# dylkot/cNMF

Measured on AMD Instinct MI355X. Metric: NMF restarts/sec (50000x2000xK5..13), higher is better.
Workload: dtype f32 (exact integer f16 plane x 2 f16 planes with per-row exponent, f32 accumulate)

## Files before the change

### cnmf_amd/csrc/batch_host.hip.h

```cpp
#pragma once

#include "batch_sched.h"

static_assert(PLAN_BK == BK && PLAN_G3_MW == G3_MW && PLAN_G3_JW == G3_JW && PLAN_G3C_JW == G3C_JW && PLAN_G3_BK == G3_BK &&
              PLAN_KSMALL == KSMALL, "pass_plan.h repeats the tile constants of the kernel headers");
static PadShape pad_shape(const cnmf_ctx* ctx) { return PadShape{ctx->N_pad, ctx->G_pad}; }
static int sweep_chunks(const cnmf_ctx* ctx, int L) { return sweep_chunks(ctx->knobs.sweep_parts, L); }
static int sweep_parts(const cnmf_ctx* ctx, int L) { return sweep_parts(ctx->knobs.sweep_parts, L); }

static int ensure_batch(cnmf_ctx* ctx, int KC, int max_k = KMAX, int min_k = 1)
{
    const bool use3 = gemm3_enabled(ctx, KC);
    const SplitCaps caps = size_splits(pad_shape(ctx), KC, use3, gemm3_wg_slots(ctx->knobs));
    const int nsplit = caps.nsplit, nsplitA = caps.nsplitA;
    const int parts = std::max(sweep_parts(ctx, (int)ctx->N), sweep_parts(ctx, (int)ctx->G));
    const size_t gp_need = (size_t)(KC / std::max(1, min_k) + 1) * parts * max_k * max_k;
    if (ctx->bat.kc == KC && ctx->bat.nsplit == nsplit && ctx->bat.nsplitA == nsplitA &&
        ctx->bat.parts == parts && ctx->bat.gram_part_floats >= gp_need && (!use3 || ctx->bat.H3)) return CNMF_OK;
    ctx->bat.release();
    OwnedLocal<BatchBuffersF> b;
    const size_t hb = (size_t)KC * ctx->G_pad * sizeof(float);
    const size_t wb = (size_t)KC * ctx->N_pad * sizeof(float);
    HIP_TRY(ctx, hipMalloc(&b.H, hb));
    HIP_TRY(ctx, hipMalloc(&b.Wt, wb));
    HIP_TRY(ctx, hipMalloc(&b.XHt, wb * nsplitA));
    HIP_TRY(ctx, hipMalloc(&b.XHt1, wb));
    if (use3) {
        HIP_TRY(ctx, hipMalloc(&b.XHt2, wb));
        HIP_TRY(ctx, hipMalloc(&b.H3, (size_t)KC * (ctx->G_pad / 16) * G3_ROWB));
        HIP_TRY(ctx, hipMalloc(&b.Wt3, (size_t)KC * (ctx->N_pad / 16) * G3_ROWB));
        HIP_TRY(ctx, hipMemsetAsync(b.Wt3, 0, (size_t)KC * (ctx->N_pad / 16) * G3_ROWB, ctx->stream));
        HIP_TRY(ctx, hipMalloc(&b.rmaxH, (size_t)KC * parts * sizeof(float)));
        HIP_TRY(ctx, hipMalloc(&b.rmaxW, (size_t)KC * parts * sizeof(float)));
        HIP_TRY(ctx, hipMalloc(&b.iscaleH, (size_t)KC * sizeof(float)));
        HIP_TRY(ctx, hipMalloc(&b.iscaleW, (size_t)KC * sizeof(float)));
        HIP_TRY(ctx, hipMemsetAsync(b.rmaxH, 0, (size_t)KC * parts * sizeof(float), ctx->stream));
        HIP_TRY(ctx, hipMemsetAsync(b.rmaxW, 0, (size_t)KC * parts * sizeof(float), ctx->stream));
        HIP_TRY(ctx, hipMemsetAsync(b.iscaleH, 0, (size_t)KC * sizeof(float), ctx->stream));
        HIP_TRY(ctx, hipMemsetAsync(b.iscaleW, 0, (size_t)KC * sizeof(float), ctx->stream));
        HIP_TRY(ctx, hipMalloc(&b.shiftW, (size_t)3 * KC * sizeof(int)));
        HIP_TRY(ctx, hipMemsetAsync(b.shiftW, 0, (size_t)3 * KC * sizeof(int), ctx->stream));
    }
    HIP_TRY(ctx, hipMalloc(&b.d_split, (size_t)(KC / 32 + 1) * (ctx->N_pad / 128 + 1)));
    HIP_TRY(ctx, hipMalloc(&b.XtW, hb * nsplit));
    HIP_TRY(ctx, hipMalloc(&b.gramH, (size_t)KC * GRAM_SZ * sizeof(float)));
    HIP_TRY(ctx, hipMalloc(&b.gramW, (size_t)KC * GRAM_SZ * sizeof(float)));
    HIP_TRY(ctx, hipMalloc(&b.gram_part, gp_need * sizeof(float)));
    HIP_TRY(ctx, hipMalloc(&b.viol_part, (size_t)KC * parts * sizeof(double)));
    HIP_TRY(ctx, hipMalloc(&b.d_slots, (size_t)KC * sizeof(SlotDesc)));
    HIP_TRY(ctx, hipMalloc(&b.d_slot_list, (size_t)KC * RING * sizeof(int)));
    HIP_TRY(ctx, hipHostMalloc(&b.h_slots, (size_t)KC * sizeof(SlotDesc)));
    HIP_TRY(ctx, hipHostMalloc(&b.h_snap, (size_t)KC * RING * sizeof(SlotDesc),
                               hipHostMallocMapped | hipHostMallocCoherent));
    memset(b.h_snap, 0, (size_t)KC * RING * sizeof(SlotDesc));
    HIP_TRY(ctx, hipHostMalloc(&b.h_slot_list, (size_t)KC * RING * sizeof(int)));
    HIP_TRY(ctx, hipMemsetAsync(b.H, 0, hb, ctx->stream));
    HIP_TRY(ctx, hipMemsetAsync(b.Wt, 0, wb, ctx->stream));
    HIP_TRY(ctx, hipMemsetAsync(b.XHt, 0, wb * nsplitA, ctx->stream));
    HIP_TRY(ctx, hipMemsetAsync(b.XtW, 0, hb * nsplit, ctx->stream));
    HIP_TRY(ctx, hipMemsetAsync(b.d_slots, 0, (size_t)KC * sizeof(SlotDesc), ctx->stream));
    b.kc = KC; b.nsplit = nsplit; b.nsplitA = nsplitA; b.parts = parts; b.gram_part_floats = gp_need;
    ctx->bat.take(b);
    return CNMF_OK;
}

static int ensure_stage(cnmf_ctx* ctx, size_t wfloats, size_t hfloats)
{
    if (wfloats > ctx->stageW_sz) {
        hipFree(ctx->stageW); ctx->stageW = nullptr;
        HIP_TRY(ctx, hipMalloc(&ctx->stageW, wfloats * sizeof(float)));
        ctx->stageW_sz = wfloats;
    }
    if (hfloats > ctx->stageH_sz) {
        hipFree(ctx->stageH); ctx->stageH = nullptr;
        HIP_TRY(ctx, hipMalloc(&ctx->stageH, hfloats * sizeof(float)));
        ctx->stageH_sz = hfloats;
    }
    return CNMF_OK;
}

static int wait_snapshot(cnmf_ctx* ctx, const SlotDesc* sp, int n, int stamp)
{
    using clk = std::chrono::steady_clock;
    for (int s = 0; s < n; ++s) {
        const volatile int* flag = &sp[s].pad_;
        long spins = 0;
        clk::time_point t0;
        bool timing = false;
        while (*flag != stamp) {
            if (++spins % 4096 != 0) continue;
            if (!timing) { t0 = clk::now(); timing = true; continue; }
            if (std::chrono::duration_cast<std::chrono::milliseconds>(clk::now() - t0).count() < 20) continue;
            t0 = clk::now();
            const hipError_t q = hipStreamQuery(ctx->stream);
            if (q == hipSuccess) {
                if (*flag == stamp) break;
                SET_ERR(ctx, "slot snapshot %d was never published (slot %d)", stamp, s);
                return CNMF_EHIP;
            }
            if (q != hipErrorNotReady) {
                SET_ERR(ctx, "stream failed while waiting for a slot snapshot: %s", hipGetErrorString(q));
                return CNMF_EHIP;
            }
        }
    }
    __atomic_thread_fence(__ATOMIC_ACQUIRE);
    return CNMF_OK;
}

static int validate_params(cnmf_ctx* ctx, const cnmf_cd_params* p)
{
    if (!p) { SET_ERR(ctx, "params is NULL"); return CNMF_EINVAL; }
    if (!(p->tol >= 0) || p->max_iter < 1) { SET_ERR(ctx, "bad tol/max_iter"); return CNMF_EINVAL; }
    if (p->l1_reg_W < 0 || p->l2_reg_W < 0 || p->l1_reg_H < 0 || p->l2_reg_H < 0) {
        SET_ERR(ctx, "negative regularisation"); return CNMF_EINVAL;
    }
    return CNMF_OK;
}

static_assert(SCHED_KMAX == KMAX && SCHED_RING == RING, "batch_sched.h repeats KMAX and RING");

struct PassScheme {
    bool use3 = false;
    bool usec = false;
    bool use2g = false;
    bool use2h = false;
    int mode = 0;
    XOperand xA{}, xB{};
    const double* dsc = nullptr;
    int jwA = G3_JW;
    int nsubA = 1, nsubB = 1, KbA = 0, KbB = 0;
    void leave_matrix_pipe() { use3 = usec = use2h = use2g = false; }
};

static int pick_scheme(cnmf_ctx* ctx, int KC, PassScheme* out)
{
    const CdKnobs& kn = ctx->knobs;
    PassScheme p;
    int rc;
    p.use3 = gemm3_enabled(ctx, KC);
    if (p.use3 && kn.gemm3 >= 3) {
        if ((rc = ensure_counts(ctx))) return rc;
        p.usec = ctx->counts.state == 1;
    }
    p.use2g = p.use3 && !p.usec && kn.gemm3 >= 4 && ctx->G_pad % G3C_JW == 0 && ctx->N_pad % G3C_JW == 0;
    if (p.use2g && (rc = ensure_x2planes(ctx))) return rc;
    p.use2h = (p.usec && ctx->counts.fmt == 4) || p.use2g;
    p.mode = !p.use3 ? 0 : (p.use2g ? 5 : (p.usec ? (p.use2h ? 4 : 3) : std::min(kn.gemm3, 2)));
    p.KbA = ctx->G_pad / 16; p.KbB = ctx->N_pad / 16;
    p.xA = p.use2g ? ctx->x2.passA() : ctx->counts.passA();
    p.xB = p.use2g ? ctx->x2.passB() : ctx->counts.passB();
    p.dsc = p.use2g ? nullptr : ctx->counts.d_scale;
    p.nsubA = p.use2h ? gemm2h_nsub(p.xA.hi != nullptr, p.KbA, kn.g2_nsub) : 1;
    p.nsubB = p.use2h ? gemm2h_nsub(p.xB.hi != nullptr, p.KbB, kn.g2_nsub) : 1;
    if (p.use3 && !p.usec && !p.use2g && (rc = ensure_planes(ctx))) return rc;
    p.jwA = (p.usec || p.use2g) ? G3C_JW : G3_JW;
    *out = p;
    return CNMF_OK;
}

struct BatchRun {
    cnmf_ctx* ctx; const cnmf_cd_params* prm; hipStream_t st;
    int n; const int32_t* kk; int init_mode; const double* avg; const float *W0, *H0;
    int32_t* n_iter_out; double* viol_out; bool resident;
    int N, G, max_k; int64_t total_k;
    std::vector<size_t> hoff, woff;
    DevPool pool;
    EventPool events;
    struct PinnedInts { int* p = nullptr; ~PinnedInts() { if (p) hipHostFree(p); } } repack_host;
    float *d_Hres = nullptr, *d_Wres = nullptr;
    float *d_H0 = nullptr, *d_Wt0 = nullptr;
    int* d_repack = nullptr;
    int n_repack = 0;
    PassScheme ps;
    bool fuseW = false;
    int shgen = 0;
    int* shW[2] = {nullptr, nullptr};
    bool h3_valid = false;
    int fin_y = 1, lag = 2;
    int chunksW, partsW, chunksH, partsH;
    float l1W, l2W, l1H, l2H;
    PassPlan plan;
    int time_stride = 0;
    std::vector<hipEvent_t> gev;
    hipEvent_t ev_begin = nullptr, ev_end = nullptr, ev_tail = nullptr;
    int nsplit3_first = 1;
    BatchSched sched;
    BatchRun(int n_, const int32_t* kk_, int KC, const double* hint, bool dbg) : n(n_), kk(kk_), sched(n_, kk_, KC, hint, dbg) {}
};

static int plan_passes(BatchRun& b, int cap, int capA)
{
    cnmf_ctx* ctx = b.ctx;
    PassPlan& p = b.plan;
    plan_pass_splits(p, pad_shape(ctx), b.sched.KC, b.ps.use3, b.ps.jwA, b.ps.nsubA, gemm3_wg_slots(ctx->knobs), ctx->knobs.no_streamk, cap, capA);
    const std::vector<unsigned char>* flags = b.ps.use3 ? (p.sk3.on ? &p.sk3.flags : nullptr) : (p.sk.on ? &p.sk.split : nullptr);
    if (flags) HIP_TRY(ctx, hipMemcpyAsync(ctx->bat.d_split, flags->data(), flags->size(), hipMemcpyHostToDevice, b.st));
    return CNMF_OK;
}

static int retire_slot(BatchRun& b, int s, const SlotDesc& snap)
{
    cnmf_ctx* ctx = b.ctx;
    hipStream_t st = b.st;
    const HostSlot& h = b.sched.hs[s];
    const int r = h.restart, k = h.k, N = b.N, G = b.G;
    dim3 gH((G + 255) / 256, k), gW((N + 255) / 256, k);
    extract_kernel<<<gH, 256, 0, st>>>(ctx->bat.H, ctx->G_pad, G, h.off, k, b.d_Hres + b.hoff[r], 0);
    if (b.d_Wres) extract_kernel<<<gW, 256, 0, st>>>(ctx->bat.Wt, ctx->N_pad, N, h.off, k, b.d_Wres + b.woff[r], 1);
    clear_rows_kernel<<<gH, 256, 0, st>>>(ctx->bat.H, ctx->G_pad, ctx->G_pad, h.off, k);
    clear_rows_kernel<<<gW, 256, 0, st>>>(ctx->bat.Wt, ctx->N_pad, ctx->N_pad, h.off, k);
    HIP_TRY(ctx, hipGetLastError());
    if (b.n_iter_out) b.n_iter_out[r] = snap.iter;
    if (b.viol_out) b.viol_out[r] = snap.viol_last;
    b.sched.retire(s, snap.iter);
    return CNMF_OK;
}

static int repack(BatchRun& b, int width, bool balanced = false)
{
    cnmf_ctx* ctx = b.ctx;
    hipStream_t st = b.st;
    const int KC0 = b.sched.KC0;
    int* hm = b.repack_host.p + (size_t)(b.n_repack++ % RING) * 3 * KC0;
    int* d_colmap = b.d_repack, *d_ids = b.d_repack + KC0, *d_offs = b.d_repack + 2 * KC0;
    const RepackPlan pl = b.sched.plan_repack(width, balanced, hm);
    if (pl.nmove || pl.pos < width) {
        HIP_TRY(ctx, hipMemcpyAsync(d_colmap, hm, (size_t)width * sizeof(int), hipMemcpyHostToDevice, st));
        gather_rows_cm_kernel<<<dim3((ctx->N_pad / 4 + 255) / 256, width), 256, 0, st>>>(ctx->bat.Wt, ctx->N_pad, d_colmap, ctx->bat.XHt);
        gather_rows_cm_kernel<<<dim3((ctx->G_pad / 4 + 255) / 256, width), 256, 0, st>>>(ctx->bat.H, ctx->G_pad, d_colmap, ctx->bat.XtW);
        HIP_TRY(ctx, hipGetLastError());
        HIP_TRY(ctx, hipMemcpyAsync(ctx->bat.Wt, ctx->bat.XHt, (size_t)width * ctx->N_pad * sizeof(float), hipMemcpyDeviceToDevice, st));
        HIP_TRY(ctx, hipMemcpyAsync(ctx->bat.H, ctx->bat.XtW, (size_t)width * ctx->G_pad * sizeof(float), hipMemcpyDeviceToDevice, st));
        if (b.fuseW) {
            int* tmp = ctx->bat.shiftW + 2 * ctx->bat.kc;
            for (int g2 = 0; g2 < 2; ++g2) {
                permute_ints_kernel<<<(width + 255) / 256, 256, 0, st>>>(b.shW[g2], d_colmap, tmp, width);
                HIP_TRY(ctx, hipMemcpyAsync(b.shW[g2], tmp, (size_t)width * sizeof(int), hipMemcpyDeviceToDevice, st));
            }
            HIP_TRY(ctx, hipGetLastError());
        }
        if (pl.nmove) {
            HIP_TRY(ctx, hipMemcpyAsync(d_ids, hm + KC0, (size_t)pl.nmove * sizeof(int), hipMemcpyHostToDevice, st));
            HIP_TRY(ctx, hipMemcpyAsync(d_offs, hm + 2 * KC0, (size_t)pl.nmove * sizeof(int), hipMemcpyHostToDevice, st));
            set_slot_offs_kernel<<<(pl.nmove + 255) / 256, 256, 0, st>>>(ctx->bat.d_slots, d_ids, d_offs, pl.nmove);
            HIP_TRY(ctx, hipGetLastError());
        }
    }
    b.h3_valid = false;
    if (b.ps.use2h) HIP_TRY(ctx, launch_rowmax_part(st, ctx->bat.Wt, ctx->N_pad, b.N, b.sched.KC, b.chunksW * 256, nullptr, b.partsW, ctx->bat.rmaxW));
    return CNMF_OK;
}

static int install(BatchRun& b, const Placement& p)
{
    cnmf_ctx* ctx = b.ctx;
    hipStream_t st = b.st;
    const int r = p.restart, k = p.k, off = p.off, N = b.N, G = b.G;
    dim3 gI((std::max(N, G) + 255) / 256, k);
    if (b.init_mode == 0) {
        HIP_TRY(ctx, hipMemcpyAsync(ctx->stageH, b.H0 + b.hoff[r], (size_t)k * G * sizeof(float), hipMemcpyHostToDevice, st));
        HIP_TRY(ctx, hipMemcpyAsync(ctx->stageW, b.W0 + b.woff[r], (size_t)k * N * sizeof(float), hipMemcpyHostToDevice, st));
        install_kernel<<<gI, 256, 0, st>>>(ctx->stageH, ctx->stageW, ctx->bat.H, ctx->G_pad, G, ctx->bat.Wt, ctx->N_pad, N, off, k);
    } else {
        install_cm_kernel<<<gI, 256, 0, st>>>(b.d_H0 + b.hoff[r], b.d_Wt0 + b.woff[r], ctx->bat.H, ctx->G_pad, G, ctx->bat.Wt, ctx->N_pad, N, off);
    }
    HIP_TRY(ctx, hipGetLastError());
    if (b.fuseW) {
        float mx = 0.f;
        if (b.init_mode == 1) mx = 6.0f * (float)b.avg[r];
        else if (b.init_mode == 2) mx = ctx->inits.maxW[r];
        else for (size_t q = 0; q < (size_t)k * N; ++q) mx = std::max(mx, b.W0[b.woff[r] + q]);
        int e2 = 0;
        if (mx > 0.f) std::frexp(mx, &e2);
        const int sh0 = mx > 0.f ? std::max(-110, std::min(120, 13 - e2)) : 0;
        set_ints_kernel<<<1, 128, 0, st>>>(b.shW[0], b.shW[1], off, k, sh0);
        HIP_TRY(ctx, hipGetLastError());
    }
    SlotDesc* d = &ctx->bat.h_slots[p.slot];
    memset(d, 0, sizeof *d);
    d->off = off; d->k = k; d->active = 1; d->iter = 0; d->restart = r;
    HIP_TRY(ctx, hipMemcpyAsync(ctx->bat.d_slots + p.slot, d, sizeof(SlotDesc), hipMemcpyHostToDevice, st));
    return CNMF_OK;
}

static int refill(BatchRun& b, int& n_new)
{
    cnmf_ctx* ctx = b.ctx;
    BatchSched& sc = b.sched;
    n_new = 0;
    int* new_list = ctx->bat.h_slot_list + (size_t)(sc.it % RING) * sc.KC0;
    int rc;
    sc.begin_refill();
    while (true) {
        Placement p;
        while (sc.next_placement(&p)) {
            if ((rc = install(b, p))) return rc;
            new_list[n_new++] = p.slot;
        }
        if (!sc.defrag_due()) break;
// ... 551 lines not shown
```

### cnmf_amd/csrc/cnmf_hip.hip

```cpp
#include <hip/hip_runtime.h>

#include <algorithm>
#include <chrono>
#include <cmath>
#include <cstdint>
#include <cstdio>
#include <cstdlib>
#include <cstring>
#include <functional>
#include <string>
#include <vector>

#include "../../include/cnmf_hip.h"
#ifdef CNMF_DEBUG_ABI
#include "../../include/cnmf_hip_debug.h"
#endif
#include "kernels_gemm.hip.h"
#include "kernels_gemm3.hip.h"
#include "kernels_counts.hip.h"
#include "kernels_planes.hip.h"
#include "kernels_gemm2h.hip.h"
#include "kernels_rng.hip.h"
#include "kernels_sweep.hip.h"

// ... 65 lines not shown

extern "C" void cnmf_destroy(cnmf_ctx* ctx)
{
    if (!ctx) return;
    hipSetDevice(ctx->device);
    hipStreamSynchronize(ctx->stream);
    ctx->bat.release();
    cnmf_comm_finalize(ctx);
    drop_derived_images(ctx);
    hipFree(ctx->X);
    hipFree(ctx->stageW); hipFree(ctx->stageH); hipFree(ctx->spectra);
    ctx->cons_ws.release();
    ctx->prep.release();
    ctx->pre.release();
    ctx->har.release();
    if (ctx->cons_pinned) hipHostFree(ctx->cons_pinned);
    hipStreamDestroy(ctx->stream);
    delete ctx;
}

static int alloc_dense(cnmf_ctx* ctx)
{
    const size_t bytes = ((size_t)ctx->N_pad + 1) * ctx->G_pad * sizeof(float);
    HIP_TRY(ctx, hipMalloc(&ctx->X, bytes));
    HIP_TRY(ctx, hipMemsetAsync(ctx->X, 0, bytes, ctx->stream));
    return CNMF_OK;
}

static int alloc_matrix(cnmf_ctx* ctx, int64_t N, int64_t G, bool dense = true)
{
    if (N <= 0 || G <= 0 || N > (1ll << 30) || G > (1ll << 24)) {
        SET_ERR(ctx, "bad matrix shape %lld x %lld", (long long)N, (long long)G);
        return CNMF_EINVAL;
    }
    HIP_TRY(ctx, hipSetDevice(ctx->device));
    ctx->bat.release();
    drop_derived_images(ctx);
    hipFree(ctx->X); ctx->X = nullptr;
    ctx->iter_prior.clear(); ctx->iter_hint.clear();
    ctx->N = N; ctx->G = G;
    ctx->N_pad = round_up(N, N >= 512 ? 256 : 128);
    ctx->G_pad = round_up(G, G >= 512 ? 256 : 32);
    return dense ? alloc_dense(ctx) : CNMF_OK;
}

extern "C" int cnmf_set_matrix(cnmf_ctx* ctx, const float* X, int64_t N, int64_t G)
{
    if (!ctx || !X) { SET_ERR(ctx, "null argument"); return CNMF_EINVAL; }
    int rc = alloc_matrix(ctx, N, G);
    if (rc) return rc;
    HIP_TRY(ctx, hipMemcpy2DAsync(ctx->X, (size_t)ctx->G_pad * sizeof(float), X,
                                  (size_t)G * sizeof(float), (size_t)G * sizeof(float), (size_t)N,
                                  hipMemcpyHostToDevice, ctx->stream));
    HIP_TRY(ctx, hipStreamSynchronize(ctx->stream));
    return CNMF_OK;
}

__global__ void csr_densify_kernel(const long long* __restrict__ indptr, const int* __restrict__ indices,
                                   const float* __restrict__ data, float* __restrict__ X, int ld,
                                   int n_rows, int n_cols, int* __restrict__ bad)
{
    const int row = blockIdx.x;
    if (row >= n_rows) return;
    const long long b = indptr[row], e = indptr[row + 1];
    for (long long p = b + threadIdx.x; p < e; p += blockDim.x) {
        const int c = indices[p];
        if (c < 0 || c >= n_cols) { if (bad) atomicOr(bad, 2); continue; }
        if (bad && ((p > b && indices[p - 1] >= c) || data[p] == 0.f)) atomicOr(bad, 1);
        if (X) atomicAdd(&X[(size_t)row * ld + c], data[p]);
    }
}

static int ensure_dense(cnmf_ctx* ctx)
{
    if (ctx->X) return CNMF_OK;
    if (ctx->N <= 0 || !ctx->csr.ptr) { SET_ERR(ctx, "cnmf_set_matrix has not been called"); return CNMF_ESTATE; }
    HIP_TRY(ctx, hipSetDevice(ctx->device));
    int rc = alloc_dense(ctx);
    if (rc) return rc;
    if (ctx->csr.nnz > 0) {
        csr_densify_kernel<<<(unsigned)ctx->N, 64, 0, ctx->stream>>>(ctx->csr.ptr, ctx->csr.idx, ctx->csr.val, ctx->X, ctx->G_pad,
                                                                    (int)ctx->N, (int)ctx->G, nullptr);
        hipError_t e = hipGetLastError();
        if (e == hipSuccess) e = hipStreamSynchronize(ctx->stream);
        if (e != hipSuccess) { hipFree(ctx->X); ctx->X = nullptr; HIP_TRY(ctx, e); }
    }
    return CNMF_OK;
}

extern "C" int cnmf_set_matrix_csr(cnmf_ctx* ctx, const int32_t* indptr, const int32_t* indices,
                                   const float* data, int64_t N, int64_t G)
{
    if (!ctx || !indptr || (!indices && indptr[N] > 0) || (!data && indptr[N] > 0)) {
        SET_ERR(ctx, "null argument");
        return CNMF_EINVAL;
    }
    int rc = alloc_matrix(ctx, N, G, false);
    if (rc) return rc;
    const int64_t nnz = indptr[N];
    DevPool pool;
    int* d_ptr32 = pool.get<int>((size_t)(N + 1));
    int* d_bad = pool.get<int>(1, true, ctx->stream);
    POOL_TRY(ctx, pool);
    hipStream_t st = ctx->stream;
    DevCsrLocal<float> L;
    HIP_TRY(ctx, L.alloc_ptr(N, G));
    HIP_TRY(ctx, L.alloc_entries(nnz));
    HIP_TRY(ctx, hipMemcpyAsync(d_ptr32, indptr, (size_t)(N + 1) * sizeof(int), hipMemcpyHostToDevice, st));
    if (nnz > 0) {
        HIP_TRY(ctx, hipMemcpyAsync(L.idx, indices, (size_t)nnz * sizeof(int), hipMemcpyHostToDevice, st));
        HIP_TRY(ctx, hipMemcpyAsync(L.val, data, (size_t)nnz * sizeof(float), hipMemcpyHostToDevice, st));
    }
    int bad = 0;
    cnmf::csr_widen_ptr_kernel<<<(unsigned)((N + 1 + 255) / 256), 256, 0, st>>>(d_ptr32, N + 1, L.ptr);
    if (nnz > 0) csr_densify_kernel<<<(unsigned)N, 64, 0, st>>>(L.ptr, L.idx, L.val, nullptr, ctx->G_pad, (int)N, (int)G, d_bad);
    HIP_TRY(ctx, hipGetLastError());
    HIP_TRY(ctx, hipMemcpyAsync(&bad, d_bad, sizeof(int), hipMemcpyDeviceToHost, st));
    HIP_TRY(ctx, hipStreamSynchronize(st));
    if (bad & 2) { SET_ERR(ctx, "column index out of range in the CSR arrays"); return CNMF_EINVAL; }
    ctx->csr.take(L);
    if (bad & 1) {
        rc = ensure_dense(ctx);
        free_csr(ctx);
        if (rc) return rc;
    }
    return CNMF_OK;
}

extern "C" int cnmf_set_count_detection(cnmf_ctx* ctx, int enabled)
{
    if (!ctx) return CNMF_EINVAL;
    if (ctx->count_detect != (enabled != 0)) {
        ctx->count_detect = enabled != 0;
        if (ctx->counts.state == -1 || !ctx->count_detect) {
            hipStreamSynchronize(ctx->stream);
            ctx->counts.release();
        }
    }
    return CNMF_OK;
}

extern "C" int cnmf_get_shape(const cnmf_ctx* ctx, int64_t* N, int64_t* G)
{
    if (!ctx) return CNMF_EINVAL;
    if (N) *N = ctx->N;
    if (G) *G = ctx->G;
    return (ctx->X || ctx->csr.ptr) ? CNMF_OK : CNMF_ESTATE;
}

extern "C" int cnmf_matrix_images(const cnmf_ctx* ctx, int32_t* flags)
{
    if (!ctx || !flags) return CNMF_EINVAL;
    *flags = (ctx->X ? 1 : 0) | (ctx->csr.ptr ? 2 : 0) | (ctx->csc.ptr ? 4 : 0) | (ctx->XtF.p ? 8 : 0) |
             ((ctx->spA[0].ent && ctx->spB[0].ent) ? 16 : 0) | ((ctx->spA[1].ent && ctx->spB[1].ent) ? 32 : 0) | (ctx->counts.C1 ? 64 : 0);
    return CNMF_OK;
}

#include "batch_host.hip.h"

#include "consensus_host.hip.h"
#include "linkage_host.hip.h"

#include "mu_host.hip.h"
#include "mu_refit_host.hip.h"
#include "comm_host.hip.h"
#include "normalize_host.hip.h"
#include "prepare_host.hip.h"
#include "preprocess_host.hip.h"
#include "pca_host.hip.h"
#include "tridiag_eig_host.hip.h"
#include "harmony_host.hip.h"
#include "harmony_init_host.hip.h"
#include "filter_host.hip.h"
#include "hvg_host.hip.h"
#include "hvg_batch_host.hip.h"
#include "select_mi_host.hip.h"
#include "tail_host.hip.h"
#include "mu2_refit_host.hip.h"

#include "debug_host.hip.h"
#include "nndsvd_host.hip.h"
#include "nndsvd_tail_host.hip.h"
#include "format_host.hip.h"
```

### cnmf_amd/csrc/debug_host.hip.h

```cpp
#pragma once

extern "C" int cnmf_x_matmul(cnmf_ctx* ctx, int trans, const float* Q, int ncols, float* out)
{
    if (!ctx || !Q || !out) { SET_ERR(ctx, "null argument"); return CNMF_EINVAL; }
    if (int rcd_ = ensure_dense(ctx)) return rcd_;
    if (ncols < 1 || ncols > 256 || (trans != 0 && trans != 1)) { SET_ERR(ctx, "bad ncols/trans"); return CNMF_EINVAL; }
    HIP_TRY(ctx, hipSetDevice(ctx->device));
    hipStream_t st = ctx->stream;
    const int N = (int)ctx->N, G = (int)ctx->G;
    const int KC = ncols <= 32 ? 32 : (ncols <= 64 ? 64 : (ncols <= 128 ? 128 : 256));
    const int Kin = trans ? N : G, Kp = trans ? ctx->N_pad : ctx->G_pad;
    const int Jout = trans ? G : N, Jp = trans ? ctx->G_pad : ctx->N_pad;
    DevPool pool;
    float* dQ = pool.get<float>((size_t)Kin * ncols);
    float* dA = pool.get<float>((size_t)KC * Kp, true, st);
    const int nsplit = trans ? std::max(1, std::min(16, Kp / 2048)) : 1;
    float* dC = pool.get<float>((size_t)nsplit * KC * Jp);
    float* dO = pool.get<float>((size_t)Jout * ncols);
    if (pool.err) { SET_ERR(ctx, "device allocation failed"); return CNMF_ENOMEM; }
    HIP_TRY(ctx, hipMemcpyAsync(dQ, Q, (size_t)Kin * ncols * sizeof(float), hipMemcpyHostToDevice, st));
    dim3 gI((Kin + 255) / 256, ncols);
    install_kernel<<<gI, 256, 0, st>>>(nullptr, dQ, dA, Kp, 0, dA, Kp, Kin, 0, ncols);
    if (!trans)
        HIP_TRY(ctx, launch_gemm<false>(st, 0, dA, Kp, ctx->X, ctx->G_pad, dC, Jp, 0, KC, Kp, Jp, 1));
// ... 20 lines not shown
    HIP_TRY(ctx, hipSetDevice(ctx->device));
    hipStream_t st = ctx->stream;
    const int Jp = round_up(J, 128);
    const int Kp = K;
    DevPool pool;
    EventPool events;
    const size_t bA = (size_t)KC * Kp * sizeof(float);
    const size_t bB = (mode == 0 ? (size_t)Jp * Kp : ((size_t)Kp + 1) * J + 128) * sizeof(float);
    const size_t bC = (size_t)nsplit * KC * Jp * sizeof(float);
    float* dA = pool.get<float>(bA / sizeof(float));
    float* dB = pool.get<float>(bB / sizeof(float));
    float* dC = pool.get<float>(bC / sizeof(float));
    POOL_TRY(ctx, pool);
    HIP_TRY(ctx, hipMemsetAsync(dB, 0, bB, st));
    HIP_TRY(ctx, hipMemcpyAsync(dA, A, bA, hipMemcpyHostToDevice, st));
    HIP_TRY(ctx, hipMemcpyAsync(dB, B, (size_t)(mode == 0 ? J : Kp) * (mode == 0 ? Kp : J) * sizeof(float), hipMemcpyHostToDevice, st));
    hipEvent_t e0 = events.get(), e1 = events.get();
    POOL_TRY(ctx, events);
    reps = std::max(1, reps);
    for (int i = 0; i < reps + 1; ++i) {
        if (i == 1) hipEventRecord(e0, st);
        hipError_t e = (mode == 0)
            ? launch_gemm<false>(st, variant, dA, Kp, dB, Kp, dC, Jp, (long long)KC * Jp, KC, Kp, Jp, 1, ctx->knobs.s_mtw2)
            : launch_gemm<true>(st, variant, dA, Kp, dB, J, dC, Jp, (long long)KC * Jp, KC, Kp, J, nsplit, ctx->knobs.s_mtw2);
        HIP_TRY(ctx, e);
    }
    hipEventRecord(e1, st);
    HIP_TRY(ctx, hipStreamSynchronize(st));
    float ms = 0.f;
    if (reps >= 1) hipEventElapsedTime(&ms, e0, e1);
    if (ms_out) *ms_out = (reps >= 1) ? ms / reps : 0.0;
    std::vector<float> hc((size_t)(mode == 0 ? 1 : nsplit) * KC * Jp);
    HIP_TRY(ctx, hipMemcpy(hc.data(), dC, hc.size() * sizeof(float), hipMemcpyDeviceToHost));
    for (int c = 0; c < KC; ++c)
        for (int j = 0; j < J; ++j) {
            float s = hc[(size_t)c * Jp + j];
            if (mode == 1)
                for (int z = 1; z < nsplit; ++z) s += hc[((size_t)z * KC + c) * Jp + j];
            C[(size_t)c * J + j] = s;
        }
    return CNMF_OK;
}

extern "C" int cnmf_debug_gemm3(cnmf_ctx* ctx, const float* A, const float* B, float* C, int KC, int K, int J,
                                int nsplit, double* ms_out, int reps)
{
    if (!ctx || !A || !B || !C) { SET_ERR(ctx, "null argument"); return CNMF_EINVAL; }
    if (KC % 256 || K % 16 || J < 1 || nsplit < 1) { SET_ERR(ctx, "debug_gemm3 needs KC %% 256 == 0, K %% 16 == 0"); return CNMF_EINVAL; }
    HIP_TRY(ctx, hipSetDevice(ctx->device));
    hipStream_t st = ctx->stream;
    const int Jp = round_up(J, gemm3_jw()), Kb = K / 16;
    DevPool pool;
    EventPool events;
    float* dA = pool.get<float>((size_t)KC * K);
    float* dB = pool.get<float>((size_t)Jp * K, true, st);
    unsigned char* dA3 = pool.get<unsigned char>((size_t)KC * Kb * G3_ROWB);
    unsigned char* dB3 = pool.get<unsigned char>((size_t)Jp * Kb * G3_ROWB);
    float* dC = pool.get<float>((size_t)nsplit * KC * Jp);
    hipEvent_t e0 = events.get(), e1 = events.get();
    POOL_TRY(ctx, pool);
    POOL_TRY(ctx, events);
    HIP_TRY(ctx, hipMemcpyAsync(dA, A, (size_t)KC * K * sizeof(float), hipMemcpyHostToDevice, st));
    HIP_TRY(ctx, hipMemcpyAsync(dB, B, (size_t)J * K * sizeof(float), hipMemcpyHostToDevice, st));
    HIP_TRY(ctx, launch_split3(st, dA, K, KC, K, dA3, G3_MW));
    HIP_TRY(ctx, launch_split3(st, dB, K, Jp, K, dB3, gemm3_jw()));
    reps = std::max(1, reps);
    int zs = 1;
    for (int i = 0; i < reps + 1; ++i) {
        if (i == 1) hipEventRecord(e0, st);
        HIP_TRY(ctx, launch_gemm3(st, dA3, dB3, Kb, dC, Jp, (long long)KC * Jp, KC, Jp, nsplit, ctx->knobs.gemm3));
    }
    hipEventRecord(e1, st);
    HIP_TRY(ctx, hipStreamSynchronize(st));
    { const int kb_per = (Kb + nsplit - 1) / nsplit; zs = (Kb + kb_per - 1) / kb_per; }
    float ms = 0.f;
    hipEventElapsedTime(&ms, e0, e1);
    if (ms_out) *ms_out = ms / reps;
    std::vector<float> hc((size_t)zs * KC * Jp);
    HIP_TRY(ctx, hipMemcpy(hc.data(), dC, hc.size() * sizeof(float), hipMemcpyDeviceToHost));
    for (int c = 0; c < KC; ++c)
        for (int j = 0; j < J; ++j) {
            float v = hc[(size_t)c * Jp + j];
            for (int z = 1; z < zs; ++z) v += hc[((size_t)z * KC + c) * Jp + j];
            C[(size_t)c * J + j] = v;
        }
    return CNMF_OK;
}

extern "C" int cnmf_debug_gemm3c(cnmf_ctx* ctx, const float* A, const float* Bn, float* C, int KC, int K, int J,
                                 int nsplit, double* ms_out, int reps)
{
    if (!ctx || !A || !Bn || !C) { SET_ERR(ctx, "null argument"); return CNMF_EINVAL; }
    if (KC % 256 || K % 16 || J < 1 || nsplit < 1) { SET_ERR(ctx, "debug_gemm3c needs KC %% 256 == 0, K %% 16 == 0"); return CNMF_EINVAL; }
    HIP_TRY(ctx, hipSetDevice(ctx->device));
    hipStream_t st = ctx->stream;
    const int Jp = round_up(J, G3C_JW), Kb = K / 16;
    DevPool pool;
    EventPool events;
    float* dA = pool.get<float>((size_t)KC * K);
    float* dB = pool.get<float>((size_t)J * K);
    float* dUnit = pool.get<float>(K);
    unsigned char* dA3 = pool.get<unsigned char>((size_t)KC * Kb * G3_ROWB);
    unsigned char* dB1 = pool.get<unsigned char>((size_t)Jp * Kb * 32);
    unsigned char* dBh = pool.get<unsigned char>((size_t)Jp * Kb * 32);
    unsigned int* dFl = pool.get<unsigned int>((size_t)(Jp / G3C_JW) * ((Kb + 31) / 32), true, st);
    float* dC = pool.get<float>((size_t)nsplit * KC * Jp);
    hipEvent_t e0 = events.get(), e1 = events.get();
    POOL_TRY(ctx, pool);
    POOL_TRY(ctx, events);
    std::vector<float> ones(K, 1.0f);
    HIP_TRY(ctx, hipMemcpyAsync(dA, A, (size_t)KC * K * sizeof(float), hipMemcpyHostToDevice, st));
    HIP_TRY(ctx, hipMemcpyAsync(dB, Bn, (size_t)J * K * sizeof(float), hipMemcpyHostToDevice, st));
    HIP_TRY(ctx, hipMemcpyAsync(dUnit, ones.data(), (size_t)K * sizeof(float), hipMemcpyHostToDevice, st));
    HIP_TRY(ctx, launch_split3(st, dA, K, KC, K, dA3, G3_MW));
    HIP_TRY(ctx, launch_x_planes(st, XPlaneFormat::COUNT_BF16, false, dB, K, J, K, Jp, K, dUnit, dB1, dBh, dFl));
    reps = std::max(1, reps);
    for (int i = 0; i < reps + 1; ++i) {
        if (i == 1) hipEventRecord(e0, st);
        HIP_TRY(ctx, launch_gemm3c(st, dA3, dB1, dBh, dFl, Kb, dC, Jp, (long long)KC * Jp, KC, Jp, nsplit));
    }
    hipEventRecord(e1, st);
    HIP_TRY(ctx, hipStreamSynchronize(st));
    const int kb_per = (Kb + nsplit - 1) / nsplit, zs = (Kb + kb_per - 1) / kb_per;
    float ms = 0.f;
    hipEventElapsedTime(&ms, e0, e1);
    if (ms_out) *ms_out = ms / reps;
    std::vector<float> hc((size_t)zs * KC * Jp);
    HIP_TRY(ctx, hipMemcpy(hc.data(), dC, hc.size() * sizeof(float), hipMemcpyDeviceToHost));
    for (int c = 0; c < KC; ++c)
        for (int j = 0; j < J; ++j) {
            float v = hc[(size_t)c * Jp + j];
            for (int z = 1; z < zs; ++z) v += hc[((size_t)z * KC + c) * Jp + j];
            C[(size_t)c * J + j] = v;
        }
    return CNMF_OK;
}

__global__ __launch_bounds__(256) void debug_rowbound_part_kernel(const float* __restrict__ V, int ld, int L, int span,
                                                                  int parts, float* __restrict__ rmax_part)
{
    const int row = blockIdx.y * 4 + (threadIdx.x >> 6), lane = threadIdx.x & 63, p = blockIdx.x;
    const int j0 = p * span, j1 = min(L, j0 + span);
    float s = 0.f;
    for (int j = j0 + lane; j < j1; j += 64) { const float x = V[(size_t)row * ld + j]; s = fmaf(x, x, s); }
#pragma unroll
    for (int o = 32; o > 0; o >>= 1) s += __shfl_xor(s, o, 64);
    if (lane == 0) rmax_part[(size_t)row * parts + p] = sqrtf(s) * 1.0001f;
}

extern "C" int cnmf_debug_gemm2h(cnmf_ctx* ctx, const float* A, const float* Bn, float* C, int KC, int K, int J,
                                 int nsplit, int nsub, double* ms_out, int reps)
{
    const bool sweep_bound = (nsub & 128) != 0;
    nsub &= 127;
    if (!ctx || !A || !Bn || !C) { SET_ERR(ctx, "null argument"); return CNMF_EINVAL; }
    if (KC % 256 || K % 64 || J < 1 || nsplit < 1) { SET_ERR(ctx, "debug_gemm2h needs KC %% 256 == 0, K %% 64 == 0"); return CNMF_EINVAL; }
    HIP_TRY(ctx, hipSetDevice(ctx->device));
    hipStream_t st = ctx->stream;
    const int Jp = round_up(J, G3C_JW), Kb = K / 16;
    bool has_hi = false;
    for (size_t i = 0; i < (size_t)J * K && !has_hi; ++i) has_hi = Bn[i] > G2_COUNT_BASE;
    DevPool pool;
    EventPool events;
    float* dA = pool.get<float>((size_t)KC * K);
    float* dB = pool.get<float>((size_t)J * K);
    float* dUnit = pool.get<float>(K);
    const int bparts = sweep_bound ? (K + 1023) / 1024 : 1;
    float* dRmax = pool.get<float>((size_t)KC * bparts);
    float* dInv = pool.get<float>(KC);
    unsigned char* dA2 = pool.get<unsigned char>((size_t)KC * Kb * G2_ROWB);
    unsigned char* dB1 = pool.get<unsigned char>((size_t)Jp * Kb * 32);
    unsigned char* dBh = has_hi ? pool.get<unsigned char>((size_t)Jp * Kb * 32) : nullptr;
    unsigned int* dFl = pool.get<unsigned int>((size_t)(Jp / G3C_JW) * ((Kb + 31) / 32), true, st);
    float* dC = pool.get<float>((size_t)nsplit * KC * Jp);
    hipEvent_t e0 = events.get(), e1 = events.get();
    POOL_TRY(ctx, pool);
    POOL_TRY(ctx, events);
    std::vector<float> ones(K, 1.0f);
    HIP_TRY(ctx, hipMemcpyAsync(dA, A, (size_t)KC * K * sizeof(float), hipMemcpyHostToDevice, st));
    HIP_TRY(ctx, hipMemcpyAsync(dB, Bn, (size_t)J * K * sizeof(float), hipMemcpyHostToDevice, st));
    HIP_TRY(ctx, hipMemcpyAsync(dUnit, ones.data(), (size_t)K * sizeof(float), hipMemcpyHostToDevice, st));
    if (sweep_bound) {
        debug_rowbound_part_kernel<<<dim3(bparts, KC / 4), 256, 0, st>>>(dA, K, K, 1024, bparts, dRmax);
        HIP_TRY(ctx, hipGetLastError());
    } else
        HIP_TRY(ctx, launch_rowmax_part(st, dA, K, K, KC, K, nullptr, 1, dRmax));
    HIP_TRY(ctx, launch_split2h(st, dA, K, KC, K, dA2, G3_MW, nullptr, dRmax, bparts, dInv));
    HIP_TRY(ctx, launch_x_planes(st, XPlaneFormat::COUNT_F16, false, dB, K, J, K, Jp, K, dUnit, dB1, dBh, dFl));
    reps = std::max(1, reps);
    const int var = (nsub >> 4) & 7;
    nsub &= 15;
    const int ns = (!has_hi && nsub == 2 && Kb % 2 == 0) ? 2 : 1;
    G2Launch g;
    g.A2 = dA2; g.rscale = dInv; g.x = XOperand{dB1, dBh, dFl, nullptr}; g.Kb = Kb;
    g.C[0] = dC; g.ldc = Jp; g.cstride = (long long)KC * Jp; g.KC = KC; g.Jpad = Jp; g.nsplit = nsplit;
    for (int i = 0; i < reps + 1; ++i) {
        if (i == 1) hipEventRecord(e0, st);
        hipError_t e;
        if (has_hi) e = launch_gemm2h_t<1, true>(st, g);
        else if (ns == 2 && var == 2) e = launch_gemm2h_t<2, false, 2>(st, g);
        else if (ns == 2 && var == 3) e = launch_gemm2h_t<2, false, 3>(st, g);
        else if (ns == 2 && var == 4) e = launch_gemm2h_t<2, false, 4>(st, g);
        else if (ns == 2 && var == 6) e = launch_gemm2h_t<2, false, 6>(st, g);
        else if (ns == 2 && var == 7) e = launch_gemm2h_t<2, false, 7>(st, g);
        else if (ns == 2) e = launch_gemm2h_t<2, false, 0>(st, g);
        else e = launch_gemm2h_t<1, false>(st, g);
        HIP_TRY(ctx, e);
    }
    hipEventRecord(e1, st);
    HIP_TRY(ctx, hipStreamSynchronize(st));
    const int zs = gemm2h_splits(Kb, nsplit, ns);
    float ms = 0.f;
    hipEventElapsedTime(&ms, e0, e1);
    if (ms_out) *ms_out = ms / reps;
    std::vector<float> hc((size_t)zs * KC * Jp);
    HIP_TRY(ctx, hipMemcpy(hc.data(), dC, hc.size() * sizeof(float), hipMemcpyDeviceToHost));
    for (int c = 0; c < KC; ++c)
        for (int j = 0; j < J; ++j) {
            float v = hc[(size_t)c * Jp + j];
            for (int z = 1; z < zs; ++z) v += hc[((size_t)z * KC + c) * Jp + j];
            C[(size_t)c * J + j] = v;
        }
    return CNMF_OK;
}

namespace cnmf {
__global__ __launch_bounds__(256) void calib_copy1_kernel(const float* __restrict__ a, float* __restrict__ b, long long n)
{
    for (long long i = (long long)blockIdx.x * 256 + threadIdx.x; i < n; i += (long long)gridDim.x * 256) b[i] = a[i];
}
__global__ __launch_bounds__(256) void calib_copy4_kernel(const float4* __restrict__ a, float4* __restrict__ b, long long n4)
{
    for (long long i = (long long)blockIdx.x * 256 + threadIdx.x; i < n4; i += (long long)gridDim.x * 256) b[i] = a[i];
}
__global__ __launch_bounds__(256) void calib_ldsdma_kernel(const unsigned char* __restrict__ a, long long nbytes, float* __restrict__ sink)
{
    __shared__ __attribute__((aligned(16))) unsigned char buf[4][4096];
    const long long chunk = 4096;
    float acc = 0.f;
    for (long long off = (long long)blockIdx.x * chunk; off + chunk <= nbytes; off += (long long)gridDim.x * chunk) {
        const int w = (threadIdx.x >> 6);
        __builtin_amdgcn_global_load_lds(G3_AS1(a + off + threadIdx.x * 16), G3_AS3(&buf[0][0] + w * 1024), 16, 0, 0);
        asm volatile("s_waitcnt vmcnt(0)" ::: "memory");
        acc += reinterpret_cast<const float*>(&buf[0][0])[threadIdx.x];
    }
    if (acc == 1.2345f) sink[0] = acc;
}
}

extern "C" int cnmf_debug_stream(cnmf_ctx* ctx, int width, long long n_floats, int reps)
{
    using namespace cnmf;
    if (!ctx || n_floats < 1024 || reps < 1) { SET_ERR(ctx, "bad argument"); return CNMF_EINVAL; }
    HIP_TRY(ctx, hipSetDevice(ctx->device));
    hipStream_t st = ctx->stream;
    DevPool pool;
    n_floats = (n_floats / 1024) * 1024;
    float* a = pool.get<float>((size_t)n_floats, true, st);
    float* b = pool.get<float>((size_t)n_floats, true, st);
    POOL_TRY(ctx, pool);
    for (int r = 0; r < reps; ++r) {
        if (width == 1) calib_copy1_kernel<<<4096, 256, 0, st>>>(a, b, n_floats);
        else if (width == 4) calib_copy4_kernel<<<4096, 256, 0, st>>>((const float4*)a, (float4*)b, n_floats / 4);
        else calib_ldsdma_kernel<<<2048, 256, 0, st>>>((const unsigned char*)a, n_floats * 4, b);
    }
    HIP_TRY(ctx, hipGetLastError());
    HIP_TRY(ctx, hipStreamSynchronize(st));
    return CNMF_OK;
}

extern "C" int cnmf_debug_standard_normal(cnmf_ctx* ctx, uint32_t seed, int64_t n, double* out)
{
    if (!ctx || !out || n < 0) { SET_ERR(ctx, "bad argument"); return CNMF_EINVAL; }
    HIP_TRY(ctx, hipSetDevice(ctx->device));
    DevPool pool;
    double* d = pool.get<double>((size_t)n);
    POOL_TRY(ctx, pool);
    launch_standard_normal(ctx->stream, seed, n, d);
    HIP_TRY(ctx, hipGetLastError());
    HIP_TRY(ctx, hipMemcpyAsync(out, d, (size_t)n * sizeof(double), hipMemcpyDeviceToHost, ctx->stream));
    HIP_TRY(ctx, hipStreamSynchronize(ctx->stream));
    return CNMF_OK;
}
#endif
```

### cnmf_amd/csrc/gemm_host.hip.h

```cpp
#pragma once

#include "pass_plan.h"


template <int MTW, int WM, int WN, bool NN, int TBK = BK>
static hipError_t launch_gemm_t(hipStream_t st, const float* A, int lda, const float* B, int ldb,
                                float* C, int ldc, long long cstride, int KC, int Ktot, int J,
                                int nsplit)
{
    constexpr int MW = WM * MTW * 32, JW = WN * 32;
    const int Kper = round_up((Ktot + nsplit - 1) / nsplit, BK);
    dim3 grid((J + JW - 1) / JW, KC / MW, nsplit);
    constexpr size_t lds = gemm_lds_bytes<MTW, WM, WN, NN, TBK>();
    {
        if (hipError_t e_ = dyn_lds_optin((const void*)gemm_kernel<MTW, WM, WN, NN, TBK>, (int)lds)) return e_;
    }
    gemm_kernel<MTW, WM, WN, NN, TBK><<<grid, 256, lds, st>>>(A, lda, B, ldb, C, ldc, cstride, Kper,
                                                             Ktot, J);
    return hipGetLastError();
}

template <bool NN>
static hipError_t launch_gemm(hipStream_t st, int variant, const float* A, int lda, const float* B,
                              int ldb, float* C, int ldc, long long cstride, int KC, int Ktot,
// ... 15 lines not shown
            if (KC % 128 == 0) GO(4, 1, 4);
            if (KC % 64 == 0) GO(2, 1, 4);
            GO(1, 1, 4);
    }
#undef GO
}

static constexpr CutPlanes NO_CUT{nullptr, nullptr, 1, 1, 1, nullptr};
static constexpr PlaneOut NO_PLANES{nullptr, nullptr, 0, 0};

struct SweepLaunch {
    int nslots = 0;
    float* V = nullptr; int ldv = 0, L = 0;
    const float* P = nullptr;
    enum { ONE_PLANE, CUT_PLANES, SPLIT_SUM } from = ONE_PLANE;
    CutPlanes cut = NO_CUT;
    SplitSum sum{1, 0, nullptr};
    const float* gram = nullptr;
    const SlotDesc* slots = nullptr;
    float l1 = 0.f;
    float* gram_part = nullptr; double* viol_part = nullptr;
    int chunks = 1, parts = 1;
    int want_gram = 0, kmax = 0, tiers = 0;
    float* rmax_part = nullptr;
    const double* rmax_scale = nullptr;
    const PlaneOut* planes = nullptr;
};

using SweepFn = void (*)(float*, int, int, const float*, SplitInfo, const float*, const SlotDesc*, float, float*, double*, int, int, int,
                         int, float*, const double*, PlaneOut);
static constexpr SweepFn SWEEP_KERNELS[6][3] = {
    {sweep_kernel<0>, sweep_kernel<1>, sweep_kernel<2>},
    {sweep_kernel<0, false, false, false, true>, sweep_kernel<1, false, false, false, true>, sweep_kernel<2, false, false, false, true>},
    {sweep_kernel<0, false, false, true>, sweep_kernel<1, false, false, true>, sweep_kernel<2, false, false, true>},
    {sweep_kernel<0, false, false, true, true>, sweep_kernel<1, false, false, true, true>, sweep_kernel<2, false, false, true, true>},
    {sweep_kernel<0, true>, sweep_kernel<1, true>, sweep_kernel<2, true>},
    {sweep_kernel<0, true, true>, sweep_kernel<1, true, true>, sweep_kernel<2, true, true>}};

static hipError_t launch_sweep(hipStream_t st, const SweepLaunch& s)
{
    const bool pln = s.planes != nullptr, exact = s.rmax_part && s.rmax_scale;
    const SweepForm form = sweep_form(pln, s.from == SweepLaunch::SPLIT_SUM, exact, sweep_a64(s.ldv), s.tiers);
    if (form == SweepForm::INVALID || (pln && s.planes->TR != G3_MW)) return hipErrorInvalidValue;
    SplitInfo sp;
    if (form == SweepForm::H_PSUM) sp.sum = s.sum;
    else sp.cut = s.from == SweepLaunch::CUT_PLANES ? s.cut : NO_CUT;
    const dim3 grid(s.parts, s.nslots);
    for (int t = 0; t < 3; ++t) {
        if (!(s.tiers & (1 << t))) continue;
        const SweepFn fn = SWEEP_KERNELS[(int)form][t];
        if (hipError_t e_ = dyn_lds_optin((const void*)fn, (int)sweep_lds_bytes(KSMALL, pln))) return e_;
        fn<<<grid, 256, sweep_lds_bytes(s.kmax, pln), st>>>(s.V, s.ldv, s.L, s.P, sp, s.gram, s.slots, s.l1, s.gram_part, s.viol_part, s.chunks,
                                                           s.want_gram, sweep_kg(s.kmax), s.kmax, s.rmax_part, pln ? nullptr : s.rmax_scale,
                                                           pln ? *s.planes : NO_PLANES);
    }
    if (s.tiers & 8) {
        const size_t blds = sweep_big_lds_bytes();
        const auto big = exact ? sweep_big_kernel<true> : sweep_big_kernel<false>;
        if (hipError_t e_ = dyn_lds_optin((const void*)big, (int)blds)) return e_;
        big<<<grid, 256, blds, st>>>(s.V, s.ldv, s.L, s.P, sp, s.gram, s.slots, s.l1, s.viol_part, s.chunks, exact ? s.rmax_part : nullptr,
                                     exact ? s.rmax_scale : nullptr);
        if (s.want_gram)
            gram_big_kernel<<<grid, 256, 0, st>>>(s.V, s.ldv, s.L, s.slots, s.gram_part, s.chunks, s.kmax,
                                                  (s.rmax_part && !s.rmax_scale) ? s.rmax_part : nullptr);
    }
    return hipGetLastError();
}

static hipError_t launch_streamk_passA(hipStream_t st, const StreamK& sk, const float* A, int lda,
                                       const float* B, int ldb, float* C0, float* C1, int ldc, int Jtot)
{
    constexpr size_t lds = gemm_lds_bytes<4, 1, 4, false>();
    {
        if (hipError_t e_ = dyn_lds_optin((const void*)gemm_streamk_kernel<4, 1, 4, false>, (int)lds)) return e_;
    }
    gemm_streamk_kernel<4, 1, 4, false><<<sk.P, 256, lds, st>>>(A, lda, B, ldb, C0, C1, ldc, sk.MG, sk.T,
                                                               sk.nk, Jtot);
    return hipGetLastError();
}

static hipError_t launch_reduce_splits(hipStream_t st, float* P, int nsplit, long long split_stride,
                                       long long n_floats, const double* colscale = nullptr, int ld = 1)
{
    if (nsplit <= 1 && !colscale) return hipSuccess;
    const long long nv = n_floats / 4;
    reduce_splits_kernel<<<(unsigned)((nv + 255) / 256), 256, 0, st>>>(P, nsplit, split_stride, P, nv, colscale, ld);
    return hipGetLastError();
}


static hipError_t launch_split3(hipStream_t st, const float* src, int ld, int rows, int K, unsigned char* dst, int TR,
                                const double* kscale = nullptr)
{
    if (rows % 64 == 0 && K % 64 == 0 && TR % 64 == 0) {
        if (rows / 64 > PLAN_GRID_YZ) return hipErrorInvalidValue;
        dim3 grid(K / 64, rows / 64);
        split3_tiled_kernel<<<grid, 256, 0, st>>>(src, ld, K, TR, (unsigned short*)dst, kscale);
        return hipGetLastError();
    }
    const long long total = (long long)rows * (K / 16);
    split3_kernel<<<(unsigned)((total + 255) / 256), 256, 0, st>>>(src, ld, rows, K, TR, (unsigned short*)dst, kscale);
    return hipGetLastError();
}

static int gemm3_wg_slots(const CdKnobs& k) { return gemm3_wg_slots(k.gemm3, k.wg_slots); }
static int gemm3_jw() { return G3_JW; }

static hipError_t launch_gemm3(hipStream_t st, const unsigned char* A3, const unsigned char* B3, int Kb,
                               float* C, int ldc, long long cstride, int KC, int Jpad, int nsplit, int gemm3_mode)
{
    {
        if (hipError_t e_ = dyn_lds_optin((const void*)gemm3_kernel, G3_LDS_BYTES)) return e_;
        if (hipError_t e_ = dyn_lds_optin((const void*)gemm3g_kernel, G3G_LDS_BYTES)) return e_;
    }
    const int kb_per = (Kb + nsplit - 1) / nsplit;
    dim3 grid(Jpad / gemm3_jw(), KC / G3_MW, (Kb + kb_per - 1) / kb_per);
    if (gemm3_mode >= 2)
        gemm3g_kernel<<<grid, 512, G3G_LDS_BYTES, st>>>(A3, B3, Kb, C, ldc, cstride, kb_per);
    else
        gemm3_kernel<<<grid, 256, G3_LDS_BYTES, st>>>(A3, B3, Kb, C, ldc, cstride, kb_per);
    return hipGetLastError();
}


static hipError_t launch_split3_finalize(hipStream_t st, const float* src, int ld, int rows, int K, unsigned char* dst,
                                         int TR, const double* kscale, const FinalizeArgs& fa, int nslots, int fin_y)
{
    const int bx = K / 64, by = rows / 64;
    split3_finalize_kernel<<<bx * by + nslots * fin_y, 256, 0, st>>>(src, ld, K, TR, (unsigned short*)dst, kscale, bx, by,
                                                                  fa, fin_y);
    return hipGetLastError();
}

static hipError_t launch_split2h_finalize(hipStream_t st, const float* src, int ld, int rows, int K, unsigned char* dst,
                                          int TR, const double* kscale, const float* rmax_part, int parts,
                                          float* inv_scale, const FinalizeArgs& fa, int nslots, int fin_y,
                                          SplitFused fu = SplitFused{nullptr, nullptr});

static hipError_t launch_gemm3_streamk(hipStream_t st, const StreamK3& sk, const unsigned char* A3,
                                       const unsigned char* B3, float* C0, float* C1, float* C2, int ldc,
                                       int gemm3_mode)
{
    {
        if (hipError_t e_ = dyn_lds_optin((const void*)gemm3_streamk_kernel, G3_LDS_BYTES)) return e_;
        if (hipError_t e_ = dyn_lds_optin((const void*)gemm3g_streamk_kernel, G3G_LDS_BYTES)) return e_;
    }
    if (gemm3_mode >= 2)
        gemm3g_streamk_kernel<<<sk.P, 512, G3G_LDS_BYTES, st>>>(A3, B3, sk.Kb, C0, C1, C2, ldc, sk.MG, sk.T);
    else
        gemm3_streamk_kernel<<<sk.P, 256, G3_LDS_BYTES, st>>>(A3, B3, sk.Kb, C0, C1, C2, ldc, sk.MG, sk.T);
    return hipGetLastError();
}

enum class XPlaneFormat { COUNT_BF16, COUNT_F16, SPLIT_F16 };

template <class F>
static hipError_t launch_x_planes_t(hipStream_t st, bool transpose, const float* X, int ld, int N, int G, int rows_pad, int K,
                                    const void* aux, unsigned char* plane0, unsigned char* plane1, unsigned int* flags)
{
    const auto* a = static_cast<const typename F::Aux*>(aux);
    auto* p0 = reinterpret_cast<unsigned short*>(plane0);
    auto* p1 = reinterpret_cast<unsigned short*>(plane1);
    if (transpose) {
        const int groups = (rows_pad + 255) / 256;
        if (groups > PLAN_GRID_YZ) return hipErrorInvalidValue;
        x_planes_kernel<F, true><<<dim3(K / 16, groups), 256, 0, st>>>(X, ld, N, G, rows_pad, K, G3C_JW, a, p0, p1, flags);
    } else {
        const long long blocks = ((long long)rows_pad * (K / 16) + 255) / 256;
        if (blocks > 0x7fffffffll) return hipErrorInvalidValue;
        x_planes_kernel<F, false><<<(unsigned)blocks, 256, 0, st>>>(X, ld, N, G, rows_pad, K, G3C_JW, a, p0, p1, flags);
    }
    return hipGetLastError();
}

static hipError_t launch_x_planes(hipStream_t st, XPlaneFormat fmt, bool transpose, const float* X, int ld, int N, int G,
                                  int rows_pad, int K, const void* aux, unsigned char* plane0, unsigned char* plane1,
                                  unsigned int* flags = nullptr)
{
    switch (fmt) {
        case XPlaneFormat::COUNT_BF16: return launch_x_planes_t<CountBf16>(st, transpose, X, ld, N, G, rows_pad, K, aux, plane0, plane1, flags);
        case XPlaneFormat::COUNT_F16: return launch_x_planes_t<CountF16>(st, transpose, X, ld, N, G, rows_pad, K, aux, plane0, plane1, flags);
        default: return launch_x_planes_t<SplitF16>(st, transpose, X, ld, N, G, rows_pad, K, aux, plane0, plane1, flags);
    }
}

static int ensure_planes(cnmf_ctx* ctx)
{
    const int TR = gemm3_jw();
    if (ctx->planes.X3 && ctx->planes.tr == TR) return CNMF_OK;
    ctx->planes.release();
    const size_t bA = (size_t)ctx->N_pad * (ctx->G_pad / 16) * G3_ROWB;
    const size_t bB = (size_t)ctx->G_pad * (ctx->N_pad / 16) * G3_ROWB;
    OwnedLocal<Bf16PlanesF> L;
    L.tr = TR;
    HIP_TRY(ctx, hipMalloc(&L.X3, bA));
    HIP_TRY(ctx, hipMalloc(&L.Xt3, bB));
    HIP_TRY(ctx, launch_split3(ctx->stream, ctx->X, ctx->G_pad, ctx->N_pad, ctx->G_pad, L.X3, TR));
    dim3 grid(ctx->N_pad / 16, (ctx->G_pad + 255) / 256);
    split3_transpose_kernel<<<grid, 256, 0, ctx->stream>>>(ctx->X, ctx->G_pad, ctx->N_pad, ctx->G_pad, ctx->N_pad,
                                                            TR, (unsigned short*)L.Xt3);
    HIP_TRY(ctx, hipGetLastError());
    HIP_TRY(ctx, hipStreamSynchronize(ctx->stream));
    ctx->planes.take(L);
    return CNMF_OK;
}

static int ensure_x2planes(cnmf_ctx* ctx)
{
    if (ctx->x2.X2h) return CNMF_OK;
    hipStream_t st = ctx->stream;
    const int N = (int)ctx->N, G = (int)ctx->G, Np = ctx->N_pad, Gp = ctx->G_pad;
    const size_t pb = (size_t)Np * Gp * 2;
    const size_t fa = (size_t)(Np / G3C_JW) * ((Gp / 16 + 31) / 32) * sizeof(unsigned), fb = (size_t)(Gp / G3C_JW) * ((Np / 16 + 31) / 32) * sizeof(unsigned);
    DevPool pool;
    int* shA = pool.get<int>(Np);
    int* shB = pool.get<int>(Gp);
    POOL_TRY(ctx, pool);
    OwnedLocal<GeneralPlanesF> L;
    HIP_TRY(ctx, hipMalloc(&L.X2h, pb));
    HIP_TRY(ctx, hipMalloc(&L.X2m, pb));
    HIP_TRY(ctx, hipMalloc(&L.Xt2h, pb));
    HIP_TRY(ctx, hipMalloc(&L.Xt2m, pb));
    HIP_TRY(ctx, hipMalloc(&L.sA, (size_t)Np * sizeof(float)));
    HIP_TRY(ctx, hipMalloc(&L.sB, (size_t)Gp * sizeof(float)));
    HIP_TRY(ctx, hipMalloc(&L.onesA, fa));
    HIP_TRY(ctx, hipMalloc(&L.onesB, fb));
    HIP_TRY(ctx, hipMemsetAsync(L.onesA, 0xff, fa, st));
    HIP_TRY(ctx, hipMemsetAsync(L.onesB, 0xff, fb, st));
    x2h_rowshift_kernel<<<(Np + 3) / 4, 256, 0, st>>>(ctx->X, Gp, N, G, 0, Np, shA, L.sA);
    x2h_rowshift_kernel<<<(Gp + 255) / 256, 256, 0, st>>>(ctx->X, Gp, N, G, 1, Gp, shB, L.sB);
    HIP_TRY(ctx, hipGetLastError());
    HIP_TRY(ctx, launch_x_planes(st, XPlaneFormat::SPLIT_F16, false, ctx->X, Gp, N, G, Np, Gp, shA, L.X2h, L.X2m));
    HIP_TRY(ctx, launch_x_planes(st, XPlaneFormat::SPLIT_F16, true, ctx->X, Gp, N, G, Gp, Np, shB, L.Xt2h, L.Xt2m));
    HIP_TRY(ctx, hipStreamSynchronize(st));
    ctx->x2.take(L);
    return CNMF_OK;
}

static hipError_t launch_gemm3c(hipStream_t st, const unsigned char* A3, const unsigned char* B1,
                                const unsigned char* Bhi, const unsigned int* hiflag, int Kb,
                                float* C, int ldc, long long cstride, int KC, int Jpad, int nsplit)
{
    {
        if (hipError_t e_ = dyn_lds_optin((const void*)gemm3c_kernel, g3c_lds_bytes(true))) return e_;
    }
    const int kb_per = (Kb + nsplit - 1) / nsplit;
    dim3 grid(Jpad / G3C_JW, KC / G3_MW, (Kb + kb_per - 1) / kb_per);
    gemm3c_kernel<<<grid, 512, g3c_lds_bytes(Bhi != nullptr), st>>>(A3, B1, Bhi, hiflag, Kb, C, ldc, cstride, kb_per);
    return hipGetLastError();
}

static hipError_t launch_gemm3c_streamk(hipStream_t st, const StreamK3& sk, const unsigned char* A3,
                                        const unsigned char* B1, const unsigned char* Bhi,
                                        const unsigned int* hiflag, float* C0, float* C1, float* C2, int ldc)
{
    {
        if (hipError_t e_ = dyn_lds_optin((const void*)gemm3c_streamk_kernel, g3c_lds_bytes(true))) return e_;
    }
    gemm3c_streamk_kernel<<<sk.P, 512, g3c_lds_bytes(Bhi != nullptr), st>>>(A3, B1, Bhi, hiflag, sk.Kb, C0, C1, C2, ldc,
                                                                            sk.MG, sk.T);
    return hipGetLastError();
}


struct G2Launch {
    const unsigned char* A2 = nullptr;
    const float* rscale = nullptr;
    XOperand x{};
    int Kb = 0;
    float* C[3] = {nullptr, nullptr, nullptr};
    int ldc = 0;
    unsigned long long livemask = ~0ull;
    long long cstride = 0; int KC = 0, Jpad = 0, nsplit = 1;
    const StreamK3* sk = nullptr;
    const CdKnobs* kn = nullptr;
};
using G2Fn = hipError_t (*)(hipStream_t, const G2Launch&);
struct G2Entry { G2Form form; G2Fn fn; };

template <int NSUB, bool HI, int VAR = 0, bool PART = false, bool GEN = false>
static hipError_t launch_gemm2h_t(hipStream_t st, const G2Launch& g)
{
    constexpr int lds = G2Geom<NSUB, HI>::LDS_BYTES;
    {
        if (hipError_t e_ = dyn_lds_optin((const void*)gemm2h_kernel<NSUB, HI, VAR, PART, GEN>, lds)) return e_;
    }
    int kb_per = (g.Kb + g.nsplit - 1) / g.nsplit;
    kb_per = ((kb_per + NSUB - 1) / NSUB) * NSUB;
    dim3 grid(g.Jpad / G3C_JW, g.KC / G3_MW, (g.Kb + kb_per - 1) / kb_per);
    gemm2h_kernel<NSUB, HI, VAR, PART, GEN><<<grid, 512, lds, st>>>(g.A2, g.x.plane, HI ? g.x.hi : nullptr, HI ? g.x.flags : nullptr, g.rscale,
                                                                   g.Kb, g.C[0], g.ldc, g.cstride, kb_per, g.x.colscale,
                                                                   PART ? g.livemask : ~0ull);
    return hipGetLastError();
}

template <int NSUB, bool HI, int VAR = 0, bool NTB = true, bool PART = false, bool GEN = false>
static hipError_t launch_gemm2h_streamk_t(hipStream_t st, const G2Launch& g)
{
    constexpr int lds = G2Geom<NSUB, HI>::LDS_BYTES;
    {
        if (hipError_t e_ = dyn_lds_optin((const void*)gemm2h_streamk_kernel<NSUB, HI, VAR, NTB, PART, GEN>, lds)) return e_;
    }
    const int xmap = g2_xmap(G2Form{true, NSUB, HI, VAR, NTB, PART, GEN}, g.kn->g2_xmap);
    gemm2h_streamk_kernel<NSUB, HI, VAR, NTB, PART, GEN><<<g.sk->P, 512, lds, st>>>(g.A2, g.x.plane, HI ? g.x.hi : nullptr,
                                                                                    HI ? g.x.flags : nullptr, g.rscale, g.Kb, g.C[0], g.C[1],
                                                                                    g.C[2], g.ldc, g.sk->MG, g.sk->T, xmap, g.x.colscale,
                                                                                    PART ? g.livemask : ~0ull);
    return hipGetLastError();
}

template <int NSUB, bool HI, int VAR, bool PART, bool GEN>
static constexpr G2Entry g2_ksplit() { return {G2Form{true, NSUB, HI, VAR, false, PART, GEN}, launch_gemm2h_t<NSUB, HI, VAR, PART, GEN>}; }
template <int NSUB, bool HI, int VAR, bool NTB, bool PART, bool GEN>
static constexpr G2Entry g2_streamk() { return {G2Form{true, NSUB, HI, VAR, NTB, PART, GEN}, launch_gemm2h_streamk_t<NSUB, HI, VAR, NTB, PART, GEN>}; }

static constexpr G2Entry G2_KSPLIT[] = {
    g2_ksplit<1, true, 0, false, true>(),  g2_ksplit<1, true, 0, true, true>(),  g2_ksplit<1, true, 4, false, true>(),
    g2_ksplit<1, true, 4, true, true>(),   g2_ksplit<1, true, 0, false, false>(), g2_ksplit<1, true, 0, true, false>(),
    g2_ksplit<2, false, 4, false, false>(), g2_ksplit<2, false, 4, true, false>(), g2_ksplit<1, false, 4, false, false>()};
static constexpr G2Entry G2_STREAMK[] = {
    g2_streamk<1, true, 0, false, true, true>(),   g2_streamk<1, true, 0, false, false, true>(),  g2_streamk<1, true, 0, true, false, true>(),
    g2_streamk<1, true, 4, false, true, true>(),   g2_streamk<1, true, 4, false, false, true>(),  g2_streamk<1, true, 4, true, false, true>(),
    g2_streamk<1, true, 0, false, true, false>(),  g2_streamk<1, true, 0, false, false, false>(), g2_streamk<1, true, 0, true, false, false>(),
    g2_streamk<2, false, 4, false, true, false>(), g2_streamk<2, false, 4, false, false, false>(), g2_streamk<2, false, 4, true, false, false>(),
    g2_streamk<1, false, 4, false, false, false>(), g2_streamk<1, false, 4, true, false, false>()};

static G2Form g2_form_of(const G2Launch& g, int KC, bool shared)
{
    const unsigned long long full = g2_full_mask(KC);
    return g2_form(g.x.hi != nullptr, g.x.colscale != nullptr, g.kn->g2_gen4, g.kn->g2_gvar, gemm2h_nsub(false, g.Kb, g.kn->g2_nsub),
                   (g.livemask & full) != full, shared);
}

static hipError_t launch_gemm2h(hipStream_t st, const G2Launch& g)
{
    G2Form f = g2_form_of(g, g.KC, false);
    f.NTB = false;
    for (const G2Entry& e : G2_KSPLIT) if (e.form == f) return e.fn(st, g);
    return hipErrorInvalidValue;
}

static hipError_t launch_gemm2h_streamk(hipStream_t st, const G2Launch& g)
{
    const G2Form f = g2_form_of(g, g.sk->MG * G3_MW, g.sk->MG > 1);
    for (const G2Entry& e : G2_STREAMK) if (e.form == f) return e.fn(st, g);
    return hipErrorInvalidValue;
}

static hipError_t launch_split2h(hipStream_t st, const float* src, int ld, int rows, int K, unsigned char* dst, int TR,
                                 const double* kscale, const float* rmax_part, int parts, float* inv_scale)
{
    if (split2h_wide(K)) {
        dim3 grid(split2h_col_groups(K, rows), rows / 16);
        split2h_tiled_kernel<16, 16><<<grid, 256, 0, st>>>(src, ld, K, TR, (unsigned short*)dst, kscale, rmax_part, parts, inv_scale);
    } else {
        dim3 grid(split2h_col_groups(K, rows), rows / 64);
        split2h_tiled_kernel<64, 4><<<grid, 256, 0, st>>>(src, ld, K, TR, (unsigned short*)dst, kscale, rmax_part, parts, inv_scale);
    }
    return hipGetLastError();
}

static hipError_t launch_rowmax_part(hipStream_t st, const float* V, int ld, int L, int rows, int span,
                                     const double* kscale, int parts, float* rmax_part)
{
    dim3 grid(parts, rows / 4);
    rowmax_part_kernel<<<grid, 256, 0, st>>>(V, ld, L, span, kscale, parts, rmax_part);
    return hipGetLastError();
}

static int ensure_counts(cnmf_ctx* ctx)
{
    const int fmt = ctx->knobs.gemm3 == 4 ? 4 : 3;
    if (ctx->counts.state == 1 && ctx->counts.fmt != fmt) {
        hipStreamSynchronize(ctx->stream);
        ctx->counts.release();
    }
    if (ctx->counts.state != 0) return CNMF_OK;
    auto absent = [ctx] { ctx->counts.state = -1; return CNMF_OK; };
    const int N = (int)ctx->N, G = (int)ctx->G;
    if (ctx->N_pad % G3C_JW || ctx->G_pad % G3C_JW || ctx->knobs.no_counts || !ctx->count_detect) return absent();
    hipStream_t st = ctx->stream;
    const int chunks = (N + CNT_ROWS - 1) / CNT_ROWS;
    if (chunks > PLAN_GRID_YZ) { SET_ERR(ctx, "count detection: too many rows for one launch"); return CNMF_EINVAL; }
    DevPool pool;
    float* part = pool.get<float>((size_t)chunks * G);
    float* vmin = pool.get<float>(G);
    unsigned* fail = pool.get<unsigned>(G, true, st);
    float* unit = pool.get<float>(G);
    double* psx = pool.get<double>((size_t)chunks * G);
    double* psn = pool.get<double>((size_t)chunks * G);
    POOL_TRY(ctx, pool);
    dim3 grid((G + 255) / 256, chunks);
    col_minpos_kernel<<<grid, 256, 0, st>>>(ctx->X, ctx->G_pad, N, G, part);
    col_min_combine_kernel<<<(G + 255) / 256, 256, 0, st>>>(part, chunks, G, vmin);
    count_check_kernel<<<grid, 256, 0, st>>>(ctx->X, ctx->G_pad, N, G, vmin, fail);
    HIP_TRY(ctx, hipGetLastError());
    std::vector<float> h_v(G), h_unit(G);
    std::vector<unsigned> h_fail(G);
    HIP_TRY(ctx, hipMemcpyAsync(h_v.data(), vmin, (size_t)G * sizeof(float), hipMemcpyDeviceToHost, st));
    HIP_TRY(ctx, hipMemcpyAsync(h_fail.data(), fail, (size_t)G * sizeof(unsigned), hipMemcpyDeviceToHost, st));
    HIP_TRY(ctx, hipStreamSynchronize(st));
    for (int g = 0; g < G; ++g) {
        int m = 0;
        for (int c = 1; c <= CNT_MAXMULT && !m; ++c) if (!(h_fail[g] & (1u << (c - 1)))) m = c;
        if (!m) return absent();
        h_unit[g] = h_v[g] > 0.f ? h_v[g] / (float)m : 0.f;
    }
    HIP_TRY(ctx, hipMemcpyAsync(unit, h_unit.data(), (size_t)G * sizeof(float), hipMemcpyHostToDevice, st));
    OwnedLocal<CountPlanesF> L;
    L.fmt = fmt;
    HIP_TRY(ctx, hipMalloc(&L.d_scale, (size_t)ctx->G_pad * sizeof(double)));
    count_sums_kernel<<<grid, 256, 0, st>>>(ctx->X, ctx->G_pad, N, G, unit, psx, psn);
    count_scale_kernel<<<(ctx->G_pad + 255) / 256, 256, 0, st>>>(psx, psn, chunks, G, ctx->G_pad, L.d_scale);
    unsigned* any_big = pool.get<unsigned>(1, true, st);
    POOL_TRY(ctx, pool);
    count_max_base_kernel<<<grid, 256, 0, st>>>(ctx->X, ctx->G_pad, N, G, unit, fmt == 4 ? G2_COUNT_BASE : 256.0f, any_big);
    unsigned h_big = 0;
    HIP_TRY(ctx, hipMemcpyAsync(&h_big, any_big, sizeof h_big, hipMemcpyDeviceToHost, st));
    HIP_TRY(ctx, hipStreamSynchronize(st));
    const size_t bytes = (size_t)ctx->N_pad * ctx->G_pad * 2;
    HIP_TRY(ctx, hipMalloc(&L.C1, bytes));
    HIP_TRY(ctx, hipMalloc(&L.Ct1, bytes));
    if (h_big) {
        const size_t nfA = (size_t)(ctx->N_pad / G3C_JW) * ((ctx->G_pad / 16 + 31) / 32) * sizeof(unsigned int);
        const size_t nfB = (size_t)(ctx->G_pad / G3C_JW) * ((ctx->N_pad / 16 + 31) / 32) * sizeof(unsigned int);
        HIP_TRY(ctx, hipMalloc(&L.C1h, bytes));
        HIP_TRY(ctx, hipMalloc(&L.Ct1h, bytes));
        HIP_TRY(ctx, hipMalloc(&L.hiA, nfA));
        HIP_TRY(ctx, hipMalloc(&L.hiB, nfB));
        HIP_TRY(ctx, hipMemsetAsync(L.hiA, 0, nfA, st));
        HIP_TRY(ctx, hipMemsetAsync(L.hiB, 0, nfB, st));
    }
    const XPlaneFormat pf = fmt == 4 ? XPlaneFormat::COUNT_F16 : XPlaneFormat::COUNT_BF16;
    HIP_TRY(ctx, launch_x_planes(st, pf, false, ctx->X, ctx->G_pad, N, G, ctx->N_pad, ctx->G_pad, unit, L.C1, L.C1h, L.hiA));
    HIP_TRY(ctx, launch_x_planes(st, pf, true, ctx->X, ctx->G_pad, N, G, ctx->G_pad, ctx->N_pad, unit, L.Ct1, L.Ct1h, L.hiB));
    HIP_TRY(ctx, hipGetLastError());
    HIP_TRY(ctx, hipStreamSynchronize(st));
    L.state = 1;
    ctx->counts.take(L);
    return CNMF_OK;
}

static bool gemm3_enabled(const cnmf_ctx* ctx, int KC)
{
    return ctx->knobs.gemm3 != 0 && KC % G3_MW == 0 && ctx->G_pad % gemm3_jw() == 0 && ctx->N_pad % gemm3_jw() == 0 &&
           x_launches_fit(PadShape{ctx->N_pad, ctx->G_pad}, ctx->knobs.gemm3);
}

static hipError_t launch_split2h_finalize(hipStream_t st, const float* src, int ld, int rows, int K, unsigned char* dst,
                                          int TR, const double* kscale, const float* rmax_part, int parts,
                                          float* inv_scale, const FinalizeArgs& fa, int nslots, int fin_y, SplitFused fu)
{
    const int bx = split2h_col_groups(K, rows);
    if (split2h_wide(K)) {
        const int by = rows / 16;
        split2h_finalize_kernel<16, 16><<<bx * by + nslots * fin_y, 256, 0, st>>>(src, ld, K, TR, (unsigned short*)dst, kscale,
                                                                                rmax_part, parts, inv_scale, bx, by, fa, fin_y, fu);
    } else {
        const int by = rows / 64;
        split2h_finalize_kernel<64, 4><<<bx * by + nslots * fin_y, 256, 0, st>>>(src, ld, K, TR, (unsigned short*)dst, kscale,
                                                                               rmax_part, parts, inv_scale, bx, by, fa, fin_y, fu);
    }
    return hipGetLastError();
}
```

### cnmf_amd/csrc/kernels_gemm2h.hip.h

```cpp
#pragma once
#include <hip/hip_runtime.h>
#include "kernels_gemm3.hip.h"

namespace cnmf {

typedef _Float16 f16x8 __attribute__((ext_vector_type(8)));
typedef float f32x4_g __attribute__((ext_vector_type(4)));

constexpr int G2_ROWB = 64;
constexpr int G2_A = G3_MW * G2_ROWB;
constexpr int G2_B = G3C_JW * 32;

template <int NSUB, bool HI>
struct G2Geom {
    static_assert(NSUB == 1 || (NSUB == 2 && !HI), "two blocks per step: one count plane only");
    static constexpr int IMGS = NSUB == 1 ? 4 : 3;
    static constexpr int IMG = NSUB * (G2_A + (HI ? 2 : 1) * G2_B);
    static constexpr int OFF_B = NSUB * G2_A, OFF_H = OFF_B + NSUB * G2_B;
    static constexpr int NA = NSUB * 2, NB = NSUB;
    static constexpr int AHEAD = IMGS - 1;
    static constexpr int LDS_BYTES = IMGS * IMG;
};

template <int NSUB> struct G2Sub {};

#define G2_DMA_PIECE(NSUB_, HI_, NTB_, s_, i_)                                                     \
    {                                                                                              \
        using GEO_ = G2Geom<NSUB_, HI_>;                                                           \
        unsigned char* d_ = smem + ((s_) % GEO_::IMGS) * GEO_::IMG + wave * 1024;                  \
        if ((i_) < GEO_::NA)                                                                       \
            __builtin_amdgcn_global_load_lds(G3_AS1(abase + (size_t)(s_) * ((NSUB_) * G2_A) + (i_) * 8192), \
                                             G3_AS3(d_ + (i_) * 8192), 16, 0, 0);                  \
        else if ((i_) < GEO_::NA + GEO_::NB)    \
            __builtin_amdgcn_global_load_lds(G3_AS1(bbase + (size_t)(s_) * ((NSUB_) * G2_B) + ((i_) - GEO_::NA) * 8192), \
                                             G3_AS3(d_ + GEO_::OFF_B + ((i_) - GEO_::NA) * 8192), 16, 0, (NTB_) ? 2 : 0); \
        else if constexpr (HI_)                                                                    \
            __builtin_amdgcn_global_load_lds(G3_AS1(hbase + (size_t)(s_) * ((NSUB_) * G2_B) + ((i_) - GEO_::NA - GEO_::NB) * 8192), \
                                             G3_AS3(d_ + GEO_::OFF_H + ((i_) - GEO_::NA - GEO_::NB) * 8192), 16, 0, (NTB_) ? 2 : 0); \
    }

template <bool PART>
__device__ __forceinline__ unsigned g2_wave_live(unsigned live, int grp)
{
    return PART ? (unsigned)__builtin_amdgcn_readfirstlane((int)((live >> (grp * 4)) & 0xfu)) : 0xfu;
}


template <int VAR, bool NTB, bool PART>
__device__ __forceinline__ void gemm2h_segment_mf16(const unsigned char* __restrict__ A2, const unsigned char* __restrict__ B1,
                                                    const float* __restrict__ rscale, int Kb, float* __restrict__ C,
                                                    int ldc, int m0, int j0, int kb0, int nkb, unsigned char* smem,
                                                    unsigned live)
{
    static_assert(VAR == 0 || VAR == 2 || VAR == 3 || VAR == 4 || VAR == 6 || VAR == 7, "instruction streams 1 and 5 were retired");
    using GEO = G2Geom<2, false>;
    constexpr int NSUB = 2, IMGS = GEO::IMGS, IMG = GEO::IMG, OFF_B = GEO::OFF_B, NA = GEO::NA, NB = GEO::NB, AHEAD = GEO::AHEAD;
    constexpr bool BURST = VAR == 0, NOMFMA = VAR == 2, NODMA = VAR == 3 || VAR == 6 || VAR == 7;
    constexpr bool NOREAD = VAR == 6 || VAR == 7, NOBAR = VAR == 7;
    static_assert(IMGS == 3 && NA + NB == 6, "three images, six pieces per step");
    const int tid = threadIdx.x;
    const int lane = tid & 63, wave = tid >> 6;
    const int grp = wave >> 2, wn = wave & 3;
    const int r = lane & 15, g = lane >> 4;
    const int ub = g >> 1, hf = g & 1;
    const int nst = nkb / NSUB;
    const unsigned lv = g2_wave_live<PART>(live, grp);
#define G2_LIVE(mt_) (!PART || ((lv >> ((mt_) >> 1)) & 1u))

    const unsigned char* abase = A2 + ((size_t)(m0 / G3_MW) * Kb + kb0) * G2_A + tid * 16;
    const unsigned char* bbase = B1 + ((size_t)(j0 / G3C_JW) * Kb + kb0) * G2_B + tid * 16;
    constexpr const unsigned char* hbase = nullptr;

    f32x4_g acc[8][4];
#pragma unroll
    for (int mt = 0; mt < 8; ++mt)
#pragma unroll
        for (int nt = 0; nt < 4; ++nt)
#pragma unroll
            for (int i = 0; i < 4; ++i) acc[mt][nt][i] = 0.f;

    const int a_row = ub * G2_A + (grp * 128 + r) * G2_ROWB;
    const int a_s0 = ((0 + hf) ^ ((r >> 2) & 3)) * 16, a_s1 = ((2 + hf) ^ ((r >> 2) & 3)) * 16;
    const int b_off = OFF_B + ub * G2_B + (wn * 64 + r) * 32 + (hf ^ ((r >> 3) & 1)) * 16;

#define G2_PIECE(s_, i_) { G2_DMA_PIECE(2, false, NTB, s_, i_) __builtin_amdgcn_sched_barrier(0); }
#define G2_ISSUE(s_) { _Pragma("unroll") for (int i = 0; i < NA + NB; ++i) G2_PIECE(s_, i) }
#define G2_FRAG(ptr_) __builtin_bit_cast(f16x8, *reinterpret_cast<const u32x4*>(ptr_))
#define G2_AFRAG(bb_, mt_, q_) G2_FRAG((bb_) + a_row + (mt_) * 16 * G2_ROWB + ((q_) ? a_s1 : a_s0))
#define G2_READ_A(s_)                                                                              \
    {                                                                                              \
        const unsigned char* bb = smem + ((s_) % IMGS) * IMG;                                      \
        _Pragma("unroll") for (int nt = 0; nt < 4; ++nt) bq[nt] = G2_FRAG(bb + b_off + nt * 16 * 32); \
        _Pragma("unroll") for (int mp = 0; mp < 4; mp += 2) {                                      \
            aq[mp][1] = G2_AFRAG(bb, mp, 1); aq[mp + 1][1] = G2_AFRAG(bb, mp + 1, 1);              \
            aq[mp][0] = G2_AFRAG(bb, mp, 0); aq[mp + 1][0] = G2_AFRAG(bb, mp + 1, 0);              \
        }                                                                                          \
        __builtin_amdgcn_sched_barrier(0);                                                         \
    }
#define G2_READ_B(s_)                                                                              \
    {                                                                                              \
        const unsigned char* bb = smem + ((s_) % IMGS) * IMG;                                      \
        _Pragma("unroll") for (int mp = 4; mp < 8; mp += 2) {                                      \
            aq[mp][1] = G2_AFRAG(bb, mp, 1); aq[mp + 1][1] = G2_AFRAG(bb, mp + 1, 1);              \
            aq[mp][0] = G2_AFRAG(bb, mp, 0); aq[mp + 1][0] = G2_AFRAG(bb, mp + 1, 0);              \
        }                                                                                          \
        __builtin_amdgcn_sched_barrier(0);                                                         \
    }
#define G2_MF(mt_, q_)                                                                             \
    if constexpr (NOMFMA) { asm volatile("" :: "v"(aq[mt_][q_]), "v"(bq[0]), "v"(bq[1]), "v"(bq[2]), "v"(bq[3])); } \
    else if (G2_LIVE(mt_)) {                                                                       \
        _Pragma("unroll") for (int nt = 0; nt < 4; ++nt)                                           \
            acc[mt_][nt] = __builtin_amdgcn_mfma_f32_16x16x32_f16(aq[mt_][q_], bq[nt], acc[mt_][nt], 0, 0, 0); \
    }
#define G2_MF8(ma_, mb_, q_) G2_MF(ma_, q_) G2_MF(mb_, q_)
#define G2_STEP(MORE_)                                                                             \
    {                                                                                              \
        if constexpr (!NOBAR) G3_RAW_BARRIER()                   \
        if (BURST && MORE_) G2_ISSUE(s + AHEAD)                                                    \
        if constexpr (NOREAD) { if (s == 0) { G2_READ_A(s) G2_READ_B(s) } } else { G2_READ_A(s) }  \
        G2_MF8(0, 1, 1)                                                                            \
        if (!BURST && MORE_) G2_PIECE(s + AHEAD, 0)                                                \
        G2_MF8(0, 1, 0)                                                                            \
        if constexpr (!NOREAD) { G2_READ_B(s) }                                                    \
        if (!BURST && MORE_) G2_PIECE(s + AHEAD, 1)                                                \
        G2_MF8(2, 3, 1)                                                                            \
        if (!BURST && MORE_) G2_PIECE(s + AHEAD, 2)                                                \
        G2_MF8(2, 3, 0)                                                                            \
        asm volatile("s_waitcnt lgkmcnt(0)" ::: "memory");       \
         \
        if (s + 1 < nst) { if (MORE_) { if constexpr (BURST) G3_WAIT_VM(6); else G3_WAIT_VM(3); } else G3_WAIT_VM(0); } \
        if constexpr (!NOBAR) G3_RAW_BARRIER()                                            \
        G2_MF8(4, 5, 1)                                                                            \
        if (!BURST && MORE_) G2_PIECE(s + AHEAD, 3)                                                \
        G2_MF8(4, 5, 0)                                                                            \
        if (!BURST && MORE_) G2_PIECE(s + AHEAD, 4)                                                \
        G2_MF8(6, 7, 1)                                                                            \
        if (!BURST && MORE_) G2_PIECE(s + AHEAD, 5)                                                \
        G2_MF8(6, 7, 0)                                                                            \
    }

    f16x8 bq[4], aq[8][2];
    G3_WAIT_VM(0);
    G2_ISSUE(0)
    if (nst > 1) G2_ISSUE(1)
    if (nst > 1) G3_WAIT_VM(6); else G3_WAIT_VM(0);
    if (grp == 1) G3_RAW_BARRIER()
    {
        int s = 0;
        const int n_main = NODMA ? 0 : nst - AHEAD;
        for (; s < n_main; ++s) G2_STEP(true)
        for (; s < nst; ++s) G2_STEP(false)
    }
    if (grp == 0) G3_RAW_BARRIER()
#undef G2_STEP
#undef G2_MF8
#undef G2_MF
#undef G2_READ_B
#undef G2_READ_A
#undef G2_AFRAG
#undef G2_FRAG
#undef G2_ISSUE
#undef G2_PIECE

    if (C == nullptr) return;
#pragma unroll
    for (int mt = 0; mt < 8; ++mt) {
        if (!G2_LIVE(mt)) continue;
        const int row0 = m0 + grp * 128 + mt * 16 + 4 * g;
#pragma unroll
        for (int i = 0; i < 4; ++i) {
            const float rs = rscale[row0 + i];
#pragma unroll
            for (int nt = 0; nt < 4; ++nt)
                C[(size_t)(row0 + i) * ldc + j0 + wn * 64 + nt * 16 + r] = acc[mt][nt][i] * rs;
        }
    }
#undef G2_LIVE
}

template <bool HI, int VAR, bool NTB, bool PART, bool GEN>
__device__ __forceinline__ void gemm2h_segment(G2Sub<1>, const unsigned char* __restrict__ A2, const unsigned char* __restrict__ B1,
                                                   const unsigned char* __restrict__ Bhi,
                                                   const unsigned int* __restrict__ hiflag,
                                                   const float* __restrict__ rscale,
                                                   int Kb, float* __restrict__ C, int ldc, int m0, int j0, int kb0,
                                                   int nkb, unsigned char* smem, const float* __restrict__ cscale,
                                                   unsigned live)
{
    static_assert(VAR == 0 || VAR == 4, "the 32x32x16 body has the burst and the spread stream only");
    using GEO = G2Geom<1, HI>;
    constexpr int IMGS = GEO::IMGS, IMG = GEO::IMG, OFF_B = GEO::OFF_B, AHEAD = GEO::AHEAD;
    static_assert(IMGS == 4 && GEO::NA == 2 && GEO::NB == 1, "four images, pieces A0 A1 B (Bhi)");
    const int tid = threadIdx.x;
    const int lane = tid & 63, wave = tid >> 6;
    const int grp = wave >> 2, wn = wave & 3;
    const int li = lane & 31, h = lane >> 5;
    const int nst = nkb;
    const unsigned lv = g2_wave_live<PART>(live, grp);
#define G2_LIVE(m_) (!PART || ((lv >> (m_)) & 1u))

    const size_t jblk = ((size_t)(j0 / G3C_JW) * Kb + kb0);
    const unsigned char* abase = A2 + ((size_t)(m0 / G3_MW) * Kb + kb0) * G2_A + tid * 16;
    const unsigned char* bbase = B1 + jblk * G2_B + tid * 16;
    const unsigned char* hbase = HI ? Bhi + jblk * G2_B + tid * 16 : nullptr;
    unsigned int fw[5] = {0u, 0u, 0u, 0u, 0u};
    if (HI) {
        const int KW = (Kb + 31) >> 5, w0 = kb0 >> 5;
        const unsigned int* fr = hiflag + (size_t)(j0 / G3C_JW) * KW;
#pragma unroll
        for (int w = 0; w < 5; ++w)
            fw[w] = (nkb > 129) ? 0xFFFFFFFFu : ((w0 + w < KW) ? __builtin_amdgcn_readfirstlane(fr[w0 + w]) : 0u);
    }
    const int fbit0 = kb0 & 31;

    f32x16_3 acc[4][2];
#pragma unroll
    for (int m = 0; m < 4; ++m)
#pragma unroll
        for (int n = 0; n < 2; ++n)
#pragma unroll
            for (int r = 0; r < 16; ++r) acc[m][n][r] = 0.f;

    const int a_row = (grp * 128 + li) * G2_ROWB;
    const int a_s0 = ((0 + h) ^ ((li >> 2) & 3)) * 16, a_s1 = ((2 + h) ^ ((li >> 2) & 3)) * 16;
    const int b_off = OFF_B + (wn * 64 + li) * 32 + (h ^ ((li >> 3) & 1)) * 16;

#define G2_BLKFLAG(b_) (HI && ((fw[(fbit0 + (b_)) >> 5 > 4 ? 4 : (fbit0 + (b_)) >> 5] >> ((fbit0 + (b_)) & 31)) & 1u))
#define G2_ISSUE(s_)                                                                               \
    {                                                                                              \
        unsigned char* d_ = smem + ((s_) % IMGS) * IMG + wave * 1024;                              \
        const unsigned char* a_ = abase + (size_t)(s_) * G2_A;                                     \
        _Pragma("unroll") for (int i = 0; i < 2; ++i)                                              \
            __builtin_amdgcn_global_load_lds(G3_AS1(a_ + i * 8192), G3_AS3(d_ + i * 8192), 16, 0, 0); \
        __builtin_amdgcn_global_load_lds(G3_AS1(bbase + (size_t)(s_) * G2_B), G3_AS3(d_ + OFF_B), 16, 0, NTB ? 2 : 0); \
        if (HI) {                                                                                  \
            if (G2_BLKFLAG(s_))                                                                    \
                __builtin_amdgcn_global_load_lds(G3_AS1(hbase + (size_t)(s_) * G2_B), G3_AS3(d_ + GEO::OFF_H), 16, 0, NTB ? 2 : 0); \
        }                                                                                          \
    }
#define G2_PIECE(s_, i_) { G2_DMA_PIECE(1, HI, NTB, s_, i_) __builtin_amdgcn_sched_barrier(0); }
#define G2_FRAG(ptr_) __builtin_bit_cast(f16x8, *reinterpret_cast<const u32x4*>(ptr_))
#define G2_MFMA(b_, m_, q_)                                                                        \
    if (G2_LIVE(m_)) {                                                                             \
    acc[m_][0] = __builtin_amdgcn_mfma_f32_32x32x16_f16(aq[m_][q_], b_[0], acc[m_][0], 0, 0, 0);   \
    acc[m_][1] = __builtin_amdgcn_mfma_f32_32x32x16_f16(aq[m_][q_], b_[1], acc[m_][1], 0, 0, 0); }
#define G2_WAIT_AHEAD(cnt_)                                                                        \
    {                                                                                              \
        if constexpr ((cnt_) == 1) G3_WAIT_VM(3);                                                  \
        else if constexpr ((cnt_) == 2) G3_WAIT_VM(6);                                             \
        else G3_WAIT_VM(0);                                                                        \
    }

    f16x8 bq[2], bh[2], aq[4][2];
    constexpr bool SPREAD = VAR == 4 && (!HI || GEN);
    G3_WAIT_VM(0);
    G2_ISSUE(0)
    if (nst > 1) G2_ISSUE(1)
    if (nst > 2) G2_ISSUE(2)
    if (nst > 2) G2_WAIT_AHEAD(2) else if (nst > 1) G2_WAIT_AHEAD(1) else G2_WAIT_AHEAD(0)
    if (grp == 1) G3_RAW_BARRIER()
    if constexpr (SPREAD) {
#define G2_READ_A(s_)                                                                              \
        {                                                                                          \
            const unsigned char* bb = smem + ((s_) % IMGS) * IMG;                                  \
            _Pragma("unroll") for (int n = 0; n < 2; ++n) bq[n] = G2_FRAG(bb + b_off + n * 32 * 32); \
            _Pragma("unroll") for (int m = 0; m < 2; ++m) {                                        \
                aq[m][1] = G2_FRAG(bb + a_row + m * 32 * G2_ROWB + a_s1);                          \
                aq[m][0] = G2_FRAG(bb + a_row + m * 32 * G2_ROWB + a_s0);                          \
            }                                                                                      \
            if constexpr (HI) { _Pragma("unroll") for (int n = 0; n < 2; ++n) bh[n] = G2_FRAG(bb + b_off + G2_B + n * 32 * 32); } \
            __builtin_amdgcn_sched_barrier(0);                                                     \
        }
#define G2_READ_B(s_)                                                                              \
        {                                                                                          \
            const unsigned char* bb = smem + ((s_) % IMGS) * IMG;                                  \
            _Pragma("unroll") for (int m = 2; m < 4; ++m) {                                        \
                aq[m][1] = G2_FRAG(bb + a_row + m * 32 * G2_ROWB + a_s1);                          \
                aq[m][0] = G2_FRAG(bb + a_row + m * 32 * G2_ROWB + a_s0);                          \
            }                                                                                      \
            __builtin_amdgcn_sched_barrier(0);                                                     \
        }
#define G2_STEP(MORE_)                                                                             \
        {                                                                                          \
            G3_RAW_BARRIER()                                         \
            G2_READ_A(s)                                                                           \
            G2_MFMA(bq, 0, 1) G2_MFMA(bq, 1, 1)                                                    \
            if (MORE_) G2_PIECE(s + AHEAD, 0)                                                      \
            G2_MFMA(bq, 0, 0) G2_MFMA(bq, 1, 0)                                                    \
            G2_READ_B(s)                                                                           \
            if (MORE_) G2_PIECE(s + AHEAD, 1)                                                      \
            if constexpr (HI) { G2_MFMA(bh, 0, 0) G2_MFMA(bh, 1, 0) }                              \
            asm volatile("s_waitcnt lgkmcnt(0)" ::: "memory");                                     \
             \
            if (s + 1 < nst) { if (MORE_) { if constexpr (HI) G3_WAIT_VM(6); else G3_WAIT_VM(5); } else G3_WAIT_VM(0); } \
            G3_RAW_BARRIER()                                                              \
            G2_MFMA(bq, 2, 1) G2_MFMA(bq, 3, 1)                                                    \
            if (MORE_) G2_PIECE(s + AHEAD, 2)                                                      \
            G2_MFMA(bq, 2, 0) G2_MFMA(bq, 3, 0)                                                    \
            if constexpr (HI) { if (MORE_) G2_PIECE(s + AHEAD, 3)                                  \
                                G2_MFMA(bh, 2, 0) G2_MFMA(bh, 3, 0) }                              \
        }
        {
            int s = 0;
            const int n_main = nst - AHEAD;
            for (; s < n_main; ++s) G2_STEP(true)
            for (; s < nst; ++s) G2_STEP(false)
        }
#undef G2_STEP
#undef G2_READ_B
#undef G2_READ_A
    } else {
#define G2_READ(s_)                                                                                \
        {                                                                                          \
            const unsigned char* bb = smem + ((s_) % IMGS) * IMG;                                  \
            _Pragma("unroll") for (int n = 0; n < 2; ++n) bq[n] = G2_FRAG(bb + b_off + n * 32 * 32); \
            if (HI) { _Pragma("unroll") for (int n = 0; n < 2; ++n) bh[n] = G2_FRAG(bb + b_off + G2_B + n * 32 * 32); } \
            _Pragma("unroll") for (int m = 0; m < 4; ++m) {                                        \
                aq[m][0] = G2_FRAG(bb + a_row + m * 32 * G2_ROWB + a_s0);                          \
                aq[m][1] = G2_FRAG(bb + a_row + m * 32 * G2_ROWB + a_s1);                          \
            }                                                                                      \
            __builtin_amdgcn_sched_barrier(0);                                                     \
        }
#define G2_MFMA4(b_, ma_, mb_) G2_MFMA(b_, ma_, 1) G2_MFMA(b_, mb_, 1) G2_MFMA(b_, ma_, 0) G2_MFMA(b_, mb_, 0)
#define G2_MFMA2H(b_, ma_, mb_) G2_MFMA(b_, ma_, 0) G2_MFMA(b_, mb_, 0)
#define G2_HALF(ma_, mb_)                                                                          \
        {                                                                                          \
            G2_MFMA4(bq, ma_, mb_)                                                                 \
            if (HI) { if (hi_blk) { if constexpr (GEN) { G2_MFMA2H(bh, ma_, mb_) } else { G2_MFMA4(bh, ma_, mb_) } } } \
        }
        for (int s = 0; s < nst; ++s) {
            const bool hi_blk = G2_BLKFLAG(s);
            G3_RAW_BARRIER()
            if (s + AHEAD < nst) G2_ISSUE(s + AHEAD)
            G2_READ(s)
            G2_HALF(0, 1)
            asm volatile("s_waitcnt lgkmcnt(0)" ::: "memory");
            if (s + 1 < nst) {
                if (s + 3 < nst) G2_WAIT_AHEAD(2) else if (s + 2 < nst) G2_WAIT_AHEAD(1) else G2_WAIT_AHEAD(0)
            }
            G3_RAW_BARRIER()
            G2_HALF(2, 3)
        }
#undef G2_HALF
#undef G2_MFMA2H
#undef G2_MFMA4
#undef G2_READ
    }
    if (grp == 0) G3_RAW_BARRIER()
#undef G2_WAIT_AHEAD
#undef G2_MFMA
#undef G2_FRAG
#undef G2_PIECE
#undef G2_ISSUE
#undef G2_BLKFLAG

    if (C == nullptr) return;
    const int j = j0 + wn * 64 + li;
    const float cs[2] = {(HI && cscale) ? cscale[j] : 1.0f, (HI && cscale) ? cscale[j + 32] : 1.0f};
#pragma unroll
    for (int m = 0; m < 4; ++m) {
        if (!G2_LIVE(m)) continue;
        const int cbase = m0 + grp * 128 + m * 32 + 4 * h;
#pragma unroll
        for (int n = 0; n < 2; ++n)
#pragma unroll
            for (int r = 0; r < 16; ++r) {
                const int row = cbase + (r & 3) + 8 * (r >> 2);
                C[(size_t)row * ldc + j + n * 32] = (acc[m][n][r] * rscale[row]) * cs[n];
            }
    }
#undef G2_LIVE
}

template <bool HI, int VAR, bool NTB, bool PART, bool GEN>
__device__ __forceinline__ void gemm2h_segment(G2Sub<2>, const unsigned char* __restrict__ A2, const unsigned char* __restrict__ B1,
                                               const unsigned char* __restrict__, const unsigned int* __restrict__,
                                               const float* __restrict__ rscale, int Kb, float* __restrict__ C, int ldc,
                                               int m0, int j0, int kb0, int nkb, unsigned char* smem, const float* __restrict__,
                                               unsigned live)
{
    static_assert(!HI && !GEN, "two blocks per step: one count plane only");
    gemm2h_segment_mf16<VAR, NTB, PART>(A2, B1, rscale, Kb, C, ldc, m0, j0, kb0, nkb, smem, live);
}

template <int NSUB, bool HI, int VAR = 0, bool PART = false, bool GEN = false>
__global__ __launch_bounds__(512) void gemm2h_kernel(const unsigned char* __restrict__ A2,
                                                     const unsigned char* __restrict__ B1,
                                                     const unsigned char* __restrict__ Bhi,
                                                     const unsigned int* __restrict__ hiflag,
                                                     const float* __restrict__ rscale, int Kb,
                                                     float* __restrict__ C, int ldc, long long c_split_stride,
                                                     int kb_per, const float* __restrict__ cscale = nullptr,
                                                     unsigned long long livemask = ~0ull)
{
    extern __shared__ __attribute__((aligned(16))) unsigned char smem3[];
    int jt = blockIdx.x, mg = blockIdx.y, z = blockIdx.z;
    if ((gridDim.z & 7) == 0) {
        const int L = blockIdx.x + (int)gridDim.x * (blockIdx.y + (int)gridDim.y * blockIdx.z);
        const int xcd = L & 7, idx = L >> 3;
        jt = idx % (int)gridDim.x;
        mg = (idx / (int)gridDim.x) % (int)gridDim.y;
        z = xcd + 8 * (idx / (int)(gridDim.x * gridDim.y));
    }
    const int kb0 = z * kb_per;
    const int nkb = min(kb_per, Kb - kb0);
    gemm2h_segment<HI, VAR, true, PART, GEN>(G2Sub<NSUB>{}, A2, B1, Bhi, hiflag, rscale, Kb, C ? C + (size_t)z * c_split_stride : nullptr, ldc, mg * G3_MW,
                                                   jt * G3C_JW, kb0, nkb, smem3, cscale, (unsigned)((livemask >> (8 * mg)) & 0xffu));
}

template <int NSUB, bool HI, int VAR = 0, bool NTB = true, bool PART = false, bool GEN = false>
__global__ __launch_bounds__(512) void gemm2h_streamk_kernel(const unsigned char* __restrict__ A2,
                                                             const unsigned char* __restrict__ B1,
                                                             const unsigned char* __restrict__ Bhi,
                                                             const unsigned int* __restrict__ hiflag,
                                                             const float* __restrict__ rscale, int Kb,
                                                             float* __restrict__ C0, float* __restrict__ C1,
                                                             float* __restrict__ C2, int ldc, int MG, int T, int xmap,
                                                             const float* __restrict__ cscale = nullptr,
                                                             unsigned long long livemask = ~0ull)
{
    extern __shared__ __attribute__((aligned(16))) unsigned char smem3[];
    const int Ks = Kb / NSUB;
    const long long U = (long long)T * Ks;
    const int P = (int)gridDim.x;
    const int q = (xmap && MG > 1 && P % MG == 0) ? ((int)blockIdx.x % MG) * (P / MG) + (int)blockIdx.x / MG : (int)blockIdx.x;
    long long u = U * q / P;
    const long long u1 = U * (q + 1) / P;
    const int NJ = T / MG;
    while (u < u1) {
        const int tile = (int)(u / Ks), ks = (int)(u % Ks);
        const int ke = (int)min((long long)Ks, ks + (u1 - u));
        const int mg = tile / NJ, jt = tile % NJ;
        gemm2h_segment<HI, VAR, NTB, PART, GEN>(G2Sub<NSUB>{}, A2, B1, Bhi, hiflag, rscale, Kb, (ks == 0) ? C0 : (ke == Ks ? C1 : C2), ldc, mg * G3_MW,
                                                      jt * G3C_JW, ks * NSUB, (ke - ks) * NSUB, smem3, cscale,
                                                      (unsigned)((livemask >> (8 * mg)) & 0xffu));
        u += ke - ks;
        G3_WAIT_VM(0);
        __syncthreads();
    }
}

}
```

### cnmf_amd/csrc/kernels_planes.hip.h

```cpp
#pragma once
#include <hip/hip_runtime.h>
#include "kernels_gemm3.hip.h"

namespace cnmf {

constexpr float G2_COUNT_BASE = 2048.0f;

__device__ __forceinline__ unsigned short f16_bits(float x)
{
    const _Float16 h = (_Float16)x;
    return __builtin_bit_cast(unsigned short, h);
}
__device__ __forceinline__ float f16_to_f32(unsigned short b) { return (float)__builtin_bit_cast(_Float16, b); }

__device__ __forceinline__ int g2_row_shift(float mx)
{
    if (!(mx > 0.f)) return 0;
    int e;
    frexpf(mx, &e);
    const int s = 15 - e;
    return s > 120 ? 120 : (s < -110 ? -110 : s);
}

__device__ __forceinline__ void split2h(float y, unsigned short& h, unsigned short& m)
{
    h = f16_bits(y);
    m = f16_bits(y - f16_to_f32(h));
}

template <int BASE>
__device__ __forceinline__ void count_lo_hi(float n, float& lo, float& hi)
{
    if (n <= (float)BASE) { lo = n; hi = 0.f; }
    else { hi = floorf(n * (1.0f / (float)BASE)); lo = n - (float)BASE * hi; hi *= (float)BASE; }
}

template <int BASE>
struct CountFormat {
    using Aux = float;
    static constexpr bool FLAGGED = true;
    static __device__ __forceinline__ float value(const float* __restrict__ X, size_t at, bool inside,
                                                  const float* __restrict__ unit, int , int gene)
    {
        if (!inside) return 0.f;
        const float u = unit[gene];
        return u > 0.f ? rintf(X[at] / u) : 0.f;
    }
};
struct CountBf16 : CountFormat<256> {
    static constexpr bool SWIZZLE = false;
    static __device__ __forceinline__ void pair(float n, unsigned short& a, unsigned short& b)
    {
        float lo, hi;
        count_lo_hi<256>(n, lo, hi);
        a = bf16_rne(lo); b = bf16_rne(hi);
    }
};
struct CountF16 : CountFormat<(int)G2_COUNT_BASE> {
    static constexpr bool SWIZZLE = true;
    static __device__ __forceinline__ void pair(float n, unsigned short& a, unsigned short& b)
    {
        float lo, hi;
        count_lo_hi<(int)G2_COUNT_BASE>(n, lo, hi);
        a = f16_bits(lo); b = f16_bits(hi);
    }
};
struct SplitF16 {
    using Aux = int;
    static constexpr bool SWIZZLE = true, FLAGGED = false;
    static __device__ __forceinline__ float value(const float* __restrict__ X, size_t at, bool inside,
                                                  const int* __restrict__ shift, int row, int )
    {
        return ldexpf(inside ? X[at] : 0.f, shift[row]);
    }
    static __device__ __forceinline__ void pair(float y, unsigned short& h, unsigned short& m) { split2h(y, h, m); }
};

__device__ __forceinline__ void store_plane_row(unsigned short* d, const unsigned short* p, int swz)
{
#pragma unroll
    for (int hf = 0; hf < 2; ++hf) {
        u32x4 w;
        w.x = p[8 * hf + 0] | ((unsigned)p[8 * hf + 1] << 16); w.y = p[8 * hf + 2] | ((unsigned)p[8 * hf + 3] << 16);
        w.z = p[8 * hf + 4] | ((unsigned)p[8 * hf + 5] << 16); w.w = p[8 * hf + 6] | ((unsigned)p[8 * hf + 7] << 16);
        *reinterpret_cast<u32x4*>(d + (hf ^ swz) * 8) = w;
    }
}

template <class F, bool TRANSPOSE>
__global__ __launch_bounds__(256) void x_planes_kernel(const float* __restrict__ X, int ld, int N, int G, int rows_pad,
                                                       int K, int TR, const typename F::Aux* __restrict__ aux,
                                                       unsigned short* __restrict__ plane0,
                                                       unsigned short* __restrict__ plane1,
                                                       unsigned int* __restrict__ flags)
{
    const int Kb = K / 16;
    int row, kb;
    if constexpr (TRANSPOSE) {
        row = blockIdx.y * 256 + threadIdx.x;
        kb = blockIdx.x;
        if (row >= rows_pad) return;
    } else {
        const long long t = (long long)blockIdx.x * 256 + threadIdx.x;
        if (t >= (long long)rows_pad * Kb) return;
        row = (int)(t / Kb);
        kb = (int)(t % Kb);
    }
    unsigned short p0[16], p1[16];
    bool any1 = false;
#pragma unroll
    for (int i = 0; i < 16; ++i) {
        const int k = kb * 16 + i;
        const int cell = TRANSPOSE ? k : row, gene = TRANSPOSE ? row : k;
        const float v = F::value(X, (size_t)cell * ld + gene, cell < N && gene < G, aux, row, gene);
        F::pair(v, p0[i], p1[i]);
        any1 |= p1[i] != 0;
    }
    const int rin = row % TR, swz = F::SWIZZLE ? (rin >> 3) & 1 : 0;
    const size_t at = (((size_t)(row / TR) * Kb + kb) * TR + rin) * 16;
    store_plane_row(plane0 + at, p0, swz);
    if (plane1) {
        store_plane_row(plane1 + at, p1, swz);
        if (F::FLAGGED && any1) atomicOr(&flags[(size_t)(row / TR) * ((Kb + 31) / 32) + (kb >> 5)], 1u << (kb & 31));
    }
}

__global__ __launch_bounds__(256) void count_max_base_kernel(const float* __restrict__ X, int ld, int N, int G,
                                                             const float* __restrict__ unit, float base,
                                                             unsigned* __restrict__ any_big)
{
    const int g = blockIdx.x * 256 + threadIdx.x;
    if (g >= G) return;
    const float u = unit[g];
    if (u <= 0.f) return;
    const int r0 = blockIdx.y * 256, r1 = min(N, r0 + 256);
    bool big = false;
    for (int r = r0; r < r1; ++r) big |= rintf(X[(size_t)r * ld + g] / u) > base;
    if (big) atomicOr(any_big, 1u);
}

__global__ __launch_bounds__(256) void x2h_rowshift_kernel(const float* __restrict__ X, int ld, int N, int G,
                                                           int transpose, int rows_pad, int* __restrict__ shift,
                                                           float* __restrict__ inv_scale)
{
    if (!transpose) {
        const int row = blockIdx.x * 4 + (threadIdx.x >> 6), lane = threadIdx.x & 63;
        if (row >= rows_pad) return;
        float mx = 0.f;
        if (row < N) for (int g = lane; g < G; g += 64) mx = fmaxf(mx, X[(size_t)row * ld + g]);
#pragma unroll
        for (int o = 32; o > 0; o >>= 1) mx = fmaxf(mx, __shfl_xor(mx, o, 64));
        if (lane == 0) { const int s = g2_row_shift(mx); shift[row] = s; inv_scale[row] = ldexpf(1.0f, -s); }
    } else {
        const int g = blockIdx.x * 256 + threadIdx.x;
        if (g >= rows_pad) return;
        float mx = 0.f;
        if (g < G) for (int r = 0; r < N; ++r) mx = fmaxf(mx, X[(size_t)r * ld + g]);
        const int s = g2_row_shift(mx);
        shift[g] = s; inv_scale[g] = ldexpf(1.0f, -s);
    }
}

struct SplitFused { const int* shift_in; int* shift_out; };
template <int TROWS, int TKB>
__device__ __forceinline__ void split2h_tiled_body(const float* __restrict__ src, int ld, int K, int TR,
                                                   unsigned short* __restrict__ dst, const double* __restrict__ kscale,
                                                   const float* __restrict__ rmax_part, int parts,
                                                   float* __restrict__ inv_scale, int bx, int nbx, int by,
                                                   unsigned short* tile_, float* red_, SplitFused fu = SplitFused{nullptr, nullptr})
{
    static_assert(TROWS * TKB == 256, "tile = 256 (row, block) pairs");
    constexpr int NQ = 256 / TROWS;
    constexpr int KQ = TKB * 4;
    constexpr int RPP = 256 / KQ;
    unsigned short (*tile)[TROWS][32] = reinterpret_cast<unsigned short (*)[TROWS][32]>(tile_);
    float (*red)[TROWS] = reinterpret_cast<float (*)[TROWS]>(red_);
    const int t = threadIdx.x;
    const int r0 = by * TROWS;
    const int kq = t % KQ, rr = t / KQ;
    const int ntiles = K / (16 * TKB);
    const bool fused = fu.shift_in != nullptr;
    float4 v[4];
    if (!fused) {
        const int k0 = bx * 16 * TKB;
#pragma unroll
        for (int i = 0; i < 4; ++i)
            v[i] = *reinterpret_cast<const float4*>(src + (size_t)(r0 + rr + RPP * i) * ld + k0 + kq * 4);
    }
    {
        const int row = t % TROWS, qt = t / TROWS;
        float mx = 0.f;
        for (int p0 = qt; p0 < parts; p0 += 8 * NQ) {
            float v[8];
#pragma unroll
            for (int j = 0; j < 8; ++j) v[j] = (p0 + j * NQ < parts) ? rmax_part[(size_t)(r0 + row) * parts + p0 + j * NQ] : 0.f;
#pragma unroll
            for (int j = 0; j < 8; ++j) mx = fmaxf(mx, v[j]);
        }
        red[qt][row] = mx;
    }
    __syncthreads();
    int sh[4];
    bool redo = false;
#pragma unroll
    for (int i = 0; i < 4; ++i) {
        const int row = rr + RPP * i;
        float mx = 0.f;
#pragma unroll
        for (int q = 0; q < NQ; ++q) mx = fmaxf(mx, red[q][row]);
        sh[i] = g2_row_shift(mx);
        if (fused) {
            const int su = fu.shift_in[r0 + row];
            const float ymax = ldexpf(mx, su);
            const bool ok = !(mx > 0.f) || (ymax < 60000.0f && ymax >= 1024.0f);
            const bool keep = !(mx > 0.f) || (ymax < 46340.0f && ymax >= 8192.0f);
            if (bx == 0 && kq == 0) fu.shift_out[r0 + row] = (ok && keep) ? su : sh[i];
            if (ok) sh[i] = su; else redo = true;
        }
        if (bx == 0 && kq == 0) inv_scale[r0 + row] = ldexpf(1.0f, -sh[i]);
    }
    if (fused) {
        if (!__syncthreads_or(redo ? 1 : 0)) return;
        const int k0 = bx * 16 * TKB;
#pragma unroll
        for (int i = 0; i < 4; ++i)
            v[i] = *reinterpret_cast<const float4*>(src + (size_t)(r0 + rr + RPP * i) * ld + k0 + kq * 4);
    }
    __syncthreads();
    const int Kb = K / 16;
    const int tr = r0 / TR, rin = r0 % TR;
    for (int kt = bx; kt < ntiles; kt += nbx) {
        const int k0 = kt * 16 * TKB;
        float4 vn[4];
        const bool has_next = kt + nbx < ntiles;
        if (has_next) {
#pragma unroll
            for (int i = 0; i < 4; ++i)
                vn[i] = *reinterpret_cast<const float4*>(src + (size_t)(r0 + rr + RPP * i) * ld + (k0 + nbx * 16 * TKB) + kq * 4);
        }
#pragma unroll
        for (int i = 0; i < 4; ++i) {
            const int row = rr + RPP * i;
            float x[4] = {v[i].x, v[i].y, v[i].z, v[i].w};
            if (kscale) {
#pragma unroll
                for (int e = 0; e < 4; ++e) x[e] = (float)((double)x[e] * kscale[k0 + kq * 4 + e]);
            }
            unsigned short p[2][4];
#pragma unroll
            for (int e = 0; e < 4; ++e) split2h(ldexpf(x[e], sh[i]), p[0][e], p[1][e]);
            const int hf = (kq >> 1) & 1, swz = (row >> 2) & 3;
#pragma unroll
            for (int q = 0; q < 2; ++q) {
                uint2 w;
                w.x = p[q][0] | ((unsigned)p[q][1] << 16); w.y = p[q][2] | ((unsigned)p[q][3] << 16);
                *reinterpret_cast<uint2*>(&tile[kq >> 2][row][((2 * q + hf) ^ swz) * 8 + (kq & 1) * 4]) = w;
            }
        }
        __syncthreads();
#pragma unroll
        for (int pass = 0; pass < 4; ++pass) {
            const int c = pass * 256 + t;
            const int b = c / (TROWS * 4), within = c % (TROWS * 4);
            unsigned short* g = dst + (((size_t)tr * Kb + (k0 / 16 + b)) * TR + rin) * 32;
            reinterpret_cast<u32x4*>(g)[within] = reinterpret_cast<const u32x4*>(&tile[b][0][0])[within];
        }
        __syncthreads();
        if (has_next) {
#pragma unroll
// ... 37 lines not shown
```

### cnmf_amd/csrc/pass_plan.h

```cpp
#pragma once

#include <algorithm>
#include <cstdint>
#include <vector>

constexpr int PLAN_BK = 32, PLAN_G3_MW = 256, PLAN_G3_JW = 128, PLAN_G3C_JW = 256, PLAN_G3_BK = 16, PLAN_KSMALL = 64;

struct PadShape { int N_pad, G_pad; };

static inline int plan_round_up(int64_t v, int m) { return (int)(((v + m - 1) / m) * m); }

constexpr int PLAN_GRID_YZ = 65535;

static inline bool x_launches_fit(PadShape s, int gemm3)
{
    if (gemm3 <= 0) return true;
    const bool whole = s.N_pad % PLAN_G3C_JW == 0 && s.G_pad % PLAN_G3C_JW == 0;
    const bool detects = gemm3 >= 3 && whole;
    const bool bf16_planes = gemm3 <= 3 || !whole;
    if ((s.G_pad + 255) / 256 > PLAN_GRID_YZ) return false;
    if (detects && (s.N_pad + 255) / 256 > PLAN_GRID_YZ) return false;
    if (bf16_planes && s.N_pad % 64 == 0 && s.G_pad % 64 == 0 && s.N_pad / 64 > PLAN_GRID_YZ) return false;
    return true;
}

static inline int sweep_chunks(int parts_knob, int L) { const int64_t m = 256ll * parts_knob; return std::max(1, (int)(((int64_t)L + m - 1) / m)); }
static inline int sweep_parts(int parts_knob, int L) { const int c = sweep_chunks(parts_knob, L); return (L + 256 * c - 1) / (256 * c); }

enum class SweepForm { W, W_A64, W_PLN, W_PLN_A64, H_RMX, H_PSUM, INVALID };

static inline bool sweep_a64(int ldv) { return 64ll * ldv * 4 > 0x7fffffffll; }

static inline SweepForm sweep_form(bool has_planes_out, bool psum, bool exact_rmax, bool a64, int tiers = 7)
{
    if (has_planes_out) {
        if (psum || exact_rmax || (tiers & 8)) return SweepForm::INVALID;
        return a64 ? SweepForm::W_PLN_A64 : SweepForm::W_PLN;
    }
    if (psum) return (tiers & 8) ? SweepForm::INVALID : SweepForm::H_PSUM;
    if (exact_rmax) return SweepForm::H_RMX;
    return a64 ? SweepForm::W_A64 : SweepForm::W;
}

static inline int pick_nsplit(PadShape s, int KC)
{
    const int jt = (s.G_pad + 127) / 128;
    const int mg = std::max(1, KC / 128);
    int n = std::max(1, 512 / (jt * mg));
    const int max_by_k = std::max(1, s.N_pad / 256);
    return std::min(n, max_by_k);
}

static inline int effective_splits(int Ktot, int nsplit)
{
    const int Kper = plan_round_up((Ktot + nsplit - 1) / nsplit, PLAN_BK);
    return (Ktot + Kper - 1) / Kper;
}

static inline int pick_nsplit_A(PadShape s, int KC)
{
    const int T = (s.N_pad / 128) * std::max(1, KC / 128);
    if (T > 256) return 1;
    int n = std::max(1, 512 / T);
    n = std::min(n, std::max(1, s.G_pad / (4 * PLAN_BK)));
    return effective_splits(s.G_pad, std::min(n, 16));
}

static inline int gemm3_wg_slots(int gemm3, int wg_slots_knob)
{
    if (wg_slots_knob >= 32 && gemm3 >= 2) return wg_slots_knob;
    return gemm3 >= 2 ? 256 : 512;
}

static inline int pick_nsplit_A3(PadShape s, int KC, int jw, int wg_slots)
{
    const int T = std::max(1, s.N_pad / jw) * std::max(1, KC / PLAN_G3_MW);
    const int Kb = s.G_pad / PLAN_G3_BK;
    int n = std::max(1, std::min(wg_slots / T, Kb / 8));
    const int kb_per = (Kb + n - 1) / n;
    return (Kb + kb_per - 1) / kb_per;
}

static inline int pick_nsplit3(PadShape s, int KC, int jw, int wg_slots)
{
    const int tiles = std::max(1, s.G_pad / jw) * std::max(1, KC / PLAN_G3_MW);
    const int Kb = s.N_pad / PLAN_G3_BK;
    int n = std::max(1, std::min(wg_slots / std::max(1, tiles), Kb / 16));
    const int kb_per = (Kb + n - 1) / n;
    return (Kb + kb_per - 1) / kb_per;
}

struct SplitCaps { int nsplit, nsplitA; };
static inline SplitCaps size_splits(PadShape s, int KC, bool use3, int wg_slots)
{
    SplitCaps c{pick_nsplit(s, KC), pick_nsplit_A(s, KC)};
    if (use3) {
        c.nsplit = std::max(c.nsplit, std::max(pick_nsplit3(s, KC, PLAN_G3_JW, wg_slots), pick_nsplit3(s, KC, PLAN_G3C_JW, wg_slots)));
        c.nsplitA = std::max(c.nsplitA, std::max(pick_nsplit_A3(s, KC, PLAN_G3_JW, wg_slots), pick_nsplit_A3(s, KC, PLAN_G3C_JW, wg_slots)));
    }
    return c;
}

struct StreamK {
    bool on = false;
    int MG = 1, T = 0, nk = 0, P = 0, mw = 128;
    std::vector<unsigned char> split;
};

static inline StreamK plan_streamk(int KC, PadShape s, int n_wg_slots, bool no_streamk)
{
    StreamK sk;
    if (KC % 128 != 0 || no_streamk) return sk;
    sk.MG = KC / sk.mw;
    sk.T = sk.MG * (s.N_pad / 128);
    sk.nk = s.G_pad / PLAN_BK;
    sk.P = n_wg_slots;
    if (sk.T <= sk.P) sk.P = n_wg_slots / 2;
    if (sk.T <= sk.P || sk.T % sk.P == 0) return sk;
    sk.on = true;
    sk.split.assign(sk.T, 0);
    const long long U = (long long)sk.T * sk.nk;
    for (int p = 1; p < sk.P; ++p) {
        const long long b = U * p / sk.P;
        if (b % sk.nk) sk.split[b / sk.nk] = 1;
    }
    return sk;
}

struct StreamK3 {
    bool on = false;
    int T = 0, Kb = 0, P = 0, MG = 1;
    std::vector<unsigned char> flags;
};

static inline StreamK3 plan_streamk3(int KC, PadShape s, int n_wg_slots, int jw, int unit, bool no_streamk)
{
    StreamK3 sk;
    sk.MG = KC / PLAN_G3_MW;
    sk.T = sk.MG * (s.N_pad / jw);
    sk.Kb = s.G_pad / (PLAN_G3_BK * unit);
    sk.P = n_wg_slots;
    if (sk.T < sk.P / 2 + sk.P / 4 || sk.P > 2 * sk.T || no_streamk) return sk;
    sk.on = true;
    sk.flags.assign(sk.T, 0);
    const long long U = (long long)sk.T * sk.Kb;
    const int NJ = sk.T / sk.MG;
    for (int p = 1; p < sk.P; ++p) {
        const long long b = U * p / sk.P;
        if (b % sk.Kb) {
            const int o = (int)(b / sk.Kb);
            unsigned char& f = sk.flags[(o % NJ) * sk.MG + o / NJ];
            f = f ? 3 : 1;
        }
    }
    return sk;
}

static inline unsigned long long g2_full_mask(int KC) { const int t = KC / 32; return t >= 64 ? ~0ull : ((1ull << t) - 1ull); }

static inline int gemm2h_splits(int Kb, int nsplit, int nsub)
{
    int kb_per = (Kb + nsplit - 1) / nsplit;
    kb_per = ((kb_per + nsub - 1) / nsub) * nsub;
    return (Kb + kb_per - 1) / kb_per;
}

static inline int gemm2h_nsub(bool hi, int Kb, int nsub_knob) { return (!hi && nsub_knob == 2 && Kb % 2 == 0) ? 2 : 1; }

struct G2Form {
    bool valid; int NSUB; bool HI; int VAR; bool NTB, PART, GEN;
    bool operator==(const G2Form& o) const { return valid == o.valid && NSUB == o.NSUB && HI == o.HI && VAR == o.VAR && NTB == o.NTB && PART == o.PART && GEN == o.GEN; }
};

static inline G2Form g2_form(bool hi, bool gen, bool gen4, int gvar, int nsub, bool part, bool shared)
{
    if (gen && !hi) return G2Form{false, 1, false, 0, false, false, false};
    const bool ntb = !part && !shared;
    if (hi && gen && !gen4) return G2Form{true, 1, true, gvar == 0 ? 0 : 4, ntb, part, true};
    if (hi) return G2Form{true, 1, true, 0, ntb, part, false};
    if (nsub == 2) return G2Form{true, 2, false, 4, ntb, part, false};
    return G2Form{true, 1, false, 4, !shared, false, false};
}

static inline int g2_xmap(const G2Form& f, int xmap_knob) { return xmap_knob >= 0 ? xmap_knob : (f.GEN ? 0 : 1); }

static inline bool split2h_wide(int K) { return K % 256 == 0; }
static inline int split2h_col_groups(int K, int rows)
{
    const int tk = split2h_wide(K) ? 256 : 64, trows = split2h_wide(K) ? 16 : 64;
    const int tiles = K / tk, rg = std::max(1, rows / trows);
    const int cap = std::max(1, (256 * 7) / rg);
    int per = (tiles + cap - 1) / cap;
    return (tiles + per - 1) / per;
}

struct PassPlan {
    int nsplit = 1, nsplit3 = 1, nsplitA = 1;
    StreamK sk;
    StreamK3 sk3;
};

static inline void plan_pass_splits(PassPlan& p, PadShape s, int KC, bool use3, int jwA, int nsubA, int wg_slots, bool no_streamk,
                                    int cap, int capA)
{
    if (use3) {
        p.nsplit3 = std::max(1, std::min(pick_nsplit3(s, KC, jwA, wg_slots), cap));
        p.sk3 = plan_streamk3(KC, s, wg_slots, jwA, nsubA, no_streamk);
        if (!p.sk3.on) p.nsplitA = std::max(1, std::min(pick_nsplit_A3(s, KC, jwA, wg_slots), capA));
    } else {
        p.nsplit = std::max(1, std::min(pick_nsplit(s, KC), cap));
        p.sk = plan_streamk(KC, s, 2 * 256, no_streamk);
        if (p.sk.on) p.nsplitA = 1;
        else p.nsplitA = std::max(1, std::min(pick_nsplit_A(s, KC), capA));
    }
}

static inline int pick_kc(int kc_knob, int kc_limit, int64_t total_k, int max_k, int kc_max, bool wide_ok)
{
    if (kc_knob >= 32) kc_max = kc_knob;
    const bool autosize = kc_max <= 0;
    if (autosize) kc_max = 256;
    kc_max = std::max(32, std::min(kc_limit, (kc_max / 32) * 32));
    if (kc_max > 256) kc_max = wide_ok ? (kc_max / 256) * 256 : 256;
    int kc = 32;
    while (kc < std::min(kc_max, 256) && kc < total_k) kc *= 2;
    kc = std::min(kc, kc_max);
    if (wide_ok && kc == 256 && total_k > 256) {
        if (autosize) kc = (int)std::min<int64_t>(kc_limit, plan_round_up(total_k, 256));
        else if (!autosize && kc_max > 256) kc = (int)std::min<int64_t>(kc_max, plan_round_up(total_k, 256));
    }
    if (kc < max_k) kc = plan_round_up(max_k, 32);
    return kc;
}
```

### cnmf_amd/csrc/runtime.hip.h

```cpp
#pragma once

#include <map>
static thread_local std::string g_last_error;

struct cnmf_comm;

struct Arena {
    struct Block { char* p; size_t cap, used; };
    std::vector<Block> blocks;
    hipError_t err = hipSuccess;
    static constexpr size_t keep_limit = (size_t)2 << 30;
    void reset() { err = hipSuccess; for (Block& b : blocks) b.used = 0; }
    size_t total() const { size_t t = 0; for (const Block& b : blocks) t += b.cap; return t; }
    void release() { for (Block& b : blocks) hipFree(b.p); blocks.clear(); }
    template <typename T> T* get(size_t n, bool zero = false, hipStream_t st = nullptr) {
        const size_t bytes = (std::max<size_t>(n, 1) * sizeof(T) + 255) & ~(size_t)255;
        Block* hit = nullptr;
        for (Block& b : blocks) if (b.cap - b.used >= bytes) { hit = &b; break; }
        if (!hit) {
            void* p = nullptr;
            const size_t cap = std::max(bytes, (size_t)16 << 20);
            hipError_t e = hipMalloc(&p, cap);
            if (e != hipSuccess) { err = e; return nullptr; }
            blocks.push_back(Block{(char*)p, cap, 0});
            hit = &blocks.back();
        }
        T* out = (T*)(hit->p + hit->used);
        hit->used += bytes;
        if (zero) hipMemsetAsync(out, 0, bytes, st);
        return out;
    }
};

template <typename F>
struct Owned : F {
    Owned() = default;
    Owned(const Owned&) = delete;
    Owned& operator=(const Owned&) = delete;
    void release() { this->free_all(); static_cast<F&>(*this) = F{}; }
    void take(Owned& s) { release(); static_cast<F&>(*this) = s; static_cast<F&>(s) = F{}; }
};
template <typename F>
struct OwnedLocal : Owned<F> {
    ~OwnedLocal() { this->release(); }
};

template <typename V>
struct CsrF {
    int64_t rows = 0, cols = 0, nnz = -1;
    long long* ptr = nullptr; int* idx = nullptr; V* val = nullptr;
    void free_all() { hipFree(ptr); hipFree(idx); hipFree(val); }
    hipError_t alloc_ptr(int64_t r, int64_t c) {
        rows = r; cols = c;
        return hipMalloc((void**)&ptr, ((size_t)r + 1) * sizeof(long long));
    }
    hipError_t alloc_entries(long long n) {
        const size_t n1 = (size_t)std::max<long long>(n, 1);
        hipError_t e = hipMalloc((void**)&idx, n1 * sizeof(int));
        if (e == hipSuccess) e = hipMalloc((void**)&val, n1 * sizeof(V));
        if (e == hipSuccess) nnz = n;
        return e;
    }
};
template <typename V> using DevCsr = Owned<CsrF<V>>;
template <typename V> using DevCsrLocal = OwnedLocal<CsrF<V>>;

struct SpImageF {
    int R = 0, C = 0, BS = 0, nblk = 0, nslice = 0;
    int* perm = nullptr; long long* off = nullptr; int* len = nullptr; void* ent = nullptr;
    size_t n_ent = 0;
    void free_all() { hipFree(perm); hipFree(off); hipFree(len); hipFree(ent); }
};
using SpImage = Owned<SpImageF>;
struct DenseTF {
    float* p = nullptr;
    void free_all() { hipFree(p); }
};

struct XOperand { const unsigned char *plane, *hi; const unsigned int* flags; const float* colscale; };

struct Bf16PlanesF {
    unsigned char *X3 = nullptr, *Xt3 = nullptr;
    int tr = 0;
    void free_all() { hipFree(X3); hipFree(Xt3); }
};

struct CountPlanesF {
    int state = 0;
    int fmt = 0;
    unsigned char *C1 = nullptr, *Ct1 = nullptr;
    unsigned char *C1h = nullptr, *Ct1h = nullptr;
    unsigned int *hiA = nullptr, *hiB = nullptr;
    double* d_scale = nullptr;
    void free_all() { hipFree(C1); hipFree(Ct1); hipFree(C1h); hipFree(Ct1h); hipFree(hiA); hipFree(hiB); hipFree(d_scale); }
    XOperand passA() const { return {C1, C1h, hiA, nullptr}; }
    XOperand passB() const { return {Ct1, Ct1h, hiB, nullptr}; }
};

struct GeneralPlanesF {
    unsigned char *X2h = nullptr, *X2m = nullptr, *Xt2h = nullptr, *Xt2m = nullptr;
    float *sA = nullptr, *sB = nullptr;
    unsigned int *onesA = nullptr, *onesB = nullptr;
    void free_all() { hipFree(X2h); hipFree(X2m); hipFree(Xt2h); hipFree(Xt2m); hipFree(sA); hipFree(sB); hipFree(onesA); hipFree(onesB); }
    XOperand passA() const { return {X2h, X2m, onesA, sA}; }
    XOperand passB() const { return {Xt2h, Xt2m, onesB, sB}; }
};

struct CountStage {
    DevCsr<double> counts, columns;
    bool staged() const { return counts.nnz >= 0; }
    void release_counts() { counts.release(); columns.release(); }
};

struct PrepStage : CountStage {
    DevCsr<double> out;
    double* odense = nullptr;
    int out_dense = 0;
    void release_out() { out.release(); hipFree(odense); odense = nullptr; }
    void release() { release_counts(); release_out(); }
};

struct PreSlot {
    int64_t n = 0;
    DevCsr<double> csr;
    double* dense = nullptr;
    bool empty() const { return !dense && csr.nnz < 0; }
    void release() { csr.release(); hipFree(dense); dense = nullptr; n = 0; }
};

struct PreStage : CountStage {
    int64_t N = 0;
    PreSlot slot[2];
    double *Rt = nullptr, *Pt = nullptr;
    int K = 0, B1 = 0;
    void release_ridge() { hipFree(Rt); hipFree(Pt); Rt = Pt = nullptr; K = B1 = 0; }
    DevCsr<double> grouped;
    int* gstart = nullptr;
    std::vector<int32_t> gcodes;
    int gB = 0;
    void release_grouped() { grouped.release(); hipFree(gstart); gstart = nullptr; gcodes.clear(); gB = 0; }
    double *triA = nullptr, *triR = nullptr, *tri_tau = nullptr, *tri_mu = nullptr;
    double *tri_d = nullptr, *tri_e = nullptr;
    int tri_n = 0, tri_slot = -1;
    void release_tridiag() {
        hipFree(triA); hipFree(triR); hipFree(tri_tau); hipFree(tri_mu); hipFree(tri_d); hipFree(tri_e);
        triA = triR = tri_tau = tri_mu = tri_d = tri_e = nullptr; tri_n = 0; tri_slot = -1;
    }
    void release() {
        release_counts(); release_ridge(); release_grouped(); release_tridiag();
        slot[0].release(); slot[1].release(); N = 0;
    }
};

struct HarStage {
    int N = 0, Np = 0, d = 0, K = 0, V = 0, B = 0;
    bool ready = false;
    double *Zo = nullptr, *Zcos = nullptr, *Zcorr = nullptr;
    double *R = nullptr, *dist = nullptr, *S = nullptr;
    double *ZoT = nullptr, *ZcT = nullptr, *Rt = nullptr, *Pt = nullptr;
    double *Y = nullptr, *theta = nullptr, *sigma = nullptr, *prb = nullptr;
    double *E = nullptr, *O = nullptr, *tab = nullptr, *obj = nullptr;
    double *ypart = nullptr, *opart = nullptr, *part_old = nullptr, *part_new = nullptr;
    size_t part_old_cap = 0, part_new_cap = 0;
    int *codes = nullptr, *lvar = nullptr, *perm = nullptr;
    void release() {
        void* all[] = {Zo, Zcos, Zcorr, R, dist, S, ZoT, ZcT, Rt, Pt, Y, theta, sigma, prb, E, O, tab, obj, ypart, opart,
                       part_old, part_new, codes, lvar, perm};
        for (void* p : all) hipFree(p);
        *this = HarStage{};
    }
};

struct BatchBuffersF {
    int kc = 0, nsplit = 0, nsplitA = 0, parts = 0;
    size_t gram_part_floats = 0;
    float *H = nullptr, *Wt = nullptr, *XHt = nullptr, *XHt1 = nullptr, *XHt2 = nullptr, *XtW = nullptr;
    unsigned char *H3 = nullptr, *Wt3 = nullptr;
    unsigned char* d_split = nullptr;
    float *rmaxH = nullptr, *rmaxW = nullptr, *iscaleH = nullptr, *iscaleW = nullptr;
    int* shiftW = nullptr;
    float *gramH = nullptr, *gramW = nullptr, *gram_part = nullptr;
    double* viol_part = nullptr;
    SlotDesc* d_slots = nullptr;
    int* d_slot_list = nullptr;
    SlotDesc* h_slots = nullptr;
    SlotDesc* h_snap = nullptr;
    int* h_slot_list = nullptr;
    void free_all() {
        void* dev[] = {H, Wt, XHt, XHt1, XHt2, XtW, H3, Wt3, d_split, rmaxH, rmaxW, iscaleH, iscaleW, shiftW, gramH, gramW,
                       gram_part, viol_part, d_slots, d_slot_list};
        for (void* p : dev) hipFree(p);
        if (h_slots) hipHostFree(h_slots);
        if (h_snap) hipHostFree(h_snap);
        if (h_slot_list) hipHostFree(h_slot_list);
    }
};

static constexpr int RING = 8;
#ifndef CNMF_GEMM3_DEFAULT
#define CNMF_GEMM3_DEFAULT 4
#endif

struct CdKnobs {
    int  gemm3 = CNMF_GEMM3_DEFAULT;
    int  g2_gvar = 4;
    bool g2_gen4 = false;
    int  g2_nsub = 2;
    int  g2_xmap = -1;
    bool part = false;
    bool no_psum = false;
    bool wide_small = true;
    bool kc_set = false;
    int  kc = 0;
    int  kc_limit = 1024;
    int  lag = 0;
    int  sweep_parts = 64;
    int  wg_slots = 0;
    bool no_streamk = false;
    bool s_mtw2 = false;
    bool no_counts = false;
    bool debug = false;
};
struct MuKnobs {
    bool valu = false;
    int  sparse = -1;
    bool sp_order = true;
    bool debug = false;
};

struct cnmf_ctx {
    int device = 0;
    hipStream_t stream = nullptr;
    std::string err;
    std::map<std::string, std::string> env;
    CdKnobs knobs;
    MuKnobs mu_knobs;

    int64_t N = 0, G = 0;
    int N_pad = 0, G_pad = 0;
    float* X = nullptr;
    bool count_detect = true;
    Owned<Bf16PlanesF> planes;
    Owned<CountPlanesF> counts;
    Owned<GeneralPlanesF> x2;
    Owned<DenseTF> XtF;
    SpImage spA[2], spB[2];
    long long x_nnz = -1;
    DevCsr<float> csr, csc;

    Owned<BatchBuffersF> bat;
    float *stageW = nullptr, *stageH = nullptr;
    size_t stageW_sz = 0, stageH_sz = 0;

    float* spectra = nullptr;
    size_t spectra_cap = 0, spectra_rows = 0;
    int64_t spectra_G = 0;
    struct InitStore {
        float *H = nullptr, *Wt = nullptr;
        size_t cap_rows = 0, rows = 0;
        int64_t N = 0, G = 0;
        std::vector<int> k;
        std::vector<float> maxW;
        void release() { hipFree(H); hipFree(Wt); H = Wt = nullptr; cap_rows = rows = 0; N = G = 0; k.clear(); maxW.clear(); }
    } inits;
    std::vector<double> iter_prior, iter_hint;

    Arena cons_ws;
    void* cons_pinned = nullptr;
    size_t cons_pinned_bytes = 0;
    double clustergram_ms[5] = {0, 0, 0, 0, 0};
    double teig_ms[5] = {0, 0, 0, 0, 0};

    cnmf_comm* comm = nullptr;

    PrepStage prep;
    PreStage pre;
    HarStage har;
};

static const char* ctx_getenv(const cnmf_ctx* ctx, const char* name)
{
    if (!ctx) return getenv(name);
    auto it = ctx->env.find(name);
    return it == ctx->env.end() ? nullptr : it->second.c_str();
}
static void parse_cd_knobs(cnmf_ctx* ctx)
{
    CdKnobs k;
    auto num = [](const char* s, int dflt) { return s ? atoi(s) : dflt; };
    k.gemm3 = num(ctx_getenv(ctx, "CNMF_GEMM3"), CNMF_GEMM3_DEFAULT);
    if (k.gemm3 < 0 || k.gemm3 > 4) k.gemm3 = CNMF_GEMM3_DEFAULT;
    k.g2_gvar = num(ctx_getenv(ctx, "CNMF_G2_GVAR"), 4) == 0 ? 0 : 4;
    k.g2_gen4 = ctx_getenv(ctx, "CNMF_G2_GEN4") != nullptr;
    k.g2_nsub = num(ctx_getenv(ctx, "CNMF_G2_NSUB"), 2) == 1 ? 1 : 2;
    k.g2_xmap = num(ctx_getenv(ctx, "CNMF_G2_XMAP"), -1);
    k.part = ctx_getenv(ctx, "CNMF_PART") != nullptr;
    k.no_psum = ctx_getenv(ctx, "CNMF_NO_PSUM") != nullptr;
    k.wide_small = num(ctx_getenv(ctx, "CNMF_WIDE_SMALL"), 1) != 0;
    k.kc_set = ctx_getenv(ctx, "CNMF_KC") != nullptr;
    k.kc = num(ctx_getenv(ctx, "CNMF_KC"), 0);
    k.kc_limit = std::max(256, std::min(2048, (num(ctx_getenv(ctx, "CNMF_KC_LIMIT"), 1024) / 256) * 256));
    k.lag = num(ctx_getenv(ctx, "CNMF_LAG"), 0);
    k.sweep_parts = std::max(1, num(ctx_getenv(ctx, "CNMF_SWEEP_PARTS"), 64));
    k.wg_slots = num(ctx_getenv(ctx, "CNMF_WG_SLOTS"), 0);
    k.no_streamk = ctx_getenv(ctx, "CNMF_NO_STREAMK") != nullptr;
    k.s_mtw2 = ctx_getenv(ctx, "CNMF_S_MTW2") != nullptr;
    k.no_counts = ctx_getenv(ctx, "CNMF_NO_COUNTS") != nullptr;
    k.debug = ctx_getenv(ctx, "CNMF_DEBUG") != nullptr;
    ctx->knobs = k;
}
static void parse_mu_knobs(cnmf_ctx* ctx)
{
    MuKnobs m;
    auto num = [](const char* s, int dflt) { return s ? atoi(s) : dflt; };
    m.valu = num(ctx_getenv(ctx, "CNMF_MU_VALU"), 0) != 0;
    const int sp = num(ctx_getenv(ctx, "CNMF_MU_SPARSE"), -1);
    m.sparse = sp == 0 || sp == 1 ? sp : -1;
    m.sp_order = num(ctx_getenv(ctx, "CNMF_SP_ORDER"), 1) != 0;
    m.debug = ctx_getenv(ctx, "CNMF_DEBUG") != nullptr;
    ctx->mu_knobs = m;
}

extern char** environ;
static void ctx_snapshot_env(cnmf_ctx* ctx)
{
    ctx->env.clear();
    for (char** e = environ; e && *e; ++e) {
        if (strncmp(*e, "CNMF_", 5) != 0) continue;
        const char* eq = strchr(*e, '=');
        if (eq) ctx->env[std::string(*e, eq - *e)] = std::string(eq + 1);
    }
    parse_cd_knobs(ctx);
    parse_mu_knobs(ctx);
}

#define SET_ERR(ctx, ...)                                                   \
    do {                                                                    \
        char buf_[512];                                                     \
        snprintf(buf_, sizeof buf_, __VA_ARGS__);                           \
        if (ctx) (ctx)->err = buf_;                                         \
        g_last_error = buf_;                                                \
    } while (0)

#define HIP_TRY(ctx, call)                                                  \
    do {                                                                    \
        hipError_t e_ = (call);                                             \
        if (e_ != hipSuccess) {                                             \
            SET_ERR(ctx, "%s failed: %s (%s:%d)", #call, hipGetErrorString(e_), __FILE__, __LINE__); \
            return (e_ == hipErrorOutOfMemory) ? CNMF_ENOMEM : CNMF_EHIP;   \
        }                                                                   \
    } while (0)

struct DevPool {
    std::vector<void*> ptrs;
    hipError_t err = hipSuccess;
    template <typename T> T* get(size_t n, bool zero = false, hipStream_t st = nullptr) {
        void* p = nullptr;
        hipError_t e = hipMalloc(&p, std::max<size_t>(n, 1) * sizeof(T));
        if (e != hipSuccess) { err = e; return nullptr; }
        ptrs.push_back(p);
        if (zero) hipMemsetAsync(p, 0, std::max<size_t>(n, 1) * sizeof(T), st);
        return (T*)p;
    }
    template <typename T> T* put(const T* host, size_t n, hipStream_t st) {
        T* p = get<T>(n);
        if (p && n > 0) {
            hipError_t e = hipMemcpyAsync(p, host, n * sizeof(T), hipMemcpyHostToDevice, st);
            if (e != hipSuccess) err = e;
        }
        return p;
    }
    ~DevPool() { for (void* p : ptrs) hipFree(p); }
};

template <typename T>
static inline hipError_t dev_fetch(hipStream_t st, void* host, const T* dev, size_t n)
{
    return hipMemcpyAsync(host, dev, n * sizeof(T), hipMemcpyDeviceToHost, st);
}

struct EventPool {
    std::vector<hipEvent_t> evs;
    hipError_t err = hipSuccess;
    hipEvent_t get(unsigned flags = hipEventDefault) {
        hipEvent_t e = nullptr;
        hipError_t r = hipEventCreateWithFlags(&e, flags);
        if (r != hipSuccess) { err = r; return nullptr; }
        evs.push_back(e);
        return e;
    }
    ~EventPool() { for (hipEvent_t e : evs) hipEventDestroy(e); }
};

#define POOL_TRY(ctx, pool)                                                                   \
    do {                                                                                      \
        if ((pool).err != hipSuccess) {                                                       \
            SET_ERR(ctx, "device allocation failed: %s (%s:%d)", hipGetErrorString((pool).err), __FILE__, __LINE__); \
            return ((pool).err == hipErrorOutOfMemory) ? CNMF_ENOMEM : CNMF_EHIP;             \
        }                                                                                     \
    } while (0)

#include <mutex>
#include <set>
#include <utility>
static hipError_t dyn_lds_optin(const void* fn, int bytes)
{
    static std::mutex mu;
    static std::set<std::pair<const void*, int>> done;
    int dev = 0;
    hipError_t e = hipGetDevice(&dev);
    if (e != hipSuccess) return e;
    std::lock_guard<std::mutex> lk(mu);
    if (done.count({fn, dev})) return hipSuccess;
    e = hipFuncSetAttribute(fn, hipFuncAttributeMaxDynamicSharedMemorySize, bytes);
    if (e == hipSuccess) done.insert({fn, dev});
    return e;
}

static inline int round_up(int64_t v, int m) { return (int)(((v + m - 1) / m) * m); }
```

### cnmf_amd/engine.py

```python
import ctypes as C
import os
import warnings

import numpy as np

from . import _lib

_ERR = {-1: ValueError, -2: RuntimeError, -3: MemoryError, -4: RuntimeError,
        -5: NotImplementedError, -6: RuntimeError}


class ConvergenceWarning(UserWarning):
    """Mirror of sklearn.exceptions.ConvergenceWarning (sklearn _nmf.py:1727-1732)."""


def _fp(a):
    return a.ctypes.data_as(C.POINTER(C.c_float))


def regularization(n_samples, n_features, alpha_W=0.0, alpha_H=0.0, l1_ratio=0.0):
    return (n_features * alpha_W * l1_ratio, n_samples * alpha_H * l1_ratio,
            n_features * alpha_W * (1.0 - l1_ratio), n_samples * alpha_H * (1.0 - l1_ratio))


# ... 12 lines not shown
    WT, HR = (VT, UT) if transpose else (UT, VT)
    S = s[:k]
    W = np.zeros_like(WT)
    H = np.zeros_like(HR)
    W[0] = np.sqrt(S[0]) * np.abs(WT[0])
    H[0] = np.sqrt(S[0]) * np.abs(HR[0])
    for j in range(1, k):
        x, y = WT[j], HR[j]
        x_p, y_p = np.maximum(x, 0), np.maximum(y, 0)
        x_n, y_n = np.abs(np.minimum(x, 0)), np.abs(np.minimum(y, 0))
        x_p_nrm, y_p_nrm = np.sqrt(x_p @ x_p), np.sqrt(y_p @ y_p)
        x_n_nrm, y_n_nrm = np.sqrt(x_n @ x_n), np.sqrt(y_n @ y_n)
        m_p, m_n = x_p_nrm * y_p_nrm, x_n_nrm * y_n_nrm
        if m_p > m_n:
            u, v, sigma = x_p / x_p_nrm, y_p / y_p_nrm, m_p
        else:
            u, v, sigma = x_n / x_n_nrm, y_n / y_n_nrm, m_n
        lbd = np.sqrt(S[j] * sigma)
        W[j] = lbd * u
        H[j] = lbd * v
    W[W < eps] = 0
    H[H < eps] = 0
    return np.ascontiguousarray(W.T), H


NNDSVD_VARIANTS = ("nndsvd", "nndsvda", "nndsvdar")


def _nndsvd_fill(W, H, variant, x_mean, random_state):
    if variant == "nndsvda":
        W[W == 0] = x_mean
        H[H == 0] = x_mean
    elif variant == "nndsvdar":
        rng = random_state if isinstance(random_state, np.random.RandomState) else np.random.RandomState(random_state)
        W[W == 0] = abs(x_mean * rng.standard_normal(size=len(W[W == 0])) / 100)
        H[H == 0] = abs(x_mean * rng.standard_normal(size=len(H[H == 0])) / 100)
    elif variant != "nndsvd":
        raise ValueError("Invalid init parameter: got %r instead of one of %r" % (variant, NNDSVD_VARIANTS))
    return W, H


class Engine:
    def __init__(self, device=0, detect_counts=True):
        self._lib = _lib.load()
        if self._lib.cnmf_device_count() <= 0:
            raise RuntimeError("cnmf_amd: no HIP device visible -- the engine has no CPU fallback")
        self._ctx = self._lib.cnmf_create(int(device))
        if not self._ctx:
            raise RuntimeError("cnmf_create failed: %s" % self._lib.cnmf_last_error(None).decode())
        self.device = int(device)
        self._env_snap = self._env_now()
        self.shape = None
        self._x_mean, self._x_mean_src = None, None
        self.x_dtype = None
        self.x_has_zero = False
        self.last_stats = None
        self._prep = None
        self.store_gen = 0
        self.last_store_offsets = None
        self.last_store_gen = -1
        if not detect_counts:
            self.set_count_detection(False)

    def set_count_detection(self, enabled):
        self._check(self._lib.cnmf_set_count_detection(self._ctx, int(bool(enabled))))

    @staticmethod
    def _env_now():
        return tuple(sorted((k, v) for k, v in os.environ.items() if k.startswith("CNMF_")))

    def reload_env(self):
        self._check(self._lib.cnmf_reload_env(self._ctx))
        self._env_snap = self._env_now()

    def _sync_env(self):
        if self._env_now() != self._env_snap:
            self.reload_env()

    def close(self):
        if getattr(self, "_ctx", None):
            self._lib.cnmf_destroy(self._ctx)
            self._ctx = None

    def __del__(self):
        try:
            self.close()
        except Exception:
            pass

    def __enter__(self):
        return self

    def __exit__(self, *a):
        self.close()

    def _check(self, rc):
        if rc != 0:
            msg = self._lib.cnmf_last_error(self._ctx).decode()
            raise _ERR.get(rc, RuntimeError)("cnmf_hip: %s (code %d)" % (msg, rc))

    def _params(self, tol, max_iter, alpha_W, alpha_H, l1_ratio, kc_max=0, lag=0, profile=0, n_features=None):
        self._sync_env()
        N, G = self.shape
        l1W, l1H, l2W, l2H = regularization(N, G if n_features is None else int(n_features), alpha_W, alpha_H, l1_ratio)
        return _lib.CdParams(float(tol), int(max_iter), int(kc_max), l1W, l2W, l1H, l2H, int(lag), int(profile))

    def set_matrix(self, X):
        import scipy.sparse as sp
        if sp.issparse(X):
            X = X.tocsr()
            if not X.has_canonical_format:
                X = X.copy()
                X.sum_duplicates()
            data = X.data
            if not np.isfinite(data).all():
                raise ValueError("Input X contains NaN or infinity.")
            if data.size and data.min() < 0:
                raise ValueError("Negative values in data passed to NMF (input X)")
            self.x_dtype = np.dtype(X.dtype) if X.dtype in (np.float32, np.float64) else np.dtype(np.float64)
            self._x_mean, self._x_mean_src = None, X
            self.x_has_zero = bool(X.nnz < X.shape[0] * X.shape[1] or (data.size and data.min() == 0))
            vals = np.ascontiguousarray(data, dtype=np.float32)
            if vals.size and not vals.all():
                Xc = sp.csr_matrix((vals, X.indices.copy(), X.indptr.copy()), shape=X.shape)
                Xc.eliminate_zeros()
                X, vals = Xc, np.ascontiguousarray(Xc.data, dtype=np.float32)
            indptr = np.ascontiguousarray(X.indptr, dtype=np.int32)
            indices = np.ascontiguousarray(X.indices, dtype=np.int32)
            ip = C.POINTER(C.c_int32)
            self._check(self._lib.cnmf_set_matrix_csr(self._ctx, indptr.ctypes.data_as(ip),
                                                      indices.ctypes.data_as(ip), _fp(vals),
                                                      X.shape[0], X.shape[1]))
        else:
            X = np.asarray(X)
            if X.ndim != 2:
                raise ValueError("Expected 2D array, got %dD array instead" % X.ndim)
            if X.dtype not in (np.float32, np.float64):
                X = X.astype(np.float64)
            if not np.isfinite(X).all():
                raise ValueError("Input X contains NaN or infinity.")
            if X.size and X.min() < 0:
                raise ValueError("Negative values in data passed to NMF (input X)")
            self.x_dtype = X.dtype
            self.x_has_zero = bool(X.size and X.min() == 0)
            self.x_mean = X.mean()
            Xf = np.ascontiguousarray(X, dtype=np.float32)
            self._check(self._lib.cnmf_set_matrix(self._ctx, _fp(Xf), Xf.shape[0], Xf.shape[1]))
        self.shape = (int(X.shape[0]), int(X.shape[1]))
        return self

    def matrix_images(self):
        f = C.c_int32(0)
        self._check(self._lib.cnmf_matrix_images(self._ctx, C.byref(f)))
        names = ("dense", "csr", "csr_of_transpose", "dense_transpose", "non_zero_images_16", "non_zero_images_32", "count_planes")
        return {n: bool(f.value >> i & 1) for i, n in enumerate(names)}

    def get_matrix(self):
        if self.shape is None:
            raise RuntimeError("set_matrix() has not been called")
        out = np.empty(self.shape, dtype=np.float32)
        self._check(self._lib.cnmf_get_matrix(self._ctx, _fp(out)))
        return out

    def col_mean_var(self):
        if self.shape is None:
            raise RuntimeError("set_matrix() has not been called")
        N, G = self.shape
        dblp = C.POINTER(C.c_double)
        mean, ssd = np.empty(G), np.empty(G)
        self._check(self._lib.cnmf_col_moments(self._ctx, mean.ctypes.data_as(dblp), ssd.ctypes.data_as(dblp)))
        return mean, ssd / N

    def scale_genes_unit_variance(self):
        if self.shape is None:
            raise RuntimeError("set_matrix() has not been called")
        N, G = self.shape
        if N < 2:
            raise ValueError("need at least two cells for a variance")
        dblp = C.POINTER(C.c_double)
        mean, ssd = np.empty(G), np.empty(G)
        self._check(self._lib.cnmf_col_moments(self._ctx, mean.ctypes.data_as(dblp), ssd.ctypes.data_as(dblp)))
        std = np.sqrt(ssd / (N - 1))
        self._check(self._lib.cnmf_scale_columns(self._ctx, std.ctypes.data_as(dblp)))
        rs = np.empty(N)
        self._check(self._lib.cnmf_row_sums(self._ctx, rs.ctypes.data_as(dblp)))
        self.x_dtype = np.dtype(np.float64)
        self.x_mean = np.float64(rs.sum() / (float(N) * float(G)))
        return std, rs

    def prepare_upload(self, counts):
        import scipy.sparse as sp
        X = sp.csr_matrix(counts)
        if not X.has_canonical_format or (X.nnz and not X.data.all()):
            X = X.copy()
            X.sum_duplicates()
            X.eliminate_zeros()
        data = X.data
        if data.dtype == np.float32 or (data.dtype.kind in "iub" and (data.size == 0 or np.abs(data).max() < (1 << 24))):
            vals, f64 = np.ascontiguousarray(data, dtype=np.float32), 0
        else:
            vals, f64 = np.ascontiguousarray(data, dtype=np.float64), 1
        indptr = np.ascontiguousarray(X.indptr, dtype=np.int64)
        indices = np.ascontiguousarray(X.indices, dtype=np.int32)
        self._check(self._lib.cnmf_prepare_upload_csr(self._ctx, indptr.ctypes.data_as(C.POINTER(C.c_int64)),
                                                      indices.ctypes.data_as(C.POINTER(C.c_int32)),
                                                      vals.ctypes.data_as(C.c_void_p), f64, X.shape[0], X.shape[1]))
        self._prep = (X.shape, X.nnz)
        return X

    def prepare_tpm_stats(self, target_sum=1e6, want_tpm=False):
        (N, G), nnz = self._prep
        dblp = C.POINTER(C.c_double)
        rs, mean, var = np.empty(N), np.empty(G), np.empty(G)
        tpm = np.empty(max(nnz, 1)) if want_tpm else None
        self._check(self._lib.cnmf_prepare_tpm_stats(self._ctx, float(target_sum), rs.ctypes.data_as(dblp),
                                                     mean.ctypes.data_as(dblp), var.ctypes.data_as(dblp),
                                                     tpm.ctypes.data_as(dblp) if want_tpm else None))
        return rs, mean, var, (tpm[:nnz] if want_tpm else None)

    def prepare_select(self, genes, densify):
        import scipy.sparse as sp
        (N, G), _ = self._prep
        genes = np.ascontiguousarray(genes, dtype=np.int32)
        n = int(genes.size)
        dblp = C.POINTER(C.c_double)
        std, rs, nnz = np.empty(max(n, 1)), np.empty(N), C.c_int64(0)
        self._check(self._lib.cnmf_prepare_select(self._ctx, n, genes.ctypes.data_as(C.POINTER(C.c_int32)), int(bool(densify)),
                                                  std.ctypes.data_as(dblp), rs.ctypes.data_as(dblp), C.byref(nnz)))
        self.shape = (int(N), n)
        self.x_dtype = np.dtype(np.float64)
        if densify:
            Y = np.empty((N, n))
            self._check(self._lib.cnmf_prepare_fetch(self._ctx, None, None, Y.ctypes.data_as(dblp)))
            self.x_has_zero = bool(Y.size and Y.min() == 0)
            self.x_mean = Y.mean()
        else:
            nz = int(nnz.value)
            indptr, indices, data = np.empty(N + 1, dtype=np.int64), np.empty(max(nz, 1), dtype=np.int32), np.empty(max(nz, 1))
            self._check(self._lib.cnmf_prepare_fetch(self._ctx, indptr.ctypes.data_as(C.POINTER(C.c_int64)),
                                                     indices.ctypes.data_as(C.POINTER(C.c_int32)), data.ctypes.data_as(dblp)))
            if indptr[-1] < (1 << 31):
                indptr = indptr.astype(np.int32)
                Y = sp.csr_matrix((data[:nz], indices[:nz], indptr), shape=(N, n))
            else:
                Y = sp.csr_matrix((data[:nz], indices[:nz].astype(np.int64), indptr), shape=(N, n))
            Y.has_canonical_format = True
            self.x_has_zero = bool(nz < N * n)
            self._x_mean, self._x_mean_src = None, Y
        self._prep = None
        return std[:n], rs, Y

    def prepare_release(self):
        self._check(self._lib.cnmf_prepare_release(self._ctx))
        self._prep = None

    def preprocess_upload(self, counts):
        import scipy.sparse as sp
        X = sp.csr_matrix(counts)
        if not X.has_canonical_format or (X.nnz and not X.data.all()):
            X = X.copy()
            X.sum_duplicates()
            X.eliminate_zeros()
        vals = np.ascontiguousarray(X.data, dtype=np.float64)
        indptr = np.ascontiguousarray(X.indptr, dtype=np.int64)
        indices = np.ascontiguousarray(X.indices, dtype=np.int32)
        self._check(self._lib.cnmf_preprocess_upload_csr(self._ctx, indptr.ctypes.data_as(C.POINTER(C.c_int64)),
                                                         indices.ctypes.data_as(C.POINTER(C.c_int32)),
                                                         vals.ctypes.data_as(C.c_void_p), 1, X.shape[0], X.shape[1]))
        self._pre = {"N": X.shape[0], "G": X.shape[1], 0: None, 1: None}
        return X

    def preprocess_set_dense(self, slot, X):
        X = np.ascontiguousarray(X, dtype=np.float64)
        self._check(self._lib.cnmf_preprocess_set_dense(self._ctx, int(slot), X.ctypes.data_as(C.POINTER(C.c_double)),
                                                        X.shape[0], X.shape[1]))
        pre = getattr(self, "_pre", None) or {"N": X.shape[0], 0: None, 1: None}
        pre["N"], pre[int(slot)] = X.shape[0], (X.shape[1], -2)
        self._pre = pre

    def preprocess_select(self, slot, genes, target_sum=0.0, max_value=None):
        genes = np.ascontiguousarray(genes, dtype=np.int32)
        n = int(genes.size)
        std, nnz = np.empty(max(n, 1)), C.c_int64(0)
        mv = np.inf if max_value is None else float(max_value)
        self._check(self._lib.cnmf_preprocess_select(self._ctx, int(slot), n, genes.ctypes.data_as(C.POINTER(C.c_int32)),
                                                     float(target_sum), mv, std.ctypes.data_as(C.POINTER(C.c_double)),
                                                     C.byref(nnz)))
        self._pre[int(slot)] = (n, int(nnz.value))
        return std[:n]

    def preprocess_order_stats(self, slot, k):
        lo, hi = C.c_double(0), C.c_double(0)
        self._check(self._lib.cnmf_preprocess_order_stats(self._ctx, int(slot), int(k), C.byref(lo), C.byref(hi)))
        return np.float64(lo.value), np.float64(hi.value)

    def preprocess_ceiling(self, slot, thresh):
        self._check(self._lib.cnmf_preprocess_ceiling(self._ctx, int(slot), float(thresh)))

    def preprocess_densify(self, slot):
        self._check(self._lib.cnmf_preprocess_densify(self._ctx, int(slot)))
        self._pre[int(slot)] = (self._pre[int(slot)][0], -2)

    def preprocess_fetch(self, slot):
        import scipy.sparse as sp
        N = self._pre["N"]
        n, nnz = self._pre[int(slot)]
        dblp = C.POINTER(C.c_double)
# ... 1221 lines not shown
        R = int(lab.size)
        dblp, i32p = C.POINTER(C.c_double), C.POINTER(C.c_int32)
        if store_rows is not None:
            rows = np.ascontiguousarray(store_rows, dtype=np.int64).ravel()
            if rows.size != R:
                raise ValueError("labels must have one entry per store row")
            G, sp, rp = int(self.spectra_genes), None, rows.ctypes.data_as(C.POINTER(C.c_int64))
        else:
            S = np.ascontiguousarray(spectra, dtype=np.float64)
            if S.ndim != 2 or S.shape[0] != R:
                raise ValueError("spectra must be 2-D with one label per row")
            G, sp, rp = int(S.shape[1]), S.ctypes.data_as(dblp), None
        Rk = int((lab >= 0).sum())
        order = np.zeros(Rk, dtype=np.int32)
        seg = np.zeros(max(k, 0) + 1, dtype=np.int32)
        Z = np.zeros((max(Rk - k, 0), 4), dtype=np.float64) if return_linkage else None
        image = np.empty((Rk, Rk), dtype=np.float64) if return_image else None
        self._check(self._lib.cnmf_clustergram(self._ctx, sp, rp, R, G, lab.ctypes.data_as(i32p), k,
                                               order.ctypes.data_as(i32p),
                                               Z.ctypes.data_as(dblp) if Z is not None else None,
                                               seg.ctypes.data_as(i32p),
                                               image.ctypes.data_as(dblp) if image is not None else None))
        linkage = None
        if return_linkage:
            linkage = [Z[seg[c] - c:seg[c + 1] - c - 1].copy() for c in range(k)]
        return dict(spectra_order=order.astype(np.int64), segments=seg, topics_dist_ordered=image, linkage=linkage)

    def clustergram_step_ms(self):
        out = np.zeros(5, dtype=np.float64)
        self._check(self._lib.cnmf_clustergram_step_ms(self._ctx, out.ctypes.data_as(C.POINTER(C.c_double))))
        return dict(zip(("distances", "cluster_blocks", "linkage_and_order", "ordered_image", "download"), out.tolist()))

    def prediction_error(self, W, H):
        if self.shape is None:
            raise RuntimeError("set_matrix() has not been called")
        N, G = self.shape
        W = np.ascontiguousarray(W, dtype=np.float64)
        H = np.ascontiguousarray(H, dtype=np.float64)
        if W.shape[0] != N or H.shape[1] != G or W.shape[1] != H.shape[0]:
            raise ValueError("shape mismatch: W %s, H %s, X %s" % (W.shape, H.shape, (N, G)))
        err = C.c_double(0.0)
        dblp = C.POINTER(C.c_double)
        self._check(self._lib.cnmf_prediction_error(self._ctx, int(H.shape[0]), W.ctypes.data_as(dblp),
                                                    H.ctypes.data_as(dblp), C.byref(err)))
        return float(err.value)

    def comm_unique_id(self):
        buf = (C.c_ubyte * _lib.COMM_ID_BYTES)()
        self._check(self._lib.cnmf_comm_unique_id(buf))
        return bytes(buf)

    def comm_init(self, unique_id, rank, world):
        if len(unique_id) != _lib.COMM_ID_BYTES:
            raise ValueError("unique_id must be %d bytes" % _lib.COMM_ID_BYTES)
        buf = (C.c_ubyte * _lib.COMM_ID_BYTES).from_buffer_copy(unique_id)
        self._check(self._lib.cnmf_comm_init(self._ctx, buf, int(rank), int(world)))

    def comm_finalize(self):
        self._check(self._lib.cnmf_comm_finalize(self._ctx))

    @property
    def comm_rank(self):
        return int(self._lib.cnmf_comm_rank(self._ctx))

    @property
    def comm_world(self):
        return int(self._lib.cnmf_comm_world(self._ctx))

    def allgather_array(self, a):
        a = np.ascontiguousarray(a)
        out = np.empty((self.comm_world,) + a.shape, dtype=a.dtype)
        self._check(self._lib.cnmf_allgather_bytes(self._ctx, a.ctypes.data_as(C.c_void_p), a.nbytes,
                                                   out.ctypes.data_as(C.c_void_p)))
        return out

    def allgather_spectra(self, local, rows_max, n_genes=None):
        if local is None:
            rows, G = self.spectra_rows, (self.spectra_genes or self.shape[1])
            lp = None
        else:
            local = np.ascontiguousarray(local, dtype=np.float32)
            rows, G = (int(local.shape[0]), int(local.shape[1] if local.ndim == 2 else n_genes))
            lp = _fp(local) if rows else None
            if not rows:
                lp = _fp(np.zeros(1, np.float32))
        if n_genes is not None and int(n_genes) != G:
            raise ValueError("n_genes does not match the block")
        out = np.empty((self.comm_world, int(rows_max), G), dtype=np.float32)
        if rows_max:
            self._check(self._lib.cnmf_allgather_spectra(self._ctx, lp, rows, int(rows_max), G, _fp(out)))
        return out

    @property
    def spectra_rows(self):
        return int(self._lib.cnmf_spectra_rows(self._ctx))

    def spectra_reset(self):
        self._check(self._lib.cnmf_spectra_reset(self._ctx))
        self.store_gen += 1

    @property
    def spectra_genes(self):
        return int(self._lib.cnmf_spectra_genes(self._ctx))

    def spectra_append(self, rows):
        rows = np.ascontiguousarray(rows, dtype=np.float32)
        if rows.ndim != 2:
            raise ValueError("rows must be 2-D")
        first = self.spectra_rows
        self._check(self._lib.cnmf_spectra_append(self._ctx, _fp(rows), rows.shape[0], rows.shape[1]))
        return first

    def spectra_fetch(self, row0=0, rows=None):
        total = self.spectra_rows
        rows = total - int(row0) if rows is None else int(rows)
        out = np.empty((rows, self.spectra_genes if total else 0), dtype=np.float32)
        if out.size:
            self._check(self._lib.cnmf_spectra_fetch_rows(self._ctx, int(row0), rows, _fp(out)))
        return out

    def debug_gemm(self, mode, A, B, variant=0, nsplit=1, reps=0):
        A = np.ascontiguousarray(A, dtype=np.float32)
        B = np.ascontiguousarray(B, dtype=np.float32)
        KC, K = A.shape
        J = B.shape[0] if mode == 0 else B.shape[1]
        Cout = np.empty((KC, J), dtype=np.float32)
        ms = C.c_double(0.0)
        self._check(self._lib.cnmf_debug_gemm(self._ctx, mode, variant, _fp(A), _fp(B), _fp(Cout),
                                              KC, K, J, nsplit, C.byref(ms), reps))
        return Cout, ms.value

    def debug_gemm3(self, A, B, nsplit=1, reps=0):
        A = np.ascontiguousarray(A, dtype=np.float32)
        B = np.ascontiguousarray(B, dtype=np.float32)
        KC, K = A.shape
        J = B.shape[0]
        Cout = np.empty((KC, J), dtype=np.float32)
        ms = C.c_double(0.0)
        self._check(self._lib.cnmf_debug_gemm3(self._ctx, _fp(A), _fp(B), _fp(Cout), KC, K, J, int(nsplit),
                                               C.byref(ms), int(reps)))
        return Cout, ms.value

    def debug_gemm3c(self, A, Bn, nsplit=1, reps=0):
        A = np.ascontiguousarray(A, dtype=np.float32)
        Bn = np.ascontiguousarray(Bn, dtype=np.float32)
        KC, K = A.shape
        J = Bn.shape[0]
        Cout = np.empty((KC, J), dtype=np.float32)
        ms = C.c_double(0.0)
        self._check(self._lib.cnmf_debug_gemm3c(self._ctx, _fp(A), _fp(Bn), _fp(Cout), KC, K, J, int(nsplit),
                                                C.byref(ms), int(reps)))
        return Cout, ms.value

    def debug_gemm2h(self, A, Bn, nsplit=1, nsub=2, reps=0, sweep_bound=False):
        nsub = int(nsub) | (128 if sweep_bound else 0)
        A = np.ascontiguousarray(A, dtype=np.float32)
        Bn = np.ascontiguousarray(Bn, dtype=np.float32)
        KC, K = A.shape
        J = Bn.shape[0]
        Cout = np.empty((KC, J), dtype=np.float32)
        ms = C.c_double(0.0)
        self._check(self._lib.cnmf_debug_gemm2h(self._ctx, _fp(A), _fp(Bn), _fp(Cout), KC, K, J, int(nsplit),
                                                int(nsub), C.byref(ms), int(reps)))
        return Cout, ms.value

    def debug_mt_normals(self, state, n):
        st = _lib.MtState.from_numpy(state)
        out = np.empty(max(n, 1), dtype=np.float64)
        self._check(self._lib.cnmf_debug_mt_normals(self._ctx, C.byref(st), n, out.ctypes.data_as(C.POINTER(C.c_double))))
        return out[:n], st.to_numpy()

    def debug_standard_normal(self, seed, n):
        out = np.empty(max(n, 1), dtype=np.float64)
        self._check(self._lib.cnmf_debug_standard_normal(self._ctx, C.c_uint32(seed), n,
                                                         out.ctypes.data_as(C.POINTER(C.c_double))))
        return out[:n]
```

Baseline: 228.4.

## Store integer count planes as bytes when all counts fit in 255

Adds a byte-per-entry count plane format (COUNT_U8) for the X operand of the split-half GEMM, used when every count is at most 255. Halves the memory and LDS footprint of the X plane so the bandwidth-bound GEMM passes stream less data. The kernel now converts bytes to f16 inside the inner loop, and a second max-check pass runs at setup. It is on by default and can be turned off with an env knob.

New measurement: 231.3, median of 6. +1.3%, better.

```diff
diff --git a/cnmf_amd/csrc/batch_host.hip.h b/cnmf_amd/csrc/batch_host.hip.h
--- a/cnmf_amd/csrc/batch_host.hip.h
+++ b/cnmf_amd/csrc/batch_host.hip.h
@@ -145,7 +145,7 @@
     }
     p.use2g = p.use3 && !p.usec && kn.gemm3 >= 4 && ctx->G_pad % G3C_JW == 0 && ctx->N_pad % G3C_JW == 0;
     if (p.use2g && (rc = ensure_x2planes(ctx))) return rc;
-    p.use2h = (p.usec && ctx->counts.fmt == 4) || p.use2g;
+    p.use2h = (p.usec && ctx->counts.fmt >= 4) || p.use2g;
     p.mode = !p.use3 ? 0 : (p.use2g ? 5 : (p.usec ? (p.use2h ? 4 : 3) : std::min(kn.gemm3, 2)));
     p.KbA = ctx->G_pad / 16; p.KbB = ctx->N_pad / 16;
     p.xA = p.use2g ? ctx->x2.passA() : ctx->counts.passA();
diff --git a/cnmf_amd/csrc/cnmf_hip.hip b/cnmf_amd/csrc/cnmf_hip.hip
--- a/cnmf_amd/csrc/cnmf_hip.hip
+++ b/cnmf_amd/csrc/cnmf_hip.hip
@@ -241,7 +241,8 @@
 {
     if (!ctx || !flags) return CNMF_EINVAL;
     *flags = (ctx->X ? 1 : 0) | (ctx->csr.ptr ? 2 : 0) | (ctx->csc.ptr ? 4 : 0) | (ctx->XtF.p ? 8 : 0) |
-             ((ctx->spA[0].ent && ctx->spB[0].ent) ? 16 : 0) | ((ctx->spA[1].ent && ctx->spB[1].ent) ? 32 : 0) | (ctx->counts.C1 ? 64 : 0);
+             ((ctx->spA[0].ent && ctx->spB[0].ent) ? 16 : 0) | ((ctx->spA[1].ent && ctx->spB[1].ent) ? 32 : 0) | (ctx->counts.C1 ? 64 : 0) |
+             ((ctx->counts.C1 && ctx->counts.bytes) ? 128 : 0);
     return CNMF_OK;
 }
 
diff --git a/cnmf_amd/csrc/debug_host.hip.h b/cnmf_amd/csrc/debug_host.hip.h
--- a/cnmf_amd/csrc/debug_host.hip.h
+++ b/cnmf_amd/csrc/debug_host.hip.h
@@ -196,6 +196,7 @@
                                  int nsplit, int nsub, double* ms_out, int reps)
 {
     const bool sweep_bound = (nsub & 128) != 0;
+    const bool u8 = (nsub & 256) != 0;
     nsub &= 127;
     if (!ctx || !A || !Bn || !C) { SET_ERR(ctx, "null argument"); return CNMF_EINVAL; }
     if (KC % 256 || K % 64 || J < 1 || nsplit < 1) { SET_ERR(ctx, "debug_gemm2h needs KC %% 256 == 0, K %% 64 == 0"); return CNMF_EINVAL; }
@@ -204,6 +205,11 @@
     const int Jp = round_up(J, G3C_JW), Kb = K / 16;
     bool has_hi = false;
     for (size_t i = 0; i < (size_t)J * K && !has_hi; ++i) has_hi = Bn[i] > G2_COUNT_BASE;
+    if (u8) {
+        bool fits = (nsub & 15) == 2 && (((nsub >> 4) & 7) == 0 || ((nsub >> 4) & 7) == 4);
+        for (size_t i = 0; i < (size_t)J * K && fits; ++i) fits = Bn[i] <= 255.0f;
+        if (!fits) { SET_ERR(ctx, "debug_gemm2h: byte planes need nsub 2, stream 0 or 4 and counts <= 255"); return CNMF_EINVAL; }
+    }
     DevPool pool;
     EventPool events;
     float* dA = pool.get<float>((size_t)KC * K);
@@ -230,18 +236,20 @@
     } else
         HIP_TRY(ctx, launch_rowmax_part(st, dA, K, K, KC, K, nullptr, 1, dRmax));
     HIP_TRY(ctx, launch_split2h(st, dA, K, KC, K, dA2, G3_MW, nullptr, dRmax, bparts, dInv));
-    HIP_TRY(ctx, launch_x_planes(st, XPlaneFormat::COUNT_F16, false, dB, K, J, K, Jp, K, dUnit, dB1, dBh, dFl));
+    HIP_TRY(ctx, launch_x_planes(st, u8 ? XPlaneFormat::COUNT_U8 : XPlaneFormat::COUNT_F16, false, dB, K, J, K, Jp, K, dUnit, dB1, dBh, dFl));
     reps = std::max(1, reps);
     const int var = (nsub >> 4) & 7;
     nsub &= 15;
     const int ns = (!has_hi && nsub == 2 && Kb % 2 == 0) ? 2 : 1;
     G2Launch g;
-    g.A2 = dA2; g.rscale = dInv; g.x = XOperand{dB1, dBh, dFl, nullptr}; g.Kb = Kb;
+    g.A2 = dA2; g.rscale = dInv; g.x = XOperand{dB1, dBh, dFl, nullptr, u8}; g.Kb = Kb;
     g.C[0] = dC; g.ldc = Jp; g.cstride = (long long)KC * Jp; g.KC = KC; g.Jpad = Jp; g.nsplit = nsplit;
     for (int i = 0; i < reps + 1; ++i) {
         if (i == 1) hipEventRecord(e0, st);
         hipError_t e;
         if (has_hi) e = launch_gemm2h_t<1, true>(st, g);
+        else if (u8 && var == 4) e = launch_gemm2h_t<2, false, 4, false, false, true>(st, g);
+        else if (u8) e = launch_gemm2h_t<2, false, 0, false, false, true>(st, g);
         else if (ns == 2 && var == 2) e = launch_gemm2h_t<2, false, 2>(st, g);
         else if (ns == 2 && var == 3) e = launch_gemm2h_t<2, false, 3>(st, g);
         else if (ns == 2 && var == 4) e = launch_gemm2h_t<2, false, 4>(st, g);
diff --git a/cnmf_amd/csrc/gemm_host.hip.h b/cnmf_amd/csrc/gemm_host.hip.h
--- a/cnmf_amd/csrc/gemm_host.hip.h
+++ b/cnmf_amd/csrc/gemm_host.hip.h
@@ -191,7 +191,7 @@
     return hipGetLastError();
 }
 
-enum class XPlaneFormat { COUNT_BF16, COUNT_F16, SPLIT_F16 };
+enum class XPlaneFormat { COUNT_BF16, COUNT_F16, SPLIT_F16, COUNT_U8 };
 
 template <class F>
 static hipError_t launch_x_planes_t(hipStream_t st, bool transpose, const float* X, int ld, int N, int G, int rows_pad, int K,
@@ -219,6 +219,9 @@
     switch (fmt) {
         case XPlaneFormat::COUNT_BF16: return launch_x_planes_t<CountBf16>(st, transpose, X, ld, N, G, rows_pad, K, aux, plane0, plane1, flags);
         case XPlaneFormat::COUNT_F16: return launch_x_planes_t<CountF16>(st, transpose, X, ld, N, G, rows_pad, K, aux, plane0, plane1, flags);
+        case XPlaneFormat::COUNT_U8:
+            if (K % 32 || plane1) return hipErrorInvalidValue;
+            return launch_x_planes_t<CountU8>(st, transpose, X, ld, N, G, rows_pad, K, aux, plane0, nullptr, nullptr);
         default: return launch_x_planes_t<SplitF16>(st, transpose, X, ld, N, G, rows_pad, K, aux, plane0, plane1, flags);
     }
 }
@@ -317,58 +320,62 @@
 using G2Fn = hipError_t (*)(hipStream_t, const G2Launch&);
 struct G2Entry { G2Form form; G2Fn fn; };
 
-template <int NSUB, bool HI, int VAR = 0, bool PART = false, bool GEN = false>
+template <int NSUB, bool HI, int VAR = 0, bool PART = false, bool GEN = false, bool U8 = false>
 static hipError_t launch_gemm2h_t(hipStream_t st, const G2Launch& g)
 {
-    constexpr int lds = G2Geom<NSUB, HI>::LDS_BYTES;
-    {
-        if (hipError_t e_ = dyn_lds_optin((const void*)gemm2h_kernel<NSUB, HI, VAR, PART, GEN>, lds)) return e_;
+    constexpr int lds = G2Geom<NSUB, HI, U8>::LDS_BYTES;
+    if (g.x.bytes != U8) return hipErrorInvalidValue;
+    {
+        if (hipError_t e_ = dyn_lds_optin((const void*)gemm2h_kernel<NSUB, HI, VAR, PART, GEN, U8>, lds)) return e_;
     }
     int kb_per = (g.Kb + g.nsplit - 1) / g.nsplit;
     kb_per = ((kb_per + NSUB - 1) / NSUB) * NSUB;
     dim3 grid(g.Jpad / G3C_JW, g.KC / G3_MW, (g.Kb + kb_per - 1) / kb_per);
-    gemm2h_kernel<NSUB, HI, VAR, PART, GEN><<<grid, 512, lds, st>>>(g.A2, g.x.plane, HI ? g.x.hi : nullptr, HI ? g.x.flags : nullptr, g.rscale,
+    gemm2h_kernel<NSUB, HI, VAR, PART, GEN, U8><<<grid, 512, lds, st>>>(g.A2, g.x.plane, HI ? g.x.hi : nullptr, HI ? g.x.flags : nullptr, g.rscale,
                                                                    g.Kb, g.C[0], g.ldc, g.cstride, kb_per, g.x.colscale,
                                                                    PART ? g.livemask : ~0ull);
     return hipGetLastError();
 }
 
-template <int NSUB, bool HI, int VAR = 0, bool NTB = true, bool PART = false, bool GEN = false>
+template <int NSUB, bool HI, int VAR = 0, bool NTB = true, bool PART = false, bool GEN = false, bool U8 = false>
 static hipError_t launch_gemm2h_streamk_t(hipStream_t st, const G2Launch& g)
 {
-    constexpr int lds = G2Geom<NSUB, HI>::LDS_BYTES;
-    {
-        if (hipError_t e_ = dyn_lds_optin((const void*)gemm2h_streamk_kernel<NSUB, HI, VAR, NTB, PART, GEN>, lds)) return e_;
-    }
-    const int xmap = g2_xmap(G2Form{true, NSUB, HI, VAR, NTB, PART, GEN}, g.kn->g2_xmap);
-    gemm2h_streamk_kernel<NSUB, HI, VAR, NTB, PART, GEN><<<g.sk->P, 512, lds, st>>>(g.A2, g.x.plane, HI ? g.x.hi : nullptr,
+    constexpr int lds = G2Geom<NSUB, HI, U8>::LDS_BYTES;
+    if (g.x.bytes != U8) return hipErrorInvalidValue;
+    {
+        if (hipError_t e_ = dyn_lds_optin((const void*)gemm2h_streamk_kernel<NSUB, HI, VAR, NTB, PART, GEN, U8>, lds)) return e_;
+    }
+    const int xmap = g2_xmap(G2Form{true, NSUB, HI, VAR, NTB, PART, GEN, U8}, g.kn->g2_xmap);
+    gemm2h_streamk_kernel<NSUB, HI, VAR, NTB, PART, GEN, U8><<<g.sk->P, 512, lds, st>>>(g.A2, g.x.plane, HI ? g.x.hi : nullptr,
                                                                                     HI ? g.x.flags : nullptr, g.rscale, g.Kb, g.C[0], g.C[1],
                                                                                     g.C[2], g.ldc, g.sk->MG, g.sk->T, xmap, g.x.colscale,
                                                                                     PART ? g.livemask : ~0ull);
     return hipGetLastError();
 }
 
-template <int NSUB, bool HI, int VAR, bool PART, bool GEN>
-static constexpr G2Entry g2_ksplit() { return {G2Form{true, NSUB, HI, VAR, false, PART, GEN}, launch_gemm2h_t<NSUB, HI, VAR, PART, GEN>}; }
-template <int NSUB, bool HI, int VAR, bool NTB, bool PART, bool GEN>
-static constexpr G2Entry g2_streamk() { return {G2Form{true, NSUB, HI, VAR, NTB, PART, GEN}, launch_gemm2h_streamk_t<NSUB, HI, VAR, NTB, PART, GEN>}; }
+template <int NSUB, bool HI, int VAR, bool PART, bool GEN, bool U8 = false>
+static constexpr G2Entry g2_ksplit() { return {G2Form{true, NSUB, HI, VAR, false, PART, GEN, U8}, launch_gemm2h_t<NSUB, HI, VAR, PART, GEN, U8>}; }
+template <int NSUB, bool HI, int VAR, bool NTB, bool PART, bool GEN, bool U8 = false>
+static constexpr G2Entry g2_streamk() { return {G2Form{true, NSUB, HI, VAR, NTB, PART, GEN, U8}, launch_gemm2h_streamk_t<NSUB, HI, VAR, NTB, PART, GEN, U8>}; }
 
 static constexpr G2Entry G2_KSPLIT[] = {
     g2_ksplit<1, true, 0, false, true>(),  g2_ksplit<1, true, 0, true, true>(),  g2_ksplit<1, true, 4, false, true>(),
     g2_ksplit<1, true, 4, true, true>(),   g2_ksplit<1, true, 0, false, false>(), g2_ksplit<1, true, 0, true, false>(),
-    g2_ksplit<2, false, 4, false, false>(), g2_ksplit<2, false, 4, true, false>(), g2_ksplit<1, false, 4, false, false>()};
+    g2_ksplit<2, false, 4, false, false>(), g2_ksplit<2, false, 4, true, false>(), g2_ksplit<1, false, 4, false, false>(),
+    g2_ksplit<2, false, 4, false, false, true>(), g2_ksplit<2, false, 4, true, false, true>()};
 static constexpr G2Entry G2_STREAMK[] = {
     g2_streamk<1, true, 0, false, true, true>(),   g2_streamk<1, true, 0, false, false, true>(),  g2_streamk<1, true, 0, true, false, true>(),
     g2_streamk<1, true, 4, false, true, true>(),   g2_streamk<1, true, 4, false, false, true>(),  g2_streamk<1, true, 4, true, false, true>(),
     g2_streamk<1, true, 0, false, true, false>(),  g2_streamk<1, true, 0, false, false, false>(), g2_streamk<1, true, 0, true, false, false>(),
     g2_streamk<2, false, 4, false, true, false>(), g2_streamk<2, false, 4, false, false, false>(), g2_streamk<2, false, 4, true, false, false>(),
-    g2_streamk<1, false, 4, false, false, false>(), g2_streamk<1, false, 4, true, false, false>()};
+    g2_streamk<1, false, 4, false, false, false>(), g2_streamk<1, false, 4, true, false, false>(),
+    g2_streamk<2, false, 4, false, true, false, true>(), g2_streamk<2, false, 4, false, false, false, true>(), g2_streamk<2, false, 4, true, false, false, true>()};
 
 static G2Form g2_form_of(const G2Launch& g, int KC, bool shared)
 {
     const unsigned long long full = g2_full_mask(KC);
     return g2_form(g.x.hi != nullptr, g.x.colscale != nullptr, g.kn->g2_gen4, g.kn->g2_gvar, gemm2h_nsub(false, g.Kb, g.kn->g2_nsub),
-                   (g.livemask & full) != full, shared);
+                   (g.livemask & full) != full, shared, g.x.bytes);
 }
 
 static hipError_t launch_gemm2h(hipStream_t st, const G2Launch& g)
@@ -409,7 +416,7 @@
 
 static int ensure_counts(cnmf_ctx* ctx)
 {
-    const int fmt = ctx->knobs.gemm3 == 4 ? 4 : 3;
+    const int fmt = ctx->knobs.gemm3 == 4 ? ((ctx->knobs.g2_u8 && ctx->knobs.g2_nsub == 2) ? 5 : 4) : 3;
     if (ctx->counts.state == 1 && ctx->counts.fmt != fmt) {
         hipStreamSynchronize(ctx->stream);
         ctx->counts.release();
@@ -451,13 +458,16 @@
     HIP_TRY(ctx, hipMalloc(&L.d_scale, (size_t)ctx->G_pad * sizeof(double)));
     count_sums_kernel<<<grid, 256, 0, st>>>(ctx->X, ctx->G_pad, N, G, unit, psx, psn);
     count_scale_kernel<<<(ctx->G_pad + 255) / 256, 256, 0, st>>>(psx, psn, chunks, G, ctx->G_pad, L.d_scale);
-    unsigned* any_big = pool.get<unsigned>(1, true, st);
+    unsigned* any_big = pool.get<unsigned>(2, true, st);
     POOL_TRY(ctx, pool);
-    count_max_base_kernel<<<grid, 256, 0, st>>>(ctx->X, ctx->G_pad, N, G, unit, fmt == 4 ? G2_COUNT_BASE : 256.0f, any_big);
-    unsigned h_big = 0;
-    HIP_TRY(ctx, hipMemcpyAsync(&h_big, any_big, sizeof h_big, hipMemcpyDeviceToHost, st));
+    count_max_base_kernel<<<grid, 256, 0, st>>>(ctx->X, ctx->G_pad, N, G, unit, fmt >= 4 ? G2_COUNT_BASE : 256.0f, any_big);
+    if (fmt == 5) count_max_base_kernel<<<grid, 256, 0, st>>>(ctx->X, ctx->G_pad, N, G, unit, 255.0f, any_big + 1);
+    unsigned h_bigs[2] = {0, 0};
+    HIP_TRY(ctx, hipMemcpyAsync(h_bigs, any_big, sizeof h_bigs, hipMemcpyDeviceToHost, st));
     HIP_TRY(ctx, hipStreamSynchronize(st));
-    const size_t bytes = (size_t)ctx->N_pad * ctx->G_pad * 2;
+    const unsigned h_big = h_bigs[0];
+    L.bytes = fmt == 5 && !h_bigs[1];
+    const size_t bytes = (size_t)ctx->N_pad * ctx->G_pad * (L.bytes ? 1 : 2);
     HIP_TRY(ctx, hipMalloc(&L.C1, bytes));
     HIP_TRY(ctx, hipMalloc(&L.Ct1, bytes));
     if (h_big) {
@@ -470,7 +480,7 @@
         HIP_TRY(ctx, hipMemsetAsync(L.hiA, 0, nfA, st));
         HIP_TRY(ctx, hipMemsetAsync(L.hiB, 0, nfB, st));
     }
-    const XPlaneFormat pf = fmt == 4 ? XPlaneFormat::COUNT_F16 : XPlaneFormat::COUNT_BF16;
+    const XPlaneFormat pf = L.bytes ? XPlaneFormat::COUNT_U8 : (fmt >= 4 ? XPlaneFormat::COUNT_F16 : XPlaneFormat::COUNT_BF16);
     HIP_TRY(ctx, launch_x_planes(st, pf, false, ctx->X, ctx->G_pad, N, G, ctx->N_pad, ctx->G_pad, unit, L.C1, L.C1h, L.hiA));
     HIP_TRY(ctx, launch_x_planes(st, pf, true, ctx->X, ctx->G_pad, N, G, ctx->G_pad, ctx->N_pad, unit, L.Ct1, L.Ct1h, L.hiB));
     HIP_TRY(ctx, hipGetLastError());
diff --git a/cnmf_amd/csrc/kernels_gemm2h.hip.h b/cnmf_amd/csrc/kernels_gemm2h.hip.h
--- a/cnmf_amd/csrc/kernels_gemm2h.hip.h
+++ b/cnmf_amd/csrc/kernels_gemm2h.hip.h
@@ -1,28 +1,35 @@
 #pragma once
 #include <hip/hip_runtime.h>
 #include "kernels_gemm3.hip.h"
+#include "kernels_planes.hip.h"
 
 namespace cnmf {
 
 typedef _Float16 f16x8 __attribute__((ext_vector_type(8)));
 typedef float f32x4_g __attribute__((ext_vector_type(4)));
+typedef _Float16 f16x2_g __attribute__((ext_vector_type(2)));
+
+#ifndef G2_U8_SKIP
+#define G2_U8_SKIP 0
+#endif
 
 constexpr int G2_ROWB = 64;
 constexpr int G2_A = G3_MW * G2_ROWB;
 constexpr int G2_B = G3C_JW * 32;
 
-template <int NSUB, bool HI>
+template <int NSUB, bool HI, bool U8 = false>
 struct G2Geom {
     static_assert(NSUB == 1 || (NSUB == 2 && !HI), "two blocks per step: one count plane only");
+    static_assert(!U8 || NSUB == 2, "the byte plane is read by the 16x16x32 body only");
     static constexpr int IMGS = NSUB == 1 ? 4 : 3;
-    static constexpr int IMG = NSUB * (G2_A + (HI ? 2 : 1) * G2_B);
+    static constexpr int IMG = U8 ? NSUB * G2_A + G2_B : NSUB * (G2_A + (HI ? 2 : 1) * G2_B);
     static constexpr int OFF_B = NSUB * G2_A, OFF_H = OFF_B + NSUB * G2_B;
-    static constexpr int NA = NSUB * 2, NB = NSUB;
+    static constexpr int NA = NSUB * 2, NB = U8 ? 1 : NSUB;
     static constexpr int AHEAD = IMGS - 1;
     static constexpr int LDS_BYTES = IMGS * IMG;
 };
 
-template <int NSUB> struct G2Sub {};
+template <int NSUB, bool U8 = false> struct G2Sub {};
 
 #define G2_DMA_PIECE(NSUB_, HI_, NTB_, s_, i_)                                                     \
     {                                                                                              \
@@ -46,18 +53,19 @@
 }
 
 
-template <int VAR, bool NTB, bool PART>
+template <int VAR, bool NTB, bool PART, bool U8 = false>
 __device__ __forceinline__ void gemm2h_segment_mf16(const unsigned char* __restrict__ A2, const unsigned char* __restrict__ B1,
                                                     const float* __restrict__ rscale, int Kb, float* __restrict__ C,
                                                     int ldc, int m0, int j0, int kb0, int nkb, unsigned char* smem,
                                                     unsigned live)
 {
     static_assert(VAR == 0 || VAR == 2 || VAR == 3 || VAR == 4 || VAR == 6 || VAR == 7, "instruction streams 1 and 5 were retired");
-    using GEO = G2Geom<2, false>;
+    static_assert(!U8 || VAR == 0 || VAR == 4, "the byte plane has the burst and the spread stream only");
+    using GEO = G2Geom<2, false, U8>;
     constexpr int NSUB = 2, IMGS = GEO::IMGS, IMG = GEO::IMG, OFF_B = GEO::OFF_B, NA = GEO::NA, NB = GEO::NB, AHEAD = GEO::AHEAD;
     constexpr bool BURST = VAR == 0, NOMFMA = VAR == 2, NODMA = VAR == 3 || VAR == 6 || VAR == 7;
     constexpr bool NOREAD = VAR == 6 || VAR == 7, NOBAR = VAR == 7;
-    static_assert(IMGS == 3 && NA + NB == 6, "three images, six pieces per step");
+    static_assert(IMGS == 3 && NA + NB == (U8 ? 5 : 6), "three images, six pieces per step (bytes: five)");
     const int tid = threadIdx.x;
     const int lane = tid & 63, wave = tid >> 6;
     const int grp = wave >> 2, wn = wave & 3;
@@ -68,7 +76,8 @@
 #define G2_LIVE(mt_) (!PART || ((lv >> ((mt_) >> 1)) & 1u))
 
     const unsigned char* abase = A2 + ((size_t)(m0 / G3_MW) * Kb + kb0) * G2_A + tid * 16;
-    const unsigned char* bbase = B1 + ((size_t)(j0 / G3C_JW) * Kb + kb0) * G2_B + tid * 16;
+    const unsigned char* bbase = U8 ? B1 + ((size_t)(j0 / G3C_JW) * (Kb / NSUB) + kb0 / NSUB) * G2_B + tid * 16
+                                    : B1 + ((size_t)(j0 / G3C_JW) * Kb + kb0) * G2_B + tid * 16;
     constexpr const unsigned char* hbase = nullptr;
 
     f32x4_g acc[8][4];
@@ -81,21 +90,49 @@
 
     const int a_row = ub * G2_A + (grp * 128 + r) * G2_ROWB;
     const int a_s0 = ((0 + hf) ^ ((r >> 2) & 3)) * 16, a_s1 = ((2 + hf) ^ ((r >> 2) & 3)) * 16;
-    const int b_off = OFF_B + ub * G2_B + (wn * 64 + r) * 32 + (hf ^ ((r >> 3) & 1)) * 16;
-
-#define G2_PIECE(s_, i_) { G2_DMA_PIECE(2, false, NTB, s_, i_) __builtin_amdgcn_sched_barrier(0); }
+    const int b_off = U8 ? OFF_B + wn * 2048 + lane * 16 : OFF_B + ub * G2_B + (wn * 64 + r) * 32 + (hf ^ ((r >> 3) & 1)) * 16;
+
+#define G2_DMA_PIECE_U8(s_, i_)                                                                    \
+    {                                                                                              \
+        unsigned char* d_ = smem + ((s_) % IMGS) * IMG + wave * 1024;                              \
+        if ((i_) < NA)                                                                             \
+            __builtin_amdgcn_global_load_lds(G3_AS1(abase + (size_t)(s_) * (NSUB * G2_A) + (i_) * 8192), \
+                                             G3_AS3(d_ + (i_) * 8192), 16, 0, 0);                  \
+        else                                                                                       \
+            __builtin_amdgcn_global_load_lds(G3_AS1(bbase + (size_t)(s_) * G2_B), G3_AS3(d_ + OFF_B), 16, 0, NTB ? 2 : 0); \
+    }
+#define G2_PIECE(s_, i_) { if constexpr (U8) G2_DMA_PIECE_U8(s_, i_) else G2_DMA_PIECE(2, false, NTB, s_, i_) __builtin_amdgcn_sched_barrier(0); }
+#define G2_SPOT(MORE_, p_)                                                                         \
+    if (!BURST && MORE_) {                                                                         \
+        if constexpr (!U8) G2_PIECE(s + AHEAD, p_)                                                 \
+        else if constexpr ((p_) != G2_U8_SKIP) G2_PIECE(s + AHEAD, (p_) < G2_U8_SKIP ? (p_) : (p_) - 1) \
+    }
+#define G2_CVT2(w_, sel_) __builtin_bit_cast(unsigned, __builtin_bit_cast(f16x2_g, __builtin_amdgcn_perm(0x64646464u, (w_), (sel_))) - f16x2_g{(_Float16)1024.0f, (_Float16)1024.0f})
+#define G2_SEL_LO 0x04010400u
+#define G2_SEL_HI 0x04030402u
+#define G2_CVT(nt_)                                                                                \
+    {                                                                                              \
+        const unsigned w0_ = braw[(nt_) >> 1][2 * ((nt_) & 1)], w1_ = braw[(nt_) >> 1][2 * ((nt_) & 1) + 1]; \
+        u32x4 c_;                                                                                  \
+        c_.x = G2_CVT2(w0_, G2_SEL_LO); c_.y = G2_CVT2(w0_, G2_SEL_HI);                            \
+        c_.z = G2_CVT2(w1_, G2_SEL_LO); c_.w = G2_CVT2(w1_, G2_SEL_HI);                            \
+        bq[nt_] = __builtin_bit_cast(f16x8, c_);                                                   \
+    }
 #define G2_ISSUE(s_) { _Pragma("unroll") for (int i = 0; i < NA + NB; ++i) G2_PIECE(s_, i) }
 #define G2_FRAG(ptr_) __builtin_bit_cast(f16x8, *reinterpret_cast<const u32x4*>(ptr_))
 #define G2_AFRAG(bb_, mt_, q_) G2_FRAG((bb_) + a_row + (mt_) * 16 * G2_ROWB + ((q_) ? a_s1 : a_s0))
 #define G2_READ_A(s_)                                                                              \
     {                                                                                              \
         const unsigned char* bb = smem + ((s_) % IMGS) * IMG;                                      \
-        _Pragma("unroll") for (int nt = 0; nt < 4; ++nt) bq[nt] = G2_FRAG(bb + b_off + nt * 16 * 32); \
+        if constexpr (U8) { _Pragma("unroll") for (int p = 0; p < 2; ++p) braw[p] = *reinterpret_cast<const u32x4*>(bb + b_off + p * 1024); } \
+        else { _Pragma("unroll") for (int nt = 0; nt < 4; ++nt) bq[nt] = G2_FRAG(bb + b_off + nt * 16 * 32); } \
         _Pragma("unroll") for (int mp = 0; mp < 4; mp += 2) {                                      \
             aq[mp][1] = G2_AFRAG(bb, mp, 1); aq[mp + 1][1] = G2_AFRAG(bb, mp + 1, 1);              \
             aq[mp][0] = G2_AFRAG(bb, mp, 0); aq[mp + 1][0] = G2_AFRAG(bb, mp + 1, 0);              \
         }                                                                                          \
         __builtin_amdgcn_sched_barrier(0);                                                         \
+         \
+        if constexpr (U8) { _Pragma("unroll") for (int nt = 0; nt < 4; ++nt) G2_CVT(nt) }          \
     }
 #define G2_READ_B(s_)                                                                              \
     {                                                                                              \
@@ -119,31 +156,37 @@
         if (BURST && MORE_) G2_ISSUE(s + AHEAD)                                                    \
         if constexpr (NOREAD) { if (s == 0) { G2_READ_A(s) G2_READ_B(s) } } else { G2_READ_A(s) }  \
         G2_MF8(0, 1, 1)                                                                            \
-        if (!BURST && MORE_) G2_PIECE(s + AHEAD, 0)                                                \
+        G2_SPOT(MORE_, 0)                                                                          \
         G2_MF8(0, 1, 0)                                                                            \
         if constexpr (!NOREAD) { G2_READ_B(s) }                                                    \
-        if (!BURST && MORE_) G2_PIECE(s + AHEAD, 1)                                                \
+        G2_SPOT(MORE_, 1)                                                                          \
         G2_MF8(2, 3, 1)                                                                            \
-        if (!BURST && MORE_) G2_PIECE(s + AHEAD, 2)                                                \
+        G2_SPOT(MORE_, 2)                                                                          \
         G2_MF8(2, 3, 0)                                                                            \
         asm volatile("s_waitcnt lgkmcnt(0)" ::: "memory");       \
-         \
-        if (s + 1 < nst) { if (MORE_) { if constexpr (BURST) G3_WAIT_VM(6); else G3_WAIT_VM(3); } else G3_WAIT_VM(0); } \
+                                          \
+        if (s + 1 < nst) {                                                                         \
+            if (MORE_) {                                                                           \
+                if constexpr (U8) { if constexpr (BURST) G3_WAIT_VM(5); else if constexpr (G2_U8_SKIP < 3) G3_WAIT_VM(2); else G3_WAIT_VM(3); } \
+                else { if constexpr (BURST) G3_WAIT_VM(6); else G3_WAIT_VM(3); }                   \
+            } else G3_WAIT_VM(0);                                                                  \
+        }                                                                                          \
         if constexpr (!NOBAR) G3_RAW_BARRIER()                                            \
         G2_MF8(4, 5, 1)                                                                            \
-        if (!BURST && MORE_) G2_PIECE(s + AHEAD, 3)                                                \
+        G2_SPOT(MORE_, 3)                                                                          \
         G2_MF8(4, 5, 0)                                                                            \
-        if (!BURST && MORE_) G2_PIECE(s + AHEAD, 4)                                                \
+        G2_SPOT(MORE_, 4)                                                                          \
         G2_MF8(6, 7, 1)                                                                            \
-        if (!BURST && MORE_) G2_PIECE(s + AHEAD, 5)                                                \
+        G2_SPOT(MORE_, 5)                                                                          \
         G2_MF8(6, 7, 0)                                                                            \
     }
 
     f16x8 bq[4], aq[8][2];
+    u32x4 braw[2];
     G3_WAIT_VM(0);
     G2_ISSUE(0)
     if (nst > 1) G2_ISSUE(1)
-    if (nst > 1) G3_WAIT_VM(6); else G3_WAIT_VM(0);
+    if (nst > 1) { if constexpr (U8) G3_WAIT_VM(5); else G3_WAIT_VM(6); } else G3_WAIT_VM(0);
     if (grp == 1) G3_RAW_BARRIER()
     {
         int s = 0;
@@ -160,7 +203,13 @@
 #undef G2_AFRAG
 #undef G2_FRAG
 #undef G2_ISSUE
+#undef G2_CVT
+#undef G2_SEL_HI
+#undef G2_SEL_LO
+#undef G2_CVT2
+#undef G2_SPOT
 #undef G2_PIECE
+#undef G2_DMA_PIECE_U8
 
     if (C == nullptr) return;
 #pragma unroll
@@ -372,18 +421,18 @@
 #undef G2_LIVE
 }
 
-template <bool HI, int VAR, bool NTB, bool PART, bool GEN>
-__device__ __forceinline__ void gemm2h_segment(G2Sub<2>, const unsigned char* __restrict__ A2, const unsigned char* __restrict__ B1,
+template <bool HI, int VAR, bool NTB, bool PART, bool GEN, bool U8>
+__device__ __forceinline__ void gemm2h_segment(G2Sub<2, U8>, const unsigned char* __restrict__ A2, const unsigned char* __restrict__ B1,
                                                const unsigned char* __restrict__, const unsigned int* __restrict__,
                                                const float* __restrict__ rscale, int Kb, float* __restrict__ C, int ldc,
                                                int m0, int j0, int kb0, int nkb, unsigned char* smem, const float* __restrict__,
                                                unsigned live)
 {
     static_assert(!HI && !GEN, "two blocks per step: one count plane only");
-    gemm2h_segment_mf16<VAR, NTB, PART>(A2, B1, rscale, Kb, C, ldc, m0, j0, kb0, nkb, smem, live);
-}
-
-template <int NSUB, bool HI, int VAR = 0, bool PART = false, bool GEN = false>
+    gemm2h_segment_mf16<VAR, NTB, PART, U8>(A2, B1, rscale, Kb, C, ldc, m0, j0, kb0, nkb, smem, live);
+}
+
+template <int NSUB, bool HI, int VAR = 0, bool PART = false, bool GEN = false, bool U8 = false>
 __global__ __launch_bounds__(512) void gemm2h_kernel(const unsigned char* __restrict__ A2,
                                                      const unsigned char* __restrict__ B1,
                                                      const unsigned char* __restrict__ Bhi,
@@ -404,11 +453,11 @@
     }
     const int kb0 = z * kb_per;
     const int nkb = min(kb_per, Kb - kb0);
-    gemm2h_segment<HI, VAR, true, PART, GEN>(G2Sub<NSUB>{}, A2, B1, Bhi, hiflag, rscale, Kb, C ? C + (size_t)z * c_split_stride : nullptr, ldc, mg * G3_MW,
+    gemm2h_segment<HI, VAR, true, PART, GEN>(G2Sub<NSUB, U8>{}, A2, B1, Bhi, hiflag, rscale, Kb, C ? C + (size_t)z * c_split_stride : nullptr, ldc, mg * G3_MW,
                                                    jt * G3C_JW, kb0, nkb, smem3, cscale, (unsigned)((livemask >> (8 * mg)) & 0xffu));
 }
 
-template <int NSUB, bool HI, int VAR = 0, bool NTB = true, bool PART = false, bool GEN = false>
+template <int NSUB, bool HI, int VAR = 0, bool NTB = true, bool PART = false, bool GEN = false, bool U8 = false>
 __global__ __launch_bounds__(512) void gemm2h_streamk_kernel(const unsigned char* __restrict__ A2,
                                                              const unsigned char* __restrict__ B1,
                                                              const unsigned char* __restrict__ Bhi,
@@ -431,7 +480,7 @@
         const int tile = (int)(u / Ks), ks = (int)(u % Ks);
         const int ke = (int)min((long long)Ks, ks + (u1 - u));
         const int mg = tile / NJ, jt = tile % NJ;
-        gemm2h_segment<HI, VAR, NTB, PART, GEN>(G2Sub<NSUB>{}, A2, B1, Bhi, hiflag, rscale, Kb, (ks == 0) ? C0 : (ke == Ks ? C1 : C2), ldc, mg * G3_MW,
+        gemm2h_segment<HI, VAR, NTB, PART, GEN>(G2Sub<NSUB, U8>{}, A2, B1, Bhi, hiflag, rscale, Kb, (ks == 0) ? C0 : (ke == Ks ? C1 : C2), ldc, mg * G3_MW,
                                                       jt * G3C_JW, ks * NSUB, (ke - ks) * NSUB, smem3, cscale,
                                                       (unsigned)((livemask >> (8 * mg)) & 0xffu));
         u += ke - ks;
diff --git a/cnmf_amd/csrc/kernels_planes.hip.h b/cnmf_amd/csrc/kernels_planes.hip.h
--- a/cnmf_amd/csrc/kernels_planes.hip.h
+++ b/cnmf_amd/csrc/kernels_planes.hip.h
@@ -38,7 +38,7 @@
 template <int BASE>
 struct CountFormat {
     using Aux = float;
-    static constexpr bool FLAGGED = true;
+    static constexpr bool FLAGGED = true, BYTES = false;
     static __device__ __forceinline__ float value(const float* __restrict__ X, size_t at, bool inside,
                                                   const float* __restrict__ unit, int , int gene)
     {
@@ -65,9 +65,15 @@
         a = f16_bits(lo); b = f16_bits(hi);
     }
 };
+struct CountU8 : CountFormat<255> {
+    static constexpr bool SWIZZLE = false, FLAGGED = false, BYTES = true;
+    static __device__ __forceinline__ void pair(float n, unsigned short& a, unsigned short& b) { a = (unsigned short)n; b = 0; }
+};
+__host__ __device__ constexpr int g2_u8_chunk(int rin, int g) { return (rin >> 5) * 1024 + (g * 16 + (rin & 15)) * 16 + ((rin >> 4) & 1) * 8; }
+
 struct SplitF16 {
     using Aux = int;
-    static constexpr bool SWIZZLE = true, FLAGGED = false;
+    static constexpr bool SWIZZLE = true, FLAGGED = false, BYTES = false;
     static __device__ __forceinline__ float value(const float* __restrict__ X, size_t at, bool inside,
                                                   const int* __restrict__ shift, int row, int )
     {
@@ -115,6 +121,18 @@
         const float v = F::value(X, (size_t)cell * ld + gene, cell < N && gene < G, aux, row, gene);
         F::pair(v, p0[i], p1[i]);
         any1 |= p1[i] != 0;
+    }
+    if constexpr (F::BYTES) {
+        const int rin = row % TR;
+        unsigned char* d = reinterpret_cast<unsigned char*>(plane0) + ((size_t)(row / TR) * (Kb / 2) + (kb >> 1)) * ((size_t)TR * 32);
+#pragma unroll
+        for (int hf = 0; hf < 2; ++hf) {
+            uint2 w;
+            w.x = p0[8 * hf + 0] | ((unsigned)p0[8 * hf + 1] << 8) | ((unsigned)p0[8 * hf + 2] << 16) | ((unsigned)p0[8 * hf + 3] << 24);
+            w.y = p0[8 * hf + 4] | ((unsigned)p0[8 * hf + 5] << 8) | ((unsigned)p0[8 * hf + 6] << 16) | ((unsigned)p0[8 * hf + 7] << 24);
+            *reinterpret_cast<uint2*>(d + g2_u8_chunk(rin, 2 * (kb & 1) + hf)) = w;
+        }
+        return;
     }
     const int rin = row % TR, swz = F::SWIZZLE ? (rin >> 3) & 1 : 0;
     const size_t at = (((size_t)(row / TR) * Kb + kb) * TR + rin) * 16;
diff --git a/cnmf_amd/csrc/pass_plan.h b/cnmf_amd/csrc/pass_plan.h
--- a/cnmf_amd/csrc/pass_plan.h
+++ b/cnmf_amd/csrc/pass_plan.h
@@ -168,12 +168,13 @@
 static inline int gemm2h_nsub(bool hi, int Kb, int nsub_knob) { return (!hi && nsub_knob == 2 && Kb % 2 == 0) ? 2 : 1; }
 
 struct G2Form {
-    bool valid; int NSUB; bool HI; int VAR; bool NTB, PART, GEN;
-    bool operator==(const G2Form& o) const { return valid == o.valid && NSUB == o.NSUB && HI == o.HI && VAR == o.VAR && NTB == o.NTB && PART == o.PART && GEN == o.GEN; }
-};
-
-static inline G2Form g2_form(bool hi, bool gen, bool gen4, int gvar, int nsub, bool part, bool shared)
-{
+    bool valid; int NSUB; bool HI; int VAR; bool NTB, PART, GEN; bool U8 = false;
+    bool operator==(const G2Form& o) const { return valid == o.valid && NSUB == o.NSUB && HI == o.HI && VAR == o.VAR && NTB == o.NTB && PART == o.PART && GEN == o.GEN && U8 == o.U8; }
+};
+
+static inline G2Form g2_form(bool hi, bool gen, bool gen4, int gvar, int nsub, bool part, bool shared, bool u8 = false)
+{
+    if (u8) return (hi || gen || nsub != 2) ? G2Form{false, 1, false, 0, false, false, false} : G2Form{true, 2, false, 4, !part && !shared, part, false, true};
     if (gen && !hi) return G2Form{false, 1, false, 0, false, false, false};
     const bool ntb = !part && !shared;
     if (hi && gen && !gen4) return G2Form{true, 1, true, gvar == 0 ? 0 : 4, ntb, part, true};
diff --git a/cnmf_amd/csrc/runtime.hip.h b/cnmf_amd/csrc/runtime.hip.h
--- a/cnmf_amd/csrc/runtime.hip.h
+++ b/cnmf_amd/csrc/runtime.hip.h
@@ -77,7 +77,7 @@
     void free_all() { hipFree(p); }
 };
 
-struct XOperand { const unsigned char *plane, *hi; const unsigned int* flags; const float* colscale; };
+struct XOperand { const unsigned char *plane, *hi; const unsigned int* flags; const float* colscale; bool bytes = false; };
 
 struct Bf16PlanesF {
     unsigned char *X3 = nullptr, *Xt3 = nullptr;
@@ -88,13 +88,14 @@
 struct CountPlanesF {
     int state = 0;
     int fmt = 0;
+    bool bytes = false;
     unsigned char *C1 = nullptr, *Ct1 = nullptr;
     unsigned char *C1h = nullptr, *Ct1h = nullptr;
     unsigned int *hiA = nullptr, *hiB = nullptr;
     double* d_scale = nullptr;
     void free_all() { hipFree(C1); hipFree(Ct1); hipFree(C1h); hipFree(Ct1h); hipFree(hiA); hipFree(hiB); hipFree(d_scale); }
-    XOperand passA() const { return {C1, C1h, hiA, nullptr}; }
-    XOperand passB() const { return {Ct1, Ct1h, hiB, nullptr}; }
+    XOperand passA() const { return {C1, C1h, hiA, nullptr, bytes}; }
+    XOperand passB() const { return {Ct1, Ct1h, hiB, nullptr, bytes}; }
 };
 
 struct GeneralPlanesF {
@@ -207,6 +208,7 @@
     bool g2_gen4 = false;
     int  g2_nsub = 2;
     int  g2_xmap = -1;
+    bool g2_u8 = true;
     bool part = false;
     bool no_psum = false;
     bool wide_small = true;
@@ -294,6 +296,7 @@
     k.g2_gen4 = ctx_getenv(ctx, "CNMF_G2_GEN4") != nullptr;
     k.g2_nsub = num(ctx_getenv(ctx, "CNMF_G2_NSUB"), 2) == 1 ? 1 : 2;
     k.g2_xmap = num(ctx_getenv(ctx, "CNMF_G2_XMAP"), -1);
+    k.g2_u8 = num(ctx_getenv(ctx, "CNMF_G2_U8"), 1) != 0;
     k.part = ctx_getenv(ctx, "CNMF_PART") != nullptr;
     k.no_psum = ctx_getenv(ctx, "CNMF_NO_PSUM") != nullptr;
     k.wide_small = num(ctx_getenv(ctx, "CNMF_WIDE_SMALL"), 1) != 0;
diff --git a/cnmf_amd/engine.py b/cnmf_amd/engine.py
--- a/cnmf_amd/engine.py
+++ b/cnmf_amd/engine.py
@@ -188,7 +188,8 @@
     def matrix_images(self):
         f = C.c_int32(0)
         self._check(self._lib.cnmf_matrix_images(self._ctx, C.byref(f)))
-        names = ("dense", "csr", "csr_of_transpose", "dense_transpose", "non_zero_images_16", "non_zero_images_32", "count_planes")
+        names = ("dense", "csr", "csr_of_transpose", "dense_transpose", "non_zero_images_16", "non_zero_images_32", "count_planes",
+                 "count_planes_bytes")
         return {n: bool(f.value >> i & 1) for i, n in enumerate(names)}
 
     def get_matrix(self):
@@ -1716,8 +1717,8 @@
                                                 C.byref(ms), int(reps)))
         return Cout, ms.value
 
-    def debug_gemm2h(self, A, Bn, nsplit=1, nsub=2, reps=0, sweep_bound=False):
-        nsub = int(nsub) | (128 if sweep_bound else 0)
+    def debug_gemm2h(self, A, Bn, nsplit=1, nsub=2, reps=0, sweep_bound=False, count_bytes=False):
+        nsub = int(nsub) | (128 if sweep_bound else 0) | (256 if count_bytes else 0)
         A = np.ascontiguousarray(A, dtype=np.float32)
         Bn = np.ascontiguousarray(Bn, dtype=np.float32)
         KC, K = A.shape
```
